# graphcore-research/bess-kge

Measured on AMD Instinct MI355X. Metric: positive+negative triples scored/sec, higher is better.
Workload: dtype f32; 1 GPU; ogbl-biokg-shaped ComplEx d=256 fp32 (W=512), 93,773 entities per shard, n_shard=1, S=4096 positives x 256 per-triple negatives per GPU per step, EmbeddingMoving, mode=score (gather+score+loss); negatives_per_triple=256, mode=score, collectives=none

## Files before the change

bess-kge_amd/besskge/_native.py:

```python

import contextlib
import ctypes
import pathlib
import sys
import threading
from typing import Any, List, Optional, Sequence, Tuple

import torch

LIB_NAME = "libbesskge_hip.so"
ABI_VERSION = 3

TRANSE, ROTATE, DISTMULT, COMPLEX, AFFINE, BOXE = 0, 1, 2, 3, 4, 5
F32, F16 = 0, 1
CORRUPT_HEAD, CORRUPT_TAIL = 0, 1
LOSS_LOGSIGMOID, LOSS_MARGIN, LOSS_SSCE = 0, 1, 2
BAD_NEGATIVE_SCORE = -50000.0

_c_i32p = ctypes.POINTER(ctypes.c_int32)
_c_f32p = ctypes.POINTER(ctypes.c_float)
_c_u8p = ctypes.POINTER(ctypes.c_uint8)
_vp = ctypes.c_void_p
_i64 = ctypes.c_int64
_RETURNS_I64 = ("bess_neg_score_shared_workspace", "bess_neg_score_shared_bwd_workspace",
                "bess_neg_score_shared_fwd_counts_workspace", "bess_neg_score_shared_fwd_pairs_workspace",
                "bess_neg_score_table_fwd_counts_workspace", "bess_neg_score_table_fwd_pairs_workspace")
_i32 = ctypes.c_int32
_f32 = ctypes.c_float


class ModelDesc(ctypes.Structure):

    _fields_ = [
        ("scorer", _i32),
        ("norm_p", _i32),
        ("dtype", _i32),
        ("width", _i32),
        ("rel_width", _i32),
        ("reserved", _i32 * 3),
    ]


class LossDesc(ctypes.Structure):

    _fields_ = [
        ("kind", _i32),
        ("adversarial", _i32),
        ("margin", _f32),
        ("adversarial_scale", _f32),
        ("loss_scale", _f32),
        ("ssce_shift", _f32),
        ("reserved", _i32 * 2),
    ]


class OptDesc(ctypes.Structure):

    _fields_ = [
        ("kind", _i32),
        ("step", _i32),
        ("lr", _f32),
        ("momentum", _f32),
        ("beta1", _f32),
        ("beta2", _f32),
        ("eps", _f32),
        ("weight_decay", _f32),
        ("step_ptr", _i64),
        ("slot_map", _i64),
    ]


OPT_SGD, OPT_ADAGRAD, OPT_ADAM = 0, 1, 2
FLAG_FP32_MATH = 1
FLAG_PREZEROED = 2
FLAG_DNEG_BY_ROW = 4


class KillDesc(ctypes.Structure):

    _fields_ = [
        ("diag_step", _i32),
        ("ht", _i32),
        ("ppp", _i32),
        ("reserved", _i32),
        ("mask", _vp),
        ("mask_rows", _i64),
        ("mask_cols", _i64),
    ]


class Pcg64State(ctypes.Structure):

    _fields_ = [
        ("state_hi", ctypes.c_uint64),
        ("state_lo", ctypes.c_uint64),
        ("inc_hi", ctypes.c_uint64),
        ("inc_lo", ctypes.c_uint64),
        ("has_uint32", ctypes.c_uint32),
        ("uinteger", ctypes.c_uint32),
    ]


_PG = ctypes.POINTER(Pcg64State)

_MD = ctypes.POINTER(ModelDesc)
_LD = ctypes.POINTER(LossDesc)

SIGNATURES = {
    "bess_version": [],
    "bess_last_error": [ctypes.c_char_p, ctypes.c_size_t],
    "bess_gather_rows": [_i32, _i32, _vp, _vp, _i64, _vp, _vp],
    "bess_score_triple_fwd": [_MD, _vp, _vp, _vp, _vp, _vp, _vp, _i64, _vp, _vp],
    "bess_score_triple_bwd": [_MD, _vp, _vp, _vp, _vp, _vp, _vp, _i64, _vp, _vp, _vp, _vp, _vp],
    "bess_query_fwd": [_MD, _i32, _vp, _vp, _vp, _vp, _i64, _vp, _vp],
    "bess_query_bwd": [_MD, _i32, _vp, _vp, _vp, _vp, _i64, _vp, _vp, _vp, _vp],
    "bess_query_triple_fwd": [_MD, _i32, _vp, _vp, _vp, _vp, _vp, _vp, _i64, _vp, _vp, _vp],
    "bess_query_triple_bwd": [_MD, _i32, _vp, _vp, _vp, _vp, _vp, _vp, _i64, _vp, _vp, _vp, _vp, _vp, _vp],
    "bess_sparse_sgd_lists": [_i32, _i32, _vp, _i32, ctypes.POINTER(_vp), ctypes.POINTER(_vp), ctypes.POINTER(_i64), _f32, _vp],
    "bess_sparse_sgd_lists_axpy": [_i32, _i32, _vp, _i32, ctypes.POINTER(_vp), ctypes.POINTER(_vp), ctypes.POINTER(_i64), _f32,
                                   _vp, _vp, _i64, _f32, _vp],
    "bess_neg_score_pertriple_fwd": [_MD, _vp, _i64, _vp, _vp, _i64, _vp, _i64, _vp],
    "bess_neg_score_pertriple_bwd": [_MD, _vp, _i64, _vp, _vp, _i64, _vp, _i64, _vp, _vp, _vp],
    "bess_neg_score_shared_fwd": [_MD, _vp, _i64, _vp, _vp, _i64, _vp, _i64, _vp],
    "bess_neg_score_shared_workspace": [_MD, _i64, _i64],
    "bess_neg_score_shared_fwd_ws": [_MD, _vp, _i64, _vp, _vp, _i64, _vp, _i64, _vp, _i64, _vp],
    "bess_neg_score_shared_fwd_pruned": [_MD, _vp, _i64, _vp, _vp, _i64, _vp, _i64, _vp, _vp, _i64, _vp, _i64, _vp],
    "bess_neg_score_shared_fwd_counts_workspace": [_MD, _i64, _i64],
    "bess_neg_score_shared_fwd_counts": [_MD, _vp, _i64, _vp, _vp, _i64, _vp, _vp, _vp, _i32, _vp, _i64, _vp],
    "bess_neg_score_shared_fwd_pairs_workspace": [_MD, _i64, _i64],
    "bess_neg_score_shared_fwd_pairs": [_MD, _vp, _vp, _vp, _i64, _i64, _i64, _vp, _vp, _i64, _vp],
    "bess_neg_score_table_fwd_counts_workspace": [_MD, _i64, _i64],
    "bess_neg_score_table_fwd_counts": [_MD, _vp, _i64, _vp, _vp, _i64, _vp, _vp, _vp, _i32, _vp, _i64, _vp],
    "bess_neg_score_table_fwd_pairs_workspace": [_MD, _i64, _i64],
    "bess_neg_score_table_fwd_pairs": [_MD, _vp, _vp, _vp, _i64, _i64, _i64, _vp, _vp, _i64, _vp],
    "bess_topk_update_flagged": [_vp, _i64, _i64, _i64, _vp, _i64, _i32, _vp, _vp, _i32, _vp],
    "bess_neg_score_shared_fwd_masked": [_MD, _vp, _i64, _vp, _vp, _i64, _vp, _i64, ctypes.POINTER(KillDesc), _vp, _i64, _vp],
    "bess_neg_score_shared_bwd": [_MD, _vp, _i64, _vp, _vp, _i64, _vp, _i64, _vp, _i64, _vp, _vp, _vp],
    "bess_neg_score_shared_bwd_workspace": [_MD, _i64, _i64],
    "bess_neg_score_shared_bwd_ws": [_MD, _vp, _i64, _vp, _vp, _i64, _vp, _i64, _vp, _i64, _vp, _vp, _vp, _i64, _vp],
    "bess_mask_scores": [_vp, _i64, _i64, _i64, _i32, _i32, _i32, _vp, _i64, _i64, _vp],
    "bess_loss_fwd_bwd": [_LD, _vp, _vp, _i64, _i64, _i64, _vp, _i64, _vp, _vp, _vp, _vp, _i64, _vp],
    "bess_loss_fwd_bwd_norm": [_LD, _vp, _vp, _i64, _i64, _i64, _vp, _i64, _vp, _vp, _vp, _vp, _i64, _vp, _vp],
    "bess_loss_fwd_bwd_one_launch": [_LD, _vp, _vp, _i64, _i64, _i64, _vp, _i64, _vp, _vp, _vp, _vp, _i64, _vp, _vp, _vp],
    "bess_scatter_add_rows": [_vp, _i32, _vp, _vp, _i64, _f32, _vp],
    "bess_sparse_sgd": [_i32, _i32, _vp, _vp, _vp, _i64, _f32, _vp],
    "bess_dense_sgd": [_i32, _vp, _vp, _i64, _f32, _vp],
    "bess_segment_index_workspace": [_i64, ctypes.POINTER(ctypes.c_size_t)],
    "bess_build_segment_index": [_vp, _i64, _i32, _vp, _vp, _vp, _vp, _vp, _i64, _vp, ctypes.c_size_t, _vp],
    "bess_pad_segments": [_vp, _vp, _i64, _vp, _i32, _vp],
    "bess_step_prologue": [_i32, ctypes.POINTER(_vp), ctypes.POINTER(_vp), ctypes.POINTER(ctypes.c_uint32),
                           ctypes.POINTER(_i64), _i32, ctypes.POINTER(_vp), ctypes.POINTER(_i64), _i32, _vp, _vp, _vp, _vp,
                           _vp, _i64, _vp],
    "bess_neg_pertriple_grad_segments": [_MD, _vp, _i64, _vp, _i64, _vp, _i64, _vp, _vp, _vp, _vp, _i64, _vp, _f32,
                                         _vp, _i64, _vp, _vp, _vp],
    "bess_apply_segments_sgd": [_i32, _i32, _vp, _vp, _vp, _i64, _vp, _f32, _vp],
    "bess_segment_sum_rows": [_i32, _vp, _vp, _vp, _vp, _i64, _vp, _vp],
    "bess_topk_update": [_vp, _i64, _i64, _i64, _vp, _i64, _i32, _vp, _i64, _vp, _vp, _i32, _vp],
    "bess_topk_update_excl": [_vp, _i64, _i64, _i64, _vp, _i64, _i32, _vp, _i64, _vp, _vp, _i64, _i32, _vp, _vp, _i32, _vp],
    "bess_topk_update_flagged_excl": [_vp, _i64, _i64, _i64, _vp, _i64, _vp, _i32, _vp, _vp, _i64, _i32, _vp, _vp, _i32, _vp],
    "bess_ranks_from_scores": [_vp, _vp, _i64, _i64, _i64, _i32, _i32, _vp, _vp],
    "bess_ranks_from_indices": [_vp, _vp, _i64, _i64, _i32, _vp, _vp],
    "bess_apply_segments_opt": [ctypes.POINTER(OptDesc), _i32, _i32, _vp, _vp, _vp, _i64, _vp, _vp, _vp, _vp, _vp],
    "bess_neg_pertriple_step_segments": [_MD, _vp, _i64, _vp, _i64, _vp, _i64, _vp, _vp, _vp, _vp, _i64,
                                         _vp, _i64, _vp, _vp, ctypes.POINTER(OptDesc), _vp, _vp, _vp, _vp, _vp],
    "bess_map_extra_rows": [_vp, _vp, _i64, _vp, _vp, _i64, _vp, _vp, _vp],
    "bess_assign_state_rows": [_vp, _vp, _i64, _vp, _vp, _vp, _i64, _vp],
    "bess_coalesced_update": [ctypes.POINTER(OptDesc), _i32, _i32, _vp, _i32, ctypes.POINTER(_vp), ctypes.POINTER(_i64),
                              _vp, _vp, _vp, _vp, _i64, _vp, _vp, _vp, _vp, _vp],
    "bess_coalesced_update_axpy": [ctypes.POINTER(OptDesc), _i32, _i32, _vp, _i32, ctypes.POINTER(_vp), ctypes.POINTER(_i64),
                                   _vp, _vp, _vp, _vp, _i64, _vp, _vp, _vp, _vp, _vp, _vp, _i64, _f32, _vp],
    "bess_neg_pertriple_items": [_MD, _i64, _i64, ctypes.POINTER(ctypes.c_int32)],
    "bess_neg_pertriple_sweep": [_MD, _i64, _i64, ctypes.POINTER(ctypes.c_int32)],
    "bess_neg_score_pertriple_fwd_dq": [_MD, _LD, _vp, _i64, _vp, _vp, _i64, _vp, _vp, _i64, _vp, _i64, _vp, _vp, _vp, _vp],
    "bess_neg_score_pertriple_fwd_dq_masked": [_MD, _LD, _vp, _i64, _vp, _vp, _i64, _vp, _vp, _i64, _vp, _i64, _i64, _vp, _i64, _vp,
                                               _vp, _vp, _vp],
    "bess_neg_score_pertriple_fwd_partials": [_MD, _LD, _vp, _i64, _vp, _vp, _i64, _vp, _i64, _vp, _vp, _vp],
    "bess_combine_dq_partials": [_vp, _vp, _i64, _i32, _i32, _vp, _vp, _vp],
    "bess_normalize_rows": [_i32, _vp, _vp, _i64, _i32, _i32, _i32, _vp, _vp, _vp],
    "bess_normalize_rows_bwd": [_vp, _vp, _vp, _i64, _i32, _i32, _vp, _vp],
    "bess_sample_negatives": [_PG, _vp, _i64, _i32, _i32, _i32, _i64, _i64, _vp, _vp, _vp, _vp, _i32, _i32, _vp, _vp],
    "bess_sample_bucket_indices": [_PG, _vp, _i64, _i64, _i64, _vp, _vp, _vp, _vp],
    "bess_lookup_triples": [_vp, _i64, _vp, _i64, _i64, _i64, _i64, _i32, _vp, _vp, _vp, _vp],
    "bess_gather_candidate_lists": [_vp, _vp, _vp, _vp, _i64, _vp, _i64, _i64, _i64, _i64, _i64, _i64, _i64, _i32, _vp, _vp, _vp],
    "bess_comm_unique_id": [_c_u8p],
    "bess_comm_init_rank": [_i32, _i32, _c_u8p, ctypes.POINTER(_vp)],
    "bess_comm_init_all": [_i32, _c_i32p, ctypes.POINTER(_vp)],
    "bess_comm_destroy": [_vp],
    "bess_comm_info": [_vp, _c_i32p, _c_i32p, _c_i32p],
    "bess_alltoall": [_vp, _vp, _vp, _i64, _vp],
    "bess_allgather": [_vp, _vp, _vp, _i64, _vp],
    "bess_allreduce_sum_f32": [_vp, _vp, _vp, _i64, _vp],
    "bess_pack_exchange": [_vp, _i32, _i32, _vp, _vp, _i64, _vp, _vp, _vp],
    "bess_graph_node_counts": [_vp, _c_i32p, _i32],
    "bess_plan_create": [ctypes.POINTER(_vp)],
    "bess_plan_destroy": [_vp],
    "bess_plan_knows": [ctypes.c_char_p],
    "bess_plan_length": [_vp],
    "bess_plan_add_call": [_vp, ctypes.c_char_p, _i32, _c_u8p, ctypes.POINTER(ctypes.c_uint64), ctypes.POINTER(_vp),
                           ctypes.POINTER(_i64)],
    "bess_plan_run": [_vp, _vp],
    "bess_direct_update": [ctypes.POINTER(OptDesc), _i32, _i32, _vp, _i32, ctypes.POINTER(_vp), ctypes.POINTER(_i64), _vp, _vp,
                           _vp, _vp, _vp, _vp, _vp, _i64, _f32, _vp],
    "bess_neg_score_shared_bwd_parts_plan": [_MD, _i64, _i64, _c_i32p, _c_i32p],
    "bess_neg_score_shared_bwd_parts": [_MD, _vp, _i64, _vp, _vp, _i64, _vp, _i64, _vp, _vp, _vp],
    "bess_query_triple_bwd_parts": [_MD, _i32, _vp, _vp, _vp, _vp, _vp, _vp, _i64, _vp, _vp, _i32, _vp, _i32, _i64, _vp,
                                    _vp, _vp, _vp, _vp, _vp],
    "bess_pertriple_tail_supported": [_MD, _i64],
    "bess_pertriple_tail": [_MD, _LD, _i32, _vp, _vp, _vp, _vp, _vp, _vp, _i64, _vp, _vp, _i32, _vp, _vp, _i64, _i64, _vp,
                            _i64, _vp, _vp, _vp, _vp, _i64, _vp, _vp, _vp, _vp, _vp, _vp],
    "bess_query_triple_fwd_jobs": [_MD, _i32, _vp, _vp, _vp, _vp, _vp, _vp, _i64, _vp, _vp, _i32, ctypes.POINTER(_vp),
                                   ctypes.POINTER(_vp), ctypes.POINTER(ctypes.c_uint32), ctypes.POINTER(_i64), _vp],
    "bess_neg_score_shared_fwd_loss": [_MD, _vp, _i64, _vp, _vp, _i64, _vp, _i64, ctypes.POINTER(KillDesc), _LD, _vp, _vp, _i64,
                                       _vp, _vp, _vp, _vp, _i64, _vp, _vp, _i64, _vp],
}
COMM_ID_BYTES = 128
AFFINE_COUNT_CHUNK_BYTES = 32 << 20
TICKET_INTS = 544
ECOMM_BASE = 10000

_lib: Optional[ctypes.CDLL] = None

_timing: Optional[list] = None
_timed_names: frozenset = frozenset()

TIMING_LABELS = {
    "bess_neg_score_pertriple_fwd_dq_masked": "bess_neg_score_pertriple_fwd_dq",
    "bess_neg_score_shared_fwd_ws": "bess_neg_score_shared_fwd",
    "bess_neg_score_shared_fwd_masked": "bess_neg_score_shared_fwd",
    "bess_neg_score_shared_fwd_pruned": "bess_neg_score_shared_fwd",
    "bess_neg_score_shared_bwd_ws": "bess_neg_score_shared_bwd",
    "bess_neg_score_shared_bwd_parts": "bess_neg_score_shared_bwd",
    "bess_sparse_sgd_lists_axpy": "bess_sparse_sgd_lists",
    "bess_coalesced_update_axpy": "bess_coalesced_update",
    "bess_topk_update_flagged": "bess_topk_update",
    "bess_topk_update_excl": "bess_topk_update",
    "bess_topk_update_flagged_excl": "bess_topk_update",
}


class _Recording(threading.local):
    plan: Optional["Plan"] = None


_recording = _Recording()


def start_kernel_timing(names: Sequence[str]) -> None:
    global _timing, _timed_names
    _timing, _timed_names = [], frozenset(names)


def kernel_timing_log() -> list:
    return list(_timing or [])


def stop_kernel_timing() -> dict:
    global _timing
    rec, _timing = _timing or [], None
    torch.cuda.synchronize()
    out: dict = {}
    for name, _, a, b in rec:
        out.setdefault(TIMING_LABELS.get(name, name), []).append(a.elapsed_time(b))
    return out


def library_path() -> pathlib.Path:
    return pathlib.Path(__file__).parent.absolute() / LIB_NAME


def load() -> ctypes.CDLL:
    global _lib
    if _lib is not None:
        return _lib
    path = library_path()
    if not path.exists():
        raise ImportError(
            f"Cannot find the HIP extension library {LIB_NAME} - tried {[str(path)]}."
            " Build it with `python -c 'import __graft_entry__ as g; g.build()'`"
            " (or `make -C bess-kge_amd/csrc`)."
        )
    lib = ctypes.CDLL(str(path))
    for name, argtypes in SIGNATURES.items():
        try:
            fn = getattr(lib, name)
        except AttributeError as e:
            raise ImportError(f"{path} does not export {name}") from e
        fn.argtypes = argtypes
        fn.restype = ctypes.c_int64 if name in _RETURNS_I64 else ctypes.c_int
    if lib.bess_version() != ABI_VERSION:
        raise ImportError(
            f"{path}: ABI version {lib.bess_version()} != expected {ABI_VERSION}"
        )
    _lib = lib
    return lib


def _check(rc: int, what: str) -> None:
    if rc != 0:
        buf = ctypes.create_string_buffer(512)
        load().bess_last_error(buf, 512)
        kind = "invalid argument" if rc < 0 else (f"ncclResult {rc - ECOMM_BASE}" if rc >= ECOMM_BASE else f"hipError {rc}")
        raise RuntimeError(f"besskge native call {what} failed ({kind}): {buf.value.decode()}")


def _dtype_code(t: torch.Tensor) -> int:
    if t.dtype == torch.float32:
        return F32
    if t.dtype == torch.float16:
        return F16
    raise TypeError(f"embedding tables must be float32 or float16, got {t.dtype}")


def _dev(t: torch.Tensor, name: str) -> torch.device:
    if not t.is_cuda:
        raise RuntimeError(
            f"besskge: `{name}` is on {t.device}; the BESS hot path runs on"
            " HIP devices only (there is no CPU fallback)"
        )
    return t.device


def _same_device(ts: Sequence[Tuple[str, Optional[torch.Tensor]]]) -> torch.device:
    dev = None
    for name, t in ts:
        if t is None:
            continue
        d = _dev(t, name)
        if dev is None:
            dev = d
        elif d != dev:
            raise RuntimeError(f"besskge: `{name}` is on {d}, expected {dev}")
    assert dev is not None
    return dev


def _rows(base: torch.Tensor, name: str, width: int) -> None:
    if base.dim() != 2 or base.shape[1] != width or not base.is_contiguous():
        raise ValueError(
            f"`{name}` must be a contiguous [rows, {width}] tensor, got"
            f" shape {tuple(base.shape)} stride {base.stride()}"
        )


def _idx(idx: Optional[torch.Tensor], name: str, n: Optional[int] = None) -> int:
    if idx is None:
        return 0
    if idx.dtype != torch.int32 or idx.dim() != 1 or not idx.is_contiguous():
        raise ValueError(
            f"`{name}` must be a contiguous 1-D int32 tensor, got {idx.dtype} {tuple(idx.shape)}"
        )
    if n is not None and idx.numel() != n:
        raise ValueError(f"`{name}` has {idx.numel()} entries, expected {n}")
    return idx.data_ptr()


def _f32(t: torch.Tensor, name: str) -> None:
    if t.dtype != torch.float32 or not t.is_contiguous():
        raise ValueError(f"`{name}` must be contiguous float32, got {t.dtype}")


def _row_count(base: torch.Tensor, idx: Optional[torch.Tensor]) -> int:
    return int(idx.numel()) if idx is not None else int(base.shape[0])


def _stream(dev: torch.device) -> int:
    return torch._C._cuda_getCurrentRawStream(dev.index if dev.index is not None else torch.cuda.current_device())


_NO_SWITCH = contextlib.nullcontext()


def _on(dev: torch.device) -> Any:
    if dev.index is None or torch.cuda.current_device() == dev.index:
        return _NO_SWITCH
    return torch.cuda.device(dev)


def _launch(name: str, dev: torch.device, *args: Any) -> None:
# ... 99 lines not shown
    out = torch.empty((n,), dtype=torch.float32, device=dev)
    _launch("bess_score_triple_fwd", dev, ctypes.byref(d), head.base.data_ptr(), _idx(head.idx, "head_idx"),
            tail.base.data_ptr(), _idx(tail.idx, "tail_idx"), rel_table.data_ptr(), rel_idx.data_ptr(), n,
            out.data_ptr())
    return out


def score_triple_bwd(d: ModelDesc, head: RowSource, tail: RowSource, rel_table: torch.Tensor,
                     rel_idx: torch.Tensor, d_out: torch.Tensor, d_rel_table: torch.Tensor
                     ) -> Tuple[torch.Tensor, torch.Tensor]:
    dev, n = _triple_operands(d, head, tail, rel_table, rel_idx)
    _same_device([("d_out", d_out), ("d_rel_table", d_rel_table), ("x", head.base)])
    _f32(d_out, "d_out")
    _f32(d_rel_table, "d_rel_table")
    if d_out.numel() != n or tuple(d_rel_table.shape) != tuple(rel_table.shape):
        raise ValueError("score_triple_bwd: gradient shapes do not match")
    dh = torch.empty((n, d.width), dtype=torch.float32, device=dev)
    dt = torch.empty((n, d.width), dtype=torch.float32, device=dev)
    _launch("bess_score_triple_bwd", dev, ctypes.byref(d), head.base.data_ptr(), _idx(head.idx, "head_idx"),
            tail.base.data_ptr(), _idx(tail.idx, "tail_idx"), rel_table.data_ptr(), rel_idx.data_ptr(), n,
            d_out.data_ptr(), dh.data_ptr(), dt.data_ptr(), d_rel_table.data_ptr())
    return dh, dt


def _job_arrays(jobs: Sequence[Tuple[torch.Tensor, Optional[torch.Tensor], int]], who: str):
    nj = len(jobs)
    if nj > MAX_WORD_JOBS:
        raise ValueError(f"{who}: too many jobs")
    dst, src = (_vp * max(1, nj))(), (_vp * max(1, nj))()
    val, words = (ctypes.c_uint32 * max(1, nj))(), (_i64 * max(1, nj))()
    for i, (d_, s_, v_) in enumerate(jobs):
        if d_.element_size() != 4 or not d_.is_contiguous():
            raise ValueError(f"{who}: job targets must be contiguous tensors of 4-byte elements")
        if s_ is not None and (s_.element_size() != 4 or not s_.is_contiguous() or s_.numel() != d_.numel()):
            raise ValueError(f"{who}: a job's source must match its target")
        dst[i], src[i], val[i], words[i] = d_.data_ptr(), (s_.data_ptr() if s_ is not None else None), int(v_), d_.numel()
    return dst, src, val, words


def query_triple_fwd(d: ModelDesc, side: int, head: RowSource, tail: RowSource, rel_table: torch.Tensor,
                     rel_idx: torch.Tensor, jobs: Optional[Sequence[Tuple[torch.Tensor, Optional[torch.Tensor], int]]] = None
                     ) -> Tuple[torch.Tensor, torch.Tensor]:
    dev, n = _triple_operands(d, head, tail, rel_table, rel_idx)
    q = torch.empty((n, d.width), dtype=torch.float32, device=dev)
    out = torch.empty((n,), dtype=torch.float32, device=dev)
    if jobs:
        _same_device([("query rows", head.base)] + [("job dst", j[0]) for j in jobs] + [("job src", j[1]) for j in jobs])
        dst, src, val, words = _job_arrays(jobs, "query_triple_fwd")
        _launch("bess_query_triple_fwd_jobs", dev, ctypes.byref(d), side, head.base.data_ptr(),
                _idx(head.idx, "head_idx"), tail.base.data_ptr(), _idx(tail.idx, "tail_idx"), rel_table.data_ptr(),
                rel_idx.data_ptr(), n, q.data_ptr(), out.data_ptr(), len(jobs), dst, src, val, words)
        return q, out
    _launch("bess_query_triple_fwd", dev, ctypes.byref(d), side, head.base.data_ptr(), _idx(head.idx, "head_idx"),
            tail.base.data_ptr(), _idx(tail.idx, "tail_idx"), rel_table.data_ptr(), rel_idx.data_ptr(), n, q.data_ptr(),
            out.data_ptr())
    return q, out


def query_triple_bwd(d: ModelDesc, side: int, head: RowSource, tail: RowSource, rel_table: torch.Tensor,
                     rel_idx: torch.Tensor, d_out: torch.Tensor, d_query: torch.Tensor, d_rel_table: torch.Tensor
                     ) -> Tuple[torch.Tensor, torch.Tensor]:
    dev, n = _triple_operands(d, head, tail, rel_table, rel_idx)
    _same_device([("d_out", d_out), ("d_query", d_query), ("d_rel_table", d_rel_table), ("x", head.base)])
    for t, nm in ((d_out, "d_out"), (d_query, "d_query"), (d_rel_table, "d_rel_table")):
        _f32(t, nm)
    if d_out.numel() != n or tuple(d_query.shape) != (n, d.width) or tuple(d_rel_table.shape) != tuple(rel_table.shape):
        raise ValueError("query_triple_bwd: gradient shapes do not match")
    dh = torch.empty((n, d.width), dtype=torch.float32, device=dev)
    dt = torch.empty((n, d.width), dtype=torch.float32, device=dev)
    _launch("bess_query_triple_bwd", dev, ctypes.byref(d), side, head.base.data_ptr(), _idx(head.idx, "head_idx"),
            tail.base.data_ptr(), _idx(tail.idx, "tail_idx"), rel_table.data_ptr(), rel_idx.data_ptr(), n,
            d_out.data_ptr(), d_query.data_ptr(), dh.data_ptr(), dt.data_ptr(), d_rel_table.data_ptr())
    return dh, dt


def _query_operands(d: ModelDesc, ent: RowSource, rel_table: torch.Tensor, rel_idx: torch.Tensor):
    dev = _same_device([("entity rows", ent.base), ("entity idx", ent.idx),
                        ("relation_embedding", rel_table), ("relation", rel_idx)])
    _rows(ent.base, "entity rows", d.width)
    _rows(rel_table, "relation_embedding", d.rel_width)
    if _dtype_code(ent.base) != d.dtype or _dtype_code(rel_table) != d.dtype:
        raise TypeError("query: operand dtype does not match the model descriptor")
    n = len(ent)
    _idx(rel_idx, "relation", n)
    return dev, n


def query_fwd(d: ModelDesc, side: int, ent: RowSource, rel_table: torch.Tensor, rel_idx: torch.Tensor) -> torch.Tensor:
    dev, n = _query_operands(d, ent, rel_table, rel_idx)
    q = torch.empty((n, query_width(d)), dtype=torch.float32, device=dev)
    _launch("bess_query_fwd", dev, ctypes.byref(d), side, ent.base.data_ptr(), _idx(ent.idx, "entity idx"),
            rel_table.data_ptr(), rel_idx.data_ptr(), n, q.data_ptr())
    return q


def query_bwd(d: ModelDesc, side: int, ent: RowSource, rel_table: torch.Tensor, rel_idx: torch.Tensor,
              d_query: torch.Tensor, d_rel_table: torch.Tensor) -> torch.Tensor:
    dev, n = _query_operands(d, ent, rel_table, rel_idx)
    _same_device([("d_query", d_query), ("d_rel_table", d_rel_table), ("x", ent.base)])
    _f32(d_query, "d_query")
    _f32(d_rel_table, "d_rel_table")
    if tuple(d_query.shape) != (n, query_width(d)) or tuple(d_rel_table.shape) != tuple(rel_table.shape):
        raise ValueError("query_bwd: gradient shapes do not match")
    dx = torch.empty((n, d.width), dtype=torch.float32, device=dev)
    _launch("bess_query_bwd", dev, ctypes.byref(d), side, ent.base.data_ptr(), _idx(ent.idx, "entity idx"),
            rel_table.data_ptr(), rel_idx.data_ptr(), n, d_query.data_ptr(), dx.data_ptr(), d_rel_table.data_ptr())
    return dx


def query_width(d: ModelDesc) -> int:
    if d.scorer == AFFINE:
        n_part = int(d.reserved[0])
        return (n_part + 1) * (d.width // n_part)
    if d.scorer == BOXE:
        return 3 * d.width
    return int(d.width)


def _neg_operands(d: ModelDesc, query: torch.Tensor, neg: RowSource, n_idx: int):
    dev = _same_device([("query", query), ("negative rows", neg.base), ("negative idx", neg.idx)])
    _f32(query, "query")
    if query.dim() != 2 or query.shape[1] != query_width(d):
        raise ValueError(f"`query` must be [n_query, {query_width(d)}], got {tuple(query.shape)}")
    _rows(neg.base, "negative rows", d.width)
    if _dtype_code(neg.base) != d.dtype:
        raise TypeError("negative rows dtype does not match the model descriptor")
    if len(neg) != n_idx:
        raise ValueError(f"expected {n_idx} negative rows, got {len(neg)}")
    return dev


def _neg_idx_ptr(neg: RowSource, dev: torch.device) -> Tuple[int, Optional[torch.Tensor]]:
    if neg.idx is not None:
        return _idx(neg.idx, "negative idx"), None
    ar = torch.arange(neg.base.shape[0], dtype=torch.int32, device=dev)
    return ar.data_ptr(), ar


def neg_score_pertriple_fwd(d: ModelDesc, query: torch.Tensor, neg: RowSource, n_neg: int,
                            out: Optional[torch.Tensor] = None) -> torch.Tensor:
    nq = int(query.shape[0])
    dev = _neg_operands(d, query, neg, nq * n_neg)
    if out is None:
        out = torch.empty((nq, n_neg), dtype=torch.float32, device=dev)
    _f32(out, "out")
    if tuple(out.shape) != (nq, n_neg):
        raise ValueError("neg_score_pertriple_fwd: bad `out` shape")
    ip, keep = _neg_idx_ptr(neg, dev)
    d = with_row_count(d, neg.base)
    _launch("bess_neg_score_pertriple_fwd", dev, ctypes.byref(d), query.data_ptr(), nq, neg.base.data_ptr(), ip, n_neg,
            out.data_ptr(), n_neg)
    del keep
    return out


def neg_score_pertriple_fwd_dq(d: ModelDesc, l: LossDesc, query: torch.Tensor, neg: RowSource, n_neg: int,
                               pos: Optional[torch.Tensor], weight: torch.Tensor, mask: Optional[torch.Tensor] = None,
                               defer: bool = False) -> Tuple[torch.Tensor, Any]:
    nq = int(query.shape[0])
    dev = _neg_operands(d, query, neg, nq * n_neg)
    _same_device([("pos", pos), ("weight", weight), ("query", query)])
    _f32(weight, "weight")
    if weight.numel() not in (1, nq):
        raise ValueError("triple weights must have 1 or n_query entries")
    if pos is not None:
        _f32(pos, "pos")
        if pos.numel() != nq:
            raise ValueError("`pos` must have n_query entries")
    items = ctypes.c_int32(0)
    _check(load().bess_neg_pertriple_items(ctypes.byref(d), nq, n_neg, ctypes.byref(items)), "bess_neg_pertriple_items")
    out = torch.empty((nq, n_neg), dtype=torch.float32, device=dev)
    dq = None if defer else torch.empty((nq, d.width), dtype=torch.float32, device=dev)
    st_ml = torch.empty((nq, items.value, 2), dtype=torch.float32, device=dev)
    st_acc = torch.empty((nq, items.value, d.width), dtype=torch.float32, device=dev)
    ip, keep = _neg_idx_ptr(neg, dev)
    mrows = mcols = 0
    if mask is not None:
        _same_device([("mask", mask), ("query", query)])
        if mask.dtype not in (torch.bool, torch.uint8) or mask.dim() != 2 or not mask.is_contiguous():
            raise ValueError("neg_score_pertriple_fwd_dq: `mask` must be a contiguous 2-D bool / uint8 tensor")
        mrows, mcols = int(mask.shape[0]), int(mask.shape[1])
    _launch("bess_neg_score_pertriple_fwd_dq_masked", dev, ctypes.byref(d), ctypes.byref(l), query.data_ptr(), nq,
            neg.base.data_ptr(), ip, n_neg, pos.data_ptr() if pos is not None else 0, weight.data_ptr(), weight.numel(),
            mask.data_ptr() if mask is not None else 0, mrows, mcols, out.data_ptr(), n_neg,
            dq.data_ptr() if dq is not None else 0, st_ml.data_ptr(), st_acc.data_ptr())
    del keep
    return out, ((st_ml, st_acc) if defer else dq)


def pertriple_tail_supported(d: ModelDesc, n_neg: int) -> bool:
    return bool(load().bess_pertriple_tail_supported(ctypes.byref(d), int(n_neg)))


def pertriple_tail(d: ModelDesc, l: LossDesc, side: int, head: RowSource, tail: RowSource, rel_table: torch.Tensor,
                   rel_idx: torch.Tensor, partials: Tuple[torch.Tensor, torch.Tensor], pos: torch.Tensor, neg: torch.Tensor,
                   weight: torch.Tensor, d_rel_table: torch.Tensor, want_d_query: bool = False) -> Tuple[Any, ...]:
    dev, n = _triple_operands(d, head, tail, rel_table, rel_idx)
    st_ml, st_acc = partials
    _same_device([("partials", st_ml), ("partials", st_acc), ("positive_score", pos), ("negative_score", neg),
                  ("triple_weight", weight), ("d_rel_table", d_rel_table), ("x", head.base)])
    for t, nm in ((st_ml, "partials"), (st_acc, "partials"), (pos, "positive_score"), (neg, "negative_score"),
                  (weight, "triple_weight"), (d_rel_table, "d_rel_table")):
        _f32(t, nm)
    N = int(neg.shape[1])
    items = int(st_ml.shape[1])
    if tuple(st_ml.shape) != (n, items, 2) or tuple(st_acc.shape) != (n, items, d.width) or pos.numel() != n \
            or neg.shape[0] != n or weight.numel() not in (1, n) or tuple(d_rel_table.shape) != tuple(rel_table.shape):
        raise ValueError("pertriple_tail: shapes do not match")
    n4 = (n + 3) // 4 * 4
    small = torch.empty((2 * n4 + 4,), dtype=torch.float32, device=dev)
    row_loss, dp, loss = small[:n], small[n4: n4 + n], small[2 * n4: 2 * n4 + 1]
    dn = torch.empty((n, N), dtype=torch.float32, device=dev)
    rows = torch.empty((3 if want_d_query else 2, n, d.width), dtype=torch.float32, device=dev)
    counter = _counters(dev, 1)
    _launch("bess_pertriple_tail", dev, ctypes.byref(d), ctypes.byref(l), side, head.base.data_ptr(),
            _idx(head.idx, "head_idx"), tail.base.data_ptr(), _idx(tail.idx, "tail_idx"), rel_table.data_ptr(),
            rel_idx.data_ptr(), n, st_ml.data_ptr(), st_acc.data_ptr(), items, pos.data_ptr(), neg.data_ptr(), N,
            int(neg.stride(0)), weight.data_ptr(), weight.numel(), row_loss.data_ptr(), loss.data_ptr(), dp.data_ptr(),
            dn.data_ptr(), N, rows[2].data_ptr() if want_d_query else 0, rows[0].data_ptr(), rows[1].data_ptr(),
            d_rel_table.data_ptr(), counter.data_ptr())
    res = (loss.reshape(()), dp, dn, rows[0], rows[1])
    return res + (rows[2],) if want_d_query else res


def row_fits_registers(d: ModelDesc) -> bool:
    W = int(d.width)
    vec = 4 if d.dtype == F32 else 8
    if W % vec:
        vec = 2 if (d.dtype == F16 and W % 2 == 0) else 1
    return W <= 256 * vec


def neg_score_pertriple_fwd_partials(d: ModelDesc, l: LossDesc, query: torch.Tensor, neg: RowSource, n_neg: int
                                     ) -> Tuple[torch.Tensor, Tuple[torch.Tensor, torch.Tensor]]:
    nq = int(query.shape[0])
    dev = _neg_operands(d, query, neg, nq * n_neg)
    items = ctypes.c_int32(0)
    _check(load().bess_neg_pertriple_items(ctypes.byref(d), nq, n_neg, ctypes.byref(items)), "bess_neg_pertriple_items")
    out = torch.empty((nq, n_neg), dtype=torch.float32, device=dev)
    st_ml = torch.empty((nq, items.value, 2), dtype=torch.float32, device=dev)
    st_acc = torch.empty((nq, items.value, d.width), dtype=torch.float32, device=dev)
    ip, keep = _neg_idx_ptr(neg, dev)
    _launch("bess_neg_score_pertriple_fwd_partials", dev, ctypes.byref(d), ctypes.byref(l), query.data_ptr(), nq,
            neg.base.data_ptr(), ip, n_neg, out.data_ptr(), n_neg, st_ml.data_ptr(), st_acc.data_ptr())
    del keep
    return out, (st_ml, st_acc)


def combine_dq_partials(state: Tuple[torch.Tensor, torch.Tensor], norm: torch.Tensor) -> torch.Tensor:
    st_ml, st_acc = state
    nq, items, W = (int(x) for x in st_acc.shape)
    dev = _same_device([("state_ml", st_ml), ("state_acc", st_acc), ("norm", norm)])
    _f32(norm, "norm")
    if tuple(norm.shape) != (nq, 2) or not norm.is_contiguous():
        raise ValueError("combine_dq_partials: `norm` must be a contiguous [n_query, 2] tensor")
    dq = torch.empty((nq, W), dtype=torch.float32, device=dev)
    _launch("bess_combine_dq_partials", dev, st_ml.data_ptr(), st_acc.data_ptr(), nq, items, W, norm.data_ptr(),
            dq.data_ptr())
    return dq


def neg_score_pertriple_bwd(d: ModelDesc, query: torch.Tensor, neg: RowSource, n_neg: int,
                            d_out: torch.Tensor, want_d_neg: bool = True, want_d_query: bool = True,
                            d_neg_rows: Optional[torch.Tensor] = None
                            ) -> Tuple[Optional[torch.Tensor], Optional[torch.Tensor]]:
    nq = int(query.shape[0])
    dev = _neg_operands(d, query, neg, nq * n_neg)
    _same_device([("d_out", d_out), ("query", query)])
    _f32(d_out, "d_out")
    if tuple(d_out.shape) != (nq, n_neg):
        raise ValueError("neg_score_pertriple_bwd: bad `d_out` shape")
    if not want_d_query and (int(d.scorer) > COMPLEX or not want_d_neg):
        raise ValueError("neg_score_pertriple_bwd: want_d_query=False is for the four native scorers, with d_neg")
    dq = torch.empty((nq, query_width(d)), dtype=torch.float32, device=dev) if want_d_query else None
    dn = torch.empty((nq * n_neg, d.width), dtype=torch.float32, device=dev) if want_d_neg else None
    if d_neg_rows is not None:
        if (int(d.scorer) > COMPLEX or not want_d_neg or d_neg_rows.dtype != torch.float32 or not d_neg_rows.is_contiguous()
                or tuple(d_neg_rows.shape) != (int(neg.base.shape[0]), int(d.width)) or d_neg_rows.device != dev):
            raise ValueError("neg_score_pertriple_bwd: `d_neg_rows` must be a contiguous f32 [rows of neg.base, W] "
                             "tensor (native scorers)")
        d = copy_desc(d)
        d.reserved[0] |= FLAG_DNEG_BY_ROW
        dn = d_neg_rows
    ip, keep = _neg_idx_ptr(neg, dev)
    _launch("bess_neg_score_pertriple_bwd", dev, ctypes.byref(d), query.data_ptr(), nq, neg.base.data_ptr(), ip, n_neg,
            d_out.data_ptr(), n_neg, dq.data_ptr() if want_d_query else 0, dn.data_ptr() if want_d_neg else 0)
    del keep
    return dq, (None if d_neg_rows is not None else dn)


def normalize_rows(neg: RowSource, n_part: int, normalize: bool) -> Tuple[torch.Tensor, torch.Tensor]:
    dev = _same_device([("rows", neg.base), ("idx", neg.idx)])
    W = int(neg.base.shape[1])
    _rows(neg.base, "rows", W)
    n = len(neg)
    hat = torch.empty((n, W), dtype=torch.float32, device=dev)
    inv = torch.empty((n, n_part), dtype=torch.float32, device=dev)
    _launch("bess_normalize_rows", dev, _dtype_code(neg.base), neg.base.data_ptr(), _idx(neg.idx, "idx"), n, W, n_part,
            int(normalize), hat.data_ptr(), inv.data_ptr())
    return hat, inv


def normalize_rows_bwd(hat: torch.Tensor, inv: torch.Tensor, d_hat: torch.Tensor) -> torch.Tensor:
    dev = _same_device([("hat", hat), ("inv", inv), ("d_hat", d_hat)])
    for t, name in ((hat, "hat"), (inv, "inv"), (d_hat, "d_hat")):
        _f32(t, name)
# ... 1149 lines not shown
```

bess-kge_amd/besskge/bess.py:

```python

from abc import ABC, abstractmethod
from typing import Any, Dict, List, Optional, Tuple, Union

import torch

from besskge import _native as nat
from besskge._native import RowSource
from besskge.collectives import ReplicaGroup, SingleProcessGroup
from besskge.loss import BaseLossFunction, SampledSoftmaxCrossEntropyLoss
from besskge.negative_sampler import (
    ShardedNegativeSampler,
    TripleBasedShardedNegativeSampler,
)
from besskge.scoring import BaseScoreFunction

BAD_NEGATIVE_SCORE = -50000.0

_Batch = Dict[str, torch.Tensor]



def _i32(x: torch.Tensor) -> torch.Tensor:
    x = x if x.dtype == torch.int32 else x.to(torch.int32)
    return x.contiguous()


class _PlainSGD:

    kind = nat.OPT_SGD
    momentum = 0.0
    weight_decay = 0.0
    is_plain_sgd = True

    def __init__(self, lr: float) -> None:
        self.lr = float(lr)


class _NegGroup:

    def __init__(self, side: int, sel: Optional[torch.Tensor], ent: RowSource, rel_idx: torch.Tensor,
                 neg: RowSource, shared: bool, n_per_query: int) -> None:
        self.side = side
        self.sel = sel
        self.ent = ent
        self.rel_idx = rel_idx
        self.neg = neg
        self.shared = shared
        self.n_per_query = n_per_query
        self.query: Optional[torch.Tensor] = None
        self.query_ctx: Any = None
        self.out: Optional[torch.Tensor] = None
        self.dq: Optional[torch.Tensor] = None
        self.partials: Any = None
        self.kill: Any = None
        self.neg_parts: Optional[List[torch.Tensor]] = None
        self.bwd_buf: Optional[torch.Tensor] = None


class _SmallPlan(list):

    def __init__(self) -> None:
        super().__init__()
        self.concats: Dict[int, Tuple[int, int]] = {}


class _ReplicaStep:

    def __init__(self) -> None:
        self.table: torch.Tensor = None
        self.triple_ctx: Any = None
        self.head_idx: torch.Tensor = None
        self.rel_idx: torch.Tensor = None
        self.tail: RowSource = None
        self.groups: List[_NegGroup] = []
        self.send_idx: Optional[torch.Tensor] = None
        self.recv: Optional[torch.Tensor] = None
        self.recv_rows: int = 0
        self.ext_src: Optional[RowSource] = None
        self.n: int = 1
        self.ppp: int = 0
        self.neg_shape: Tuple[int, ...] = ()
        self.local_neg: torch.Tensor = None
        self.local_tail: torch.Tensor = None
        self.positive_score: torch.Tensor = None
        self.negative_score: torch.Tensor = None
        self.loss_norm: Optional[torch.Tensor] = None
        self.kill_applied = False
        self.fused_qt = False
        self.tail_pre: Optional[Tuple[torch.Tensor, torch.Tensor]] = None
        self.jobs: Optional[List[Tuple[torch.Tensor, Optional[torch.Tensor], int]]] = None
        self.d_recv: Optional[torch.Tensor] = None
        self.loss_pre: Optional[Tuple[torch.Tensor, torch.Tensor, torch.Tensor]] = None
        self.direct: Any = None
        self.direct_lists: List[torch.Tensor] = []
        self.jobs_ride = False


class _PendingUpdate:

    __slots__ = ("steps", "local_updates", "deferred", "d_rel")

    def __init__(self, steps: List[_ReplicaStep], local_updates: List[List[Tuple[torch.Tensor, torch.Tensor]]],
                 deferred: List[Tuple[torch.Tensor, _NegGroup, torch.Tensor]], d_rel: torch.Tensor) -> None:
        self.steps = steps
        self.local_updates = local_updates
        self.deferred = deferred
        self.d_rel = d_rel


class _MergedGroup:

    __slots__ = ("query", "n_per_query")

    def __init__(self, query: torch.Tensor, n_per_query: int) -> None:
        self.query, self.n_per_query = query, n_per_query


class BessKGE(torch.nn.Module, ABC):

    def __init__(
        self,
        negative_sampler: ShardedNegativeSampler,
        score_fn: BaseScoreFunction,
        loss_fn: Optional[BaseLossFunction] = None,
        evaluation: Optional[Any] = None,
        return_scores: bool = False,
        augment_negative: bool = False,
    ) -> None:
        super().__init__()
        self.sharding = score_fn.sharding
        self.negative_sampler = negative_sampler
        self.score_fn = score_fn
        self.loss_fn = loss_fn
        self.evaluation = evaluation
        self.return_scores = return_scores
        self.augment_negative = augment_negative
        if not (loss_fn or evaluation or return_scores):
            raise ValueError(
                "Nothing to return. At least one of loss_fn,"
                " evaluation or return_scores needs to be != None"
            )
        if self.augment_negative:
            assert (
                score_fn.negative_sample_sharing
            ), "Negative augmentation requires negative sample sharing"
            assert not isinstance(
                self, ScoreMovingBessKGE
            ), "ScoreMovingBessKGE does not support negative augmentation"
        if negative_sampler.flat_negative_format:
            assert (
                score_fn.negative_sample_sharing
            ), "Using flat negative format requires negative sample sharing"
        elif score_fn.negative_sample_sharing and isinstance(
            self.negative_sampler, TripleBasedShardedNegativeSampler
        ):
            raise ValueError(
                "Negative sample sharing cannot be used"
                " with non-flat triple-specific negatives"
            )
        self.entity_embedding = self.score_fn.entity_embedding
        self.entity_embedding_size: int = self.score_fn.entity_embedding.shape[-1]
        self.replica_group: Optional[ReplicaGroup] = None
        self._shard_slot: Optional[Dict[int, int]] = None
        self._map_cache: Dict[Any, torch.Tensor] = {}

    @property
    def n_embedding_parameters(self) -> int:
        return self.score_fn.entity_embedding.numel() + self.score_fn.relation_embedding.numel()

    def attach(self, group: ReplicaGroup, shard_slot: Optional[Dict[int, int]] = None) -> None:
        if group.n_shard != self.sharding.n_shard:
            raise ValueError(f"group has {group.n_shard} replicas, sharding {self.sharding.n_shard}")
        self.replica_group = group
        self._shard_slot = shard_slot

    def _group(self) -> ReplicaGroup:
        if self.replica_group is None:
            self.replica_group = SingleProcessGroup(self.sharding.n_shard)
        return self.replica_group

    def _local_table(self, shard: int) -> torch.Tensor:
        emb = self.score_fn.entity_embedding
        slot = shard if self._shard_slot is None else self._shard_slot[shard]
        if emb.dim() != 3 or slot >= emb.shape[0]:
            raise RuntimeError(
                f"entity_embedding {tuple(emb.shape)} does not hold shard {shard};"
                " use besskge.runtime to place the shards"
            )
# ... 566 lines not shown
                contrib = list(upd)
                for table, g, go in deferred:
                    if table is st.table:
                        seg = seg_index[id(g)]
                        gseg = nat.neg_pertriple_grad_segments(desc, g.query, table, g.n_per_query, go, seg)
                        contrib.append(nat.pad_segments(seg, gseg))
                last = st is steps[-1]
                self._apply_optimizer(optimizer, st.table, contrib,
                                      (getattr(self, "_small_ahead", None) or {}).get(id(st)),
                                      axpy=rel_axpy if last else None)
                rel_done = rel_done or (last and rel_axpy is not None)
        if rel_done:
            pass
        elif plain:
            nat.dense_sgd(rel_table, d_rel, lr)
        else:
            self._apply_optimizer_dense(optimizer, rel_table, d_rel)
        dense_grads = self.score_fn.__dict__.pop("dense_grads", {})
        for p in self.score_fn.dense_parameters():
            g = dense_grads.get(p)
            if g is None:
                continue
            (g,) = group.all_reduce_sum([g.contiguous()]) if len(group.local_shards) == 1 else (g,)
            as_table = p.data.view(p.shape[0], -1) if p.dim() > 1 else p.data.view(1, -1)
            g = g.reshape(as_table.shape).contiguous()
            if mean_over_replicas:
                g = g / group.n_shard
            if plain:
                nat.dense_sgd(as_table, g, lr)
            else:
                self._apply_optimizer_dense(optimizer, as_table, g)


    def _run_groups_one(self, g: _NegGroup, desc: nat.ModelDesc, st: Optional[_ReplicaStep] = None,
                        fuse: Optional[Dict[str, Any]] = None, partials_loss: Any = None) -> torch.Tensor:
        ahead = getattr(self, "_seg_ahead", None)
        if ahead is not None and st is not None and self._wants_segments(g, st):
            ahead[id(g)] = self._segment_index_on_side(g, st)
        if g.query is None:
            g.query, g.query_ctx = self.score_fn.query_fwd(g.side, g.ent, g.rel_idx)
        with_loss = getattr(self, "_train_loss_in_scoring", None)
        if g.shared and with_loss is not None and st is not None and len(st.groups) == 1 and g.sel is None \
                and (st.kill_applied or with_loss.get("no_kill")):
            b = with_loss["batch"]
            w = self._triple_weight(b, g.query.device)
            g.out, loss, d_pos, d_neg = nat.neg_score_shared_fwd_loss(
                desc, self.loss_fn.kernel_desc(len(g.neg)), g.query, g.neg, st.positive_score, w, kill=g.kill)
            st.loss_pre = (loss, d_pos, d_neg)
        elif g.shared:
            g.out = nat.neg_score_shared_fwd(desc, g.query, g.neg, kill=g.kill)
        elif fuse is not None and st is not None and (
                g.neg.base is st.table or (g.neg.base is st.recv and self.score_fn.bilinear_candidates)):
            pos, w = st.positive_score, fuse["weight"]
            if g.sel is not None:
                pos = pos[g.sel].contiguous()
                w = w if w.numel() == 1 else w[g.sel].contiguous()
            d_rel = self.__dict__.get("_step_d_rel")
            defer = (self.pertriple_tail and st.fused_qt and g.sel is None and g.neg.base is st.table and d_rel is not None
                     and not self.evaluation and nat.pertriple_tail_supported(desc, g.n_per_query))
            ldesc = fuse["loss"](g.n_per_query)
            g.out, g.dq = nat.neg_score_pertriple_fwd_dq(desc, ldesc, g.query, g.neg, g.n_per_query, pos, w,
                                                         mask=fuse.get("mask"), defer=defer)
            if defer:
                loss, d_pos, d_neg, dh, dt = nat.pertriple_tail(
                    desc, ldesc, g.side, RowSource(st.table, st.head_idx), st.tail, self.score_fn.relation_embedding.data,
                    st.rel_idx, g.dq, pos, g.out, w, d_rel)
                st.loss_pre = (loss, d_pos, d_neg)
                st.tail_pre = (dh, dt)
        elif partials_loss is not None:
            g.out, g.partials = nat.neg_score_pertriple_fwd_partials(desc, partials_loss, g.query, g.neg, g.n_per_query)
        else:
            g.out = nat.neg_score_pertriple_fwd(desc, g.query, g.neg, g.n_per_query)
        return g.out

    def _run_groups(self, st: _ReplicaStep, desc: nat.ModelDesc, fuse: Optional[Dict[str, Any]] = None
                    ) -> List[torch.Tensor]:
        return [self._run_groups_one(g, desc, st, fuse) for g in st.groups]

    def _fusable(self, batch: _Batch) -> Optional[Dict[str, Any]]:
        if self.loss_fn is None or not self.score_fn.supports_fused_forward or self.augment_negative:
            return None
        if not hasattr(self.loss_fn, "kernel_desc") or not nat.row_fits_registers(self.score_fn.kernel_desc()):
            return None
        dev = self.score_fn.relation_embedding.device
        w = self._triple_weight(batch, dev)
        return dict(weight=w, loss=self.loss_fn.kernel_desc, masked=batch.get("negative_mask") is not None)


class EmbeddingMovingBessKGE(BessKGE):

    def score_batch_replicas(self, batches: List[_Batch]) -> List[_ReplicaStep]:
        group = self._group()
        n = group.n_shard
        ns = self.negative_sampler
        fn = self.score_fn
        W = self.entity_embedding_size
        steps: List[_ReplicaStep] = []
        sends: List[torch.Tensor] = []
        exchange_negatives = n > 1 and not ns.local_sampling
        packed_exchange = (hasattr(group, "pack_exchange")
                           and (W * self.score_fn.entity_embedding.element_size()) % 16 == 0)
        prologue = self.__dict__.get("_small_early") is not None
        for shard, b in zip(group.local_shards, batches):
            st = _ReplicaStep()
            if prologue:
                st.jobs = []
            st.table = self._local_table(shard)
            dev = st.table.device
            head, rel, tail, neg = (b[k].to(dev) for k in ("head", "relation", "tail", "negative"))
            if head.shape[0] != n or neg.shape[0] != n:
                raise ValueError(f"batch is laid out for {head.shape[0]} shards, group has {n}")
            st.n, st.ppp = n, int(head.shape[1])
            st.head_idx = head.reshape(-1)
            st.rel_idx = rel.reshape(-1)
            st.neg_shape = tuple(neg.shape)
            if n > 1:
                parts = [tail] + ([neg.flatten(start_dim=1)] if exchange_negatives else [])
                st.send_idx = torch.cat(parts, dim=1).contiguous()
                if packed_exchange:
                    sends.append(group.pack_exchange(st.table, st.send_idx))
                else:
                    sends.append(nat.gather_rows(st.table, st.send_idx.reshape(-1)).reshape(n, -1, W))
            st.local_neg = neg
            st.local_tail = tail
            steps.append(st)
        if n > 1:
            recvs = sends if packed_exchange else group.all_to_all(sends)
            for st, y in zip(steps, recvs):
                st.recv = y.reshape(-1, W)
                st.recv_rows = st.recv.shape[0]

        desc = fn.kernel_desc()
        rel_table = fn.relation_embedding.data
        done: List[_ReplicaStep] = []
        fuse = getattr(self, "_train_fuse", None)
        for st, b in zip(steps, batches):
            self._build_groups(st, exchange_negatives)
            src = b.get("_kill_from")
            if src is not None and len(st.groups) == 1 and st.groups[0].shared:
                st.groups[0].kill = self._kill_spec(src, st.n, st.ppp, st.n * st.ppp, st.table.device)
                st.kill_applied = st.groups[0].kill is not None
            g0 = st.groups[0]
            st.fused_qt = (len(st.groups) == 1 and g0.sel is None and fn.supports_fused_query_triple
                           and st.tail.base.dtype == st.table.dtype)
            early = getattr(self, "_small_early", None)
            if early is not None:
                d_rel = None
                if not done:
                    d_rel = self.__dict__["_step_d_rel"] = torch.empty(rel_table.shape, dtype=torch.float32,
                                                                       device=rel_table.device)
                ahead = self._launch_prologue(st, self._ahead_optimizer, d_rel)
                if ahead is not None:
                    early[id(st)] = ahead
            if st.fused_qt:
                g0.query, st.positive_score = fn.query_triple_fwd(g0.side, RowSource(st.table, st.head_idx), st.tail,
                                                                  st.rel_idx, jobs=st.jobs if st.jobs_ride else None)
                if st.jobs_ride:
                    st.jobs = None
            else:
                st.positive_score, st.triple_ctx = fn.triple_fwd(
                    RowSource(st.table, st.head_idx), st.tail, st.rel_idx)
            if early is not None and id(st) not in early:
                early.update(self._small_index_ahead([st], self._ahead_optimizer))
            fz = fuse[len(done)] if fuse else None
            if fz is not None and fz.get("masked"):
                kill = self._kill_spec(b["_kill_from"], st.n, st.ppp, st.n * st.ppp, st.table.device) \
                    if b.get("_kill_from") is not None else None
                g0 = st.groups[0]
                ok = (kill is not None and kill[0] == 0 and not kill[1] and kill[3] is not None
                      and kill[3].shape[0] in (1, st.n * st.ppp) and len(st.groups) == 1 and g0.sel is None
                      and not g0.shared and g0.neg.base is st.table and kill[3].shape[1] <= g0.n_per_query)
                if ok:
                    fz = dict(fz, mask=kill[3])
                    st.kill_applied = True
                else:
                    fz = None
            in_scoring = self.__dict__.get("_train_loss_in_scoring_on")
            if in_scoring and self.loss_fn is not None and hasattr(self.loss_fn, "kernel_desc") and not self.evaluation:
                src_b = b.get("_kill_from")
                if src_b is not None:
                    no_kill = (not st.kill_applied
                               and self._kill_spec(src_b, st.n, st.ppp, st.n * st.ppp, st.table.device) is None)
                    self.__dict__["_train_loss_in_scoring"] = dict(batch=src_b, no_kill=no_kill)
            try:
                outs = self._run_groups(st, desc, fz)
            finally:
                self.__dict__["_train_loss_in_scoring"] = None
            done.append(st)
            if len(outs) == 1:
                st.negative_score = outs[0]
            else:
                n_, cut = st.n, st.ppp // 2
                st.negative_score = torch.cat(
                    [outs[0].reshape(n_, cut, -1), outs[1].reshape(n_, st.ppp - cut, -1)], dim=1
                ).flatten(end_dim=1).contiguous()
        return steps

    def _build_groups(self, st: _ReplicaStep, exchange_negatives: bool) -> None:
        ns = self.negative_sampler
        fn = self.score_fn
        n, ppp = st.n, st.ppp
        S = n * ppp
        _, B, K = st.neg_shape
        dev = st.table.device
        sharing = bool(fn.negative_sample_sharing)

        if n == 1:
            tail_src = RowSource(st.table, st.local_tail.reshape(-1))
            neg_base = st.table
            neg_idx2d = st.local_neg[0]
        else:
            L = ppp + (B * K if exchange_negatives else 0)
            tail_map = self._static_map(
                ("tail", n, ppp, L),
                lambda: (torch.arange(n)[:, None] * L + torch.arange(ppp)[None, :]).reshape(-1), dev)
            tail_src = RowSource(st.recv, tail_map)
            if exchange_negatives:
                neg_base = st.recv
                neg_idx2d = self._static_map(
                    ("neg", n, ppp, B, K),
                    lambda: (torch.arange(n)[None, :, None] * L + ppp
                             + torch.arange(B)[:, None, None] * K + torch.arange(K)[None, None, :]
                             ).reshape(B, n * K), dev)
            else:
                neg_base = st.table
                neg_idx2d = st.local_neg.transpose(0, 1).reshape(B, n * K).contiguous()
        st.tail = tail_src
        head_src = RowSource(st.table, st.head_idx)
        nK = int(neg_idx2d.shape[1])
        scheme = ns.corruption_scheme

        pos_of = {nat.CORRUPT_HEAD: head_src, nat.CORRUPT_TAIL: tail_src}
        base_of = {nat.CORRUPT_HEAD: neg_base, nat.CORRUPT_TAIL: neg_base}
        rows_of = {nat.CORRUPT_HEAD: neg_idx2d, nat.CORRUPT_TAIL: neg_idx2d}
        if self.augment_negative and n > 1:
            if neg_base is st.recv and scheme in ("h", "ht"):
                st.recv = torch.cat([st.recv, nat.gather_rows(st.table, st.head_idx)], dim=0)
                st.ext_src = head_src
                tail_src = st.tail = RowSource(st.recv, tail_src.idx)
                ext_idx = st.recv_rows + torch.arange(S, dtype=torch.int32, device=dev)
                pos_of[nat.CORRUPT_HEAD] = RowSource(st.recv, ext_idx)
                pos_of[nat.CORRUPT_TAIL] = tail_src
                base_of = {nat.CORRUPT_HEAD: st.recv, nat.CORRUPT_TAIL: st.recv}
            elif neg_base is st.table and scheme in ("t", "ht"):
                local_rows = neg_idx2d.reshape(-1).contiguous()
                st.recv = torch.cat([st.recv, nat.gather_rows(st.table, local_rows)], dim=0)
                st.ext_src = RowSource(st.table, local_rows)
                tail_src = st.tail = RowSource(st.recv, tail_src.idx)
                pos_of[nat.CORRUPT_TAIL] = tail_src
                base_of[nat.CORRUPT_TAIL] = st.recv
                rows_of[nat.CORRUPT_TAIL] = (st.recv_rows + torch.arange(local_rows.numel(), dtype=torch.int32, device=dev)
                                             ).reshape(neg_idx2d.shape)

        def make(side: int, sel: Optional[torch.Tensor], rows2d: torch.Tensor) -> _NegGroup:
            ent_src = tail_src if side == nat.CORRUPT_HEAD else head_src
            pos_src = pos_of[side]
            rel = st.rel_idx
            if sel is not None:
                ent_src = RowSource(ent_src.base, ent_src.idx[sel])
                pos_src = RowSource(pos_src.base, pos_src.idx[sel])
                rel = rel[sel].contiguous()
            Q = len(ent_src)
            Bg = int(rows2d.shape[0])
            base = base_of[side]
            if self.augment_negative:
                assert pos_src.base is base
                if st.jobs is not None and Bg == 1 and len(st.jobs) + 4 <= nat.MAX_WORD_JOBS:
                    parts = [pos_src.idx.reshape(-1).contiguous(), rows2d.reshape(-1).contiguous()]
                    lst = torch.empty((parts[0].numel() + parts[1].numel(),), dtype=torch.int32, device=dev)
                    st.jobs.append((lst[: parts[0].numel()], parts[0], 0))
                    st.jobs.append((lst[parts[0].numel():], parts[1], 0))
                    g = _NegGroup(side, sel, ent_src, rel, RowSource(base, lst), True, int(lst.numel()))
                    g.neg_parts = parts
                    return g
                rows2d = torch.cat([pos_src.idx.reshape(Bg, -1), rows2d], dim=1)
            if sharing or Bg == 1:
                lst = rows2d.reshape(-1).contiguous()
                return _NegGroup(side, sel, ent_src, rel, RowSource(base, lst), True, int(lst.numel()))
            if Bg != Q:
                raise ValueError(f"per-triple negatives: {Bg} candidate lists for {Q} queries")
            return _NegGroup(side, sel, ent_src, rel, RowSource(base, rows2d.reshape(-1).contiguous()),
                             False, int(rows2d.shape[1]))

        rows_hd, rows_tl = rows_of[nat.CORRUPT_HEAD], rows_of[nat.CORRUPT_TAIL]
        if scheme == "h":
            st.groups = [make(nat.CORRUPT_HEAD, None, rows_hd)]
        elif scheme == "t":
            st.groups = [make(nat.CORRUPT_TAIL, None, rows_tl)]
        elif scheme == "ht":
            cut = ppp // 2
            slot = torch.arange(S, device=dev).reshape(n, ppp)
            sel_h = slot[:, :cut].reshape(-1)
            sel_t = slot[:, cut:].reshape(-1)
            if ns.flat_negative_format:
                rows_h, rows_t = rows_hd[0:1], rows_tl[1:2]
            else:
                rows_h = rows_hd.reshape(n, ppp, nK)[:, :cut].reshape(-1, nK)
                rows_t = rows_tl.reshape(n, ppp, nK)[:, cut:].reshape(-1, nK)
            st.groups = [make(nat.CORRUPT_HEAD, sel_h, rows_h), make(nat.CORRUPT_TAIL, sel_t, rows_t)]
        else:
            raise ValueError(f"corruption scheme {scheme!r} not supported")

    def train_step_replicas(self, batches: List[_Batch], optimizer: Any,
                            pending: Optional[List[_PendingUpdate]] = None) -> List[Dict[str, Any]]:
        if self.loss_fn is None:
            raise RuntimeError("train_step needs a loss function")
# ... 396 lines not shown
```

bess-kge_amd/besskge/scoring.py:

```python

import struct
from abc import ABC, abstractmethod
from typing import Any, Callable, Dict, List, Optional, Tuple, Union

import torch

from besskge import _native as nat
from besskge import ops
from besskge.embedding import (
    init_KGE_normal,
    init_KGE_uniform,
    init_uniform_norm,
    init_uniform_rotation,
    init_xavier_norm,
    initialize_entity_embedding,
    initialize_relation_embedding,
    refactor_embedding_sharding,
)
from besskge.sharding import Sharding

_Init = Union[torch.Tensor, List[Callable[..., torch.Tensor]]]


def _placement(kw: Optional[Dict[str, Any]]) -> Dict[str, Any]:
    kw = dict(kw or {})
    out = dict(device=kw.pop("device", None), shards=kw.pop("shards", None), dtype=kw.pop("dtype", None))
    if kw:
        raise TypeError(f"unexpected keyword arguments {sorted(kw)}")
    return out


class BaseScoreFunction(torch.nn.Module, ABC):

    negative_sample_sharing: bool
    sharding: Sharding
    entity_embedding: torch.nn.Parameter
    relation_embedding: torch.nn.Parameter

    _scorer_id: int = -1

    def kernel_desc(self) -> nat.ModelDesc:
        rel, ent = self.relation_embedding, self.entity_embedding
        key = (rel.dtype, int(ent.shape[-1]), int(rel.shape[-1]), int(getattr(self, "scoring_norm", 0)),
               bool(getattr(self, "fp32_math", False)))
        cached = self.__dict__.get("_kernel_desc_cache")
        if cached is not None and cached[0] == key:
            return cached[1]
        d = nat.ModelDesc()
        d.scorer = self._scorer_id
        d.norm_p = key[3]
        d.dtype = nat._dtype_code(rel)
        d.width = key[1]
        d.rel_width = key[2]
        if 0 <= self._scorer_id <= nat.COMPLEX and key[4]:
            d.reserved[0] = nat.FLAG_FP32_MATH
        self.__dict__["_kernel_desc_cache"] = (key, d)
        return d

    fp32_math: bool = False

    def _table_dtype(self, x: torch.Tensor) -> torch.Tensor:
        dt = self.relation_embedding.dtype
        return x if x.dtype == dt else x.to(dt)

    supports_fused_segments = True
    supports_fused_forward = True
    bilinear_candidates = False
    supports_fused_query_triple = True

    def query_triple_fwd(self, side: int, head: nat.RowSource, tail: nat.RowSource, rel_idx: torch.Tensor,
                         jobs: Any = None) -> Tuple[torch.Tensor, torch.Tensor]:
        return nat.query_triple_fwd(self.kernel_desc(), side, head, tail, self.relation_embedding.data, rel_idx,
                                    jobs=jobs)

    def query_triple_bwd(self, side: int, head: nat.RowSource, tail: nat.RowSource, rel_idx: torch.Tensor,
                         d_pos: torch.Tensor, dq: torch.Tensor, d_rel: torch.Tensor
                         ) -> Tuple[torch.Tensor, torch.Tensor]:
        return nat.query_triple_bwd(self.kernel_desc(), side, head, tail, self.relation_embedding.data, rel_idx,
                                    d_pos, dq, d_rel)

    def query_triple_bwd_parts(self, side: int, head: nat.RowSource, tail: nat.RowSource, rel_idx: torch.Tensor,
                               d_pos: torch.Tensor, dq_parts: torch.Tensor, dneg_parts: torch.Tensor, neg_idx: torch.Tensor,
                               rows_acc: Tuple[torch.Tensor, torch.Tensor, torch.Tensor], d_rel: torch.Tensor) -> None:
        nat.query_triple_bwd_parts(self.kernel_desc(), side, head, tail, self.relation_embedding.data, rel_idx, d_pos,
                                   dq_parts, dneg_parts, neg_idx, rows_acc, d_rel)

    def dense_parameters(self) -> List[torch.nn.Parameter]:
        return []

    def _collect_dense(self, grads: Any) -> None:
        store = self.__dict__.setdefault("dense_grads", {})
        for p, g in zip(self.dense_parameters(), grads):
            if g is not None:
                store[p] = g.float() if p not in store else store[p] + g.float()

    def query_fwd(self, side: int, ent: nat.RowSource, rel_idx: torch.Tensor) -> Tuple[torch.Tensor, Any]:
        return nat.query_fwd(self.kernel_desc(), side, ent, self.relation_embedding.data, rel_idx), None

    def query_bwd(self, side: int, ent: nat.RowSource, rel_idx: torch.Tensor, ctx: Any, dq: torch.Tensor,
                  d_rel: torch.Tensor) -> torch.Tensor:
        return nat.query_bwd(self.kernel_desc(), side, ent, self.relation_embedding.data, rel_idx, dq, d_rel)

    def triple_fwd(self, head: nat.RowSource, tail: nat.RowSource, rel_idx: torch.Tensor) -> Tuple[torch.Tensor, Any]:
        return nat.score_triple_fwd(self.kernel_desc(), head, tail, self.relation_embedding.data, rel_idx), None

    def triple_bwd(self, head: nat.RowSource, tail: nat.RowSource, rel_idx: torch.Tensor, ctx: Any,
                   d_pos: torch.Tensor, d_rel: torch.Tensor) -> Tuple[torch.Tensor, torch.Tensor]:
        return nat.score_triple_bwd(self.kernel_desc(), head, tail, self.relation_embedding.data, rel_idx, d_pos,
                                    d_rel)

    def score_triple(
        self, head_emb: torch.Tensor, relation_id: torch.Tensor, tail_emb: torch.Tensor
    ) -> torch.Tensor:
        return ops.ScoreTriple.apply(
            self.kernel_desc(),
            self._table_dtype(head_emb),
            self.relation_embedding,
            relation_id,
            self._table_dtype(tail_emb),
        )

    def score_heads(
        self, head_emb: torch.Tensor, relation_id: torch.Tensor, tail_emb: torch.Tensor
    ) -> torch.Tensor:
        return ops.ScoreNegatives.apply(
            self.kernel_desc(),
            nat.CORRUPT_HEAD,
            bool(self.negative_sample_sharing),
            self._table_dtype(tail_emb),
            self.relation_embedding,
            relation_id,
            self._table_dtype(head_emb),
        )

    def score_tails(
        self, head_emb: torch.Tensor, relation_id: torch.Tensor, tail_emb: torch.Tensor
    ) -> torch.Tensor:
        return ops.ScoreNegatives.apply(
            self.kernel_desc(),
            nat.CORRUPT_TAIL,
            bool(self.negative_sample_sharing),
            self._table_dtype(head_emb),
            self.relation_embedding,
            relation_id,
            self._table_dtype(tail_emb),
        )

    def forward(
        self, head_emb: torch.Tensor, relation_id: torch.Tensor, tail_emb: torch.Tensor
    ) -> torch.Tensor:
        return self.score_triple(head_emb, relation_id, tail_emb)

    def update_sharding(self, new_sharding: Sharding) -> None:
        self.entity_embedding = refactor_embedding_sharding(
            entity_embedding=self.entity_embedding,
            old_sharding=self.sharding,
            new_sharding=new_sharding,
        )
        self.sharding = new_sharding

    def _allocate(
        self,
        sharding: Sharding,
        n_relation_type: int,
        inverse_relations: bool,
        entity_initializer: _Init,
        relation_initializer: _Init,
        entity_width: int,
        relation_width: int,
        what: str,
        placement: Optional[Dict[str, Any]] = None,
    ) -> None:
        self.sharding = sharding
        pl = _placement(placement)
        self.entity_embedding = initialize_entity_embedding(
            sharding, entity_initializer, [entity_width], **pl
        )
        self.relation_embedding = initialize_relation_embedding(
            n_relation_type, inverse_relations, relation_initializer, [relation_width],
            device=pl["device"], dtype=pl["dtype"]
        )
        assert (
            self.entity_embedding.shape[-1] == entity_width
            and self.relation_embedding.shape[-1] == relation_width
        ), what


class DistanceBasedScoreFunction(BaseScoreFunction, ABC):

    supported_norms: Optional[Tuple[int, ...]] = None

    def __init__(self, negative_sample_sharing: bool, scoring_norm: int) -> None:
        super().__init__()
        if int(scoring_norm) != scoring_norm or scoring_norm < 1:
            raise ValueError(f"scoring_norm must be an integer p >= 1, got {scoring_norm!r}")
        if self.supported_norms is not None and scoring_norm not in self.supported_norms:
            raise ValueError(f"the HIP kernels of {type(self).__name__} implement scoring_norm in {self.supported_norms}")
        self.negative_sample_sharing = negative_sample_sharing
        self.scoring_norm = int(scoring_norm)

    def reduce_embedding(self, v: torch.Tensor) -> torch.Tensor:
        return torch.norm(v, p=self.scoring_norm, dim=-1)

    def broadcasted_distance(self, v1: torch.Tensor, v2: torch.Tensor) -> torch.Tensor:
        return -ops.ReduceNegatives.apply(_plain_desc(nat.TRANSE, self.scoring_norm, v2), bool(self.negative_sample_sharing),
                                          v1.float().contiguous(), v2)


def _plain_desc(scorer: int, norm_p: int, rows: torch.Tensor) -> nat.ModelDesc:
    d = nat.ModelDesc()
    d.scorer, d.norm_p = scorer, int(norm_p)
    d.dtype = nat._dtype_code(rows)
    d.width = d.rel_width = int(rows.shape[-1])
    return d


class MatrixDecompositionScoreFunction(BaseScoreFunction, ABC):

    def __init__(self, negative_sample_sharing: bool) -> None:
        super().__init__()
        self.negative_sample_sharing = negative_sample_sharing

    def reduce_embedding(self, v: torch.Tensor) -> torch.Tensor:
        return torch.sum(v, dim=-1)

    def broadcasted_dot_product(self, v1: torch.Tensor, v2: torch.Tensor) -> torch.Tensor:
# ... 658 lines not shown
```

bess-kge_amd/csrc/loss.hip:

```cpp
#include "common.h"
#include "loss_rows.h"

namespace bess {

__global__ __launch_bounds__(256) void k_mask_scores(float* __restrict__ neg, int64_t n_triple,
                                                     int64_t n_neg, int64_t ld, int diag_step, int ht,
                                                     int ppp, const uint8_t* __restrict__ mask,
                                                     int64_t mask_rows, int64_t mask_cols) {
    const int64_t total = n_triple * n_neg;
    const int cut = ppp / 2;
    for (int64_t t = blockIdx.x * 256ll + threadIdx.x; t < total; t += 256ll * gridDim.x) {
        const int64_t s = t / n_neg;
        const int64_t j = t - s * n_neg;
        const int64_t blk = ppp > 0 ? s / ppp : 0;
        const int p = ppp > 0 ? static_cast<int>(s - blk * ppp) : 0;
        bool kill = false;
        if (diag_step > 0) {
            const int64_t qpos = ht ? (blk * cut + (p % cut)) : s;
            kill = (j == static_cast<int64_t>(diag_step) * qpos);
        }
        const int64_t mj = j - (n_neg - mask_cols);
        if (mask && mj >= 0) {
            int64_t mrow = s;
            if (mask_rows == 1) mrow = 0;
            else if (mask_rows == 2) mrow = (p >= cut) ? 1 : 0;
            kill = mask[mrow * mask_cols + mj] == 0;
        }
        if (kill) neg[s * ld + j] += BESS_BAD_NEGATIVE_SCORE;
    }
}

template <int KIND, bool ADV, bool GRAD, int CH>
__global__ __launch_bounds__(256) void k_loss_rows(bess_loss_desc l, const float* __restrict__ pos,
                                                   const float* __restrict__ neg, int64_t n_triple,
                                                   int64_t n_neg, int64_t ld_neg,
                                                   const float* __restrict__ weight,
                                                   int64_t weight_len, float* __restrict__ row_loss,
                                                   float* __restrict__ d_pos,
                                                   float* __restrict__ d_neg, int64_t ld_dneg,
                                                   float* __restrict__ row_norm, int32_t* __restrict__ counter,
                                                   float* __restrict__ loss) {
    const int64_t s = blockIdx.x * 4ll + (threadIdx.x >> 6);
    if (s < n_triple)
        loss_row<KIND, ADV, GRAD, CH>(l, pos, neg, s, n_neg, ld_neg, weight, weight_len, row_loss, d_pos, d_neg, ld_dneg,
                                      row_norm);
    if (!counter) return;
    __shared__ float part[256];
    __shared__ int last;
    release_to_agent();
    __syncthreads();
    if (threadIdx.x == 0) last = last_workgroup_ticket(counter);
    __syncthreads();
    if (!last) return;
    float acc = 0.f;
    for (int64_t i = threadIdx.x; i < n_triple; i += 256) acc += load_agent(row_loss + i);
    part[threadIdx.x] = acc;
    __syncthreads();
    for (int h = 128; h > 0; h >>= 1) {
        if (threadIdx.x < h) part[threadIdx.x] += part[threadIdx.x + h];
        __syncthreads();
    }
    if (threadIdx.x == 0) loss[0] = part[0];
}

__global__ __launch_bounds__(256) void k_ranks_from_scores(const float* __restrict__ pos,
                                                           const float* __restrict__ cand, int64_t n_row,
                                                           int64_t n_cand, int64_t ld, int mode, int worst_inf,
                                                           float* __restrict__ rank) {
    const int lane = threadIdx.x & 63;
    const int64_t s = blockIdx.x * 4ll + (threadIdx.x >> 6);
    if (s >= n_row) return;
    float p = pos[s];
    if (p != p) p = -INFINITY;
    const float* row = cand + s * ld;
    float gt = 0.f, ge = 0.f;
    for (int64_t j = lane; j < n_cand; j += 64) {
        const float c = row[j];
        gt += (c > p) ? 1.f : 0.f;
        ge += (c >= p) ? 1.f : 0.f;
    }
    gt = wave_allreduce_sum(gt);
    ge = wave_allreduce_sum(ge);
    if (lane == 0) {
        const float n = static_cast<float>(n_cand);
        float better;
        bool worst;
        if (mode == 0) { better = gt; worst = gt == n; }
        else if (mode == 1) { better = ge; worst = ge == n; }
        else { better = 0.5f * (gt + ge); worst = (gt == n) || (ge == n); }
        rank[s] = (worst_inf && worst) ? INFINITY : 1.f + better;
    }
}

__global__ __launch_bounds__(256) void k_ranks_from_indices(const int64_t* __restrict__ truth,
                                                            const int64_t* __restrict__ cand, int64_t n_row,
                                                            int64_t n_cand, int worst_inf,
                                                            float* __restrict__ rank) {
    const int64_t s = blockIdx.x * 256ll + threadIdx.x;
    if (s >= n_row) return;
    const int64_t t = truth[s];
    float r = worst_inf ? INFINITY : static_cast<float>(n_cand + 1);
    for (int64_t j = n_cand - 1; j >= 0; --j)
        if (cand[s * n_cand + j] == t) r = static_cast<float>(j + 1);
    rank[s] = r;
}

__global__ __launch_bounds__(1024) void k_sum_rows(const float* __restrict__ row_loss, int64_t n,
                                                   float* __restrict__ loss) {
    __shared__ float part[1024];
    float acc = 0.f;
    for (int64_t i = threadIdx.x; i < n; i += 1024) acc += row_loss[i];
    part[threadIdx.x] = acc;
    __syncthreads();
    for (int s = 512; s > 0; s >>= 1) {
        if (threadIdx.x < s) part[threadIdx.x] += part[threadIdx.x + s];
        __syncthreads();
    }
    if (threadIdx.x == 0) loss[0] = part[0];
}

template <int KIND, bool ADV, int CH>
static void launch_loss_ch(bool grad, const bess_loss_desc& l, const float* pos, const float* neg,
                           int64_t S, int64_t N, int64_t ld, const float* w, int64_t wl, float* rl,
                           float* dp, float* dn, int64_t ldd, float* rn, int32_t* cnt, float* loss, hipStream_t st) {
    const unsigned grid = static_cast<unsigned>(ceil_div(S, 4));
    if (grad) k_loss_rows<KIND, ADV, true, CH><<<grid, 256, 0, st>>>(l, pos, neg, S, N, ld, w, wl, rl, dp, dn, ldd, rn, cnt, loss);
    else k_loss_rows<KIND, ADV, false, CH><<<grid, 256, 0, st>>>(l, pos, neg, S, N, ld, w, wl, rl, dp, dn, ldd, rn, cnt, loss);
}

template <int KIND, bool ADV>
static void launch_loss(bool grad, const bess_loss_desc& l, const float* pos, const float* neg,
                        int64_t S, int64_t N, int64_t ld, const float* w, int64_t wl, float* rl,
                        float* dp, float* dn, int64_t ldd, float* rn, int32_t* cnt, float* loss, hipStream_t st) {
    const bool vec = N % 4 == 0 && ld % 4 == 0 && reinterpret_cast<uintptr_t>(neg) % 16 == 0 &&
                     (!grad || (ldd % 4 == 0 && reinterpret_cast<uintptr_t>(dn) % 16 == 0));
#define BESS_LOSS_CH(CH) launch_loss_ch<KIND, ADV, CH>(grad, l, pos, neg, S, N, ld, w, wl, rl, dp, dn, ldd, rn, cnt, loss, st)
    if (!vec) BESS_LOSS_CH(0);
    else if (N > 256 * 24) BESS_LOSS_CH(-1);
    else if (N <= 256 * 4) BESS_LOSS_CH(4);
    else if (N <= 256 * 12) BESS_LOSS_CH(12);
    else BESS_LOSS_CH(24);
#undef BESS_LOSS_CH
}

}

using namespace bess;

extern "C" int bess_mask_scores(float* neg, int64_t n_triple, int64_t n_neg, int64_t ld,
                                int32_t diag_step, int32_t ht, int32_t ppp, const uint8_t* mask,
                                int64_t mask_rows, int64_t mask_cols, void* stream) {
    BESS_REQUIRE(n_triple >= 0 && n_neg >= 0 && ld >= n_neg, "mask_scores: bad sizes");
    if (n_triple == 0 || n_neg == 0) return BESS_OK;
    BESS_REQUIRE(neg, "mask_scores: NULL scores");
    BESS_REQUIRE(diag_step >= 0, "mask_scores: negative diag_step");
    if (mask) {
        BESS_REQUIRE(mask_cols > 0 && mask_cols <= n_neg, "mask_scores: mask_cols %lld not in (0, n_neg]", (long long)mask_cols);
        BESS_REQUIRE(mask_rows == 1 || mask_rows == 2 || mask_rows == n_triple,
                     "mask_scores: mask_rows %lld not 1, 2 or n_triple", (long long)mask_rows);
    } else {
        mask_cols = 0;
    }
    if (ht || mask_rows == 2)
        BESS_REQUIRE(ppp >= 2 && (ppp % 2) == 0 && (n_triple % ppp) == 0, "mask_scores: 'ht' needs an even block size dividing n_triple");
    const int64_t total = n_triple * n_neg;
    int64_t blocks = ceil_div(total, 256);
    if (blocks > 4096) blocks = 4096;
    k_mask_scores<<<static_cast<unsigned>(blocks), 256, 0, as_stream(stream)>>>(
        neg, n_triple, n_neg, ld, diag_step, ht, ppp, mask, mask_rows, mask_cols);
    return check_launch("mask_scores");
}

extern "C" int bess_loss_fwd_bwd(const bess_loss_desc* l, const float* pos, const float* neg,
                                 int64_t n_triple, int64_t n_neg, int64_t ld_neg,
                                 const float* weight, int64_t weight_len, float* row_loss,
                                 float* loss, float* d_pos, float* d_neg, int64_t ld_dneg,
                                 void* stream) {
    return bess_loss_fwd_bwd_norm(l, pos, neg, n_triple, n_neg, ld_neg, weight, weight_len, row_loss, loss, d_pos, d_neg,
                                  ld_dneg, nullptr, stream);
}

static int loss_impl(const bess_loss_desc* l, const float* pos, const float* neg, int64_t n_triple, int64_t n_neg,
                     int64_t ld_neg, const float* weight, int64_t weight_len, float* row_loss, float* loss,
                     float* d_pos, float* d_neg, int64_t ld_dneg, float* row_norm, int32_t* counter, void* stream) {
    BESS_REQUIRE(l, "loss: NULL descriptor");
    BESS_REQUIRE(l->kind >= BESS_LOSS_LOGSIGMOID && l->kind <= BESS_LOSS_SSCE, "loss: unknown kind %d", l->kind);
    BESS_REQUIRE(n_triple > 0 && n_neg > 0 && n_neg < (1ll << 31), "loss: bad sizes");
    BESS_REQUIRE(pos && neg && weight && row_loss && loss, "loss: NULL pointer");
    BESS_REQUIRE(weight_len == 1 || weight_len == n_triple, "loss: weight_len must be 1 or n_triple");
    BESS_REQUIRE(ld_neg >= n_neg, "loss: leading dimension < n_neg");
    const bool grad = d_pos || d_neg;
    if (grad) BESS_REQUIRE(d_pos && d_neg && ld_dneg >= n_neg, "loss: gradients need d_pos, d_neg and ld_dneg >= n_neg");
    hipStream_t st = as_stream(stream);
    const bool adv = l->adversarial != 0;
    if (n_triple > 4 * 4096) counter = nullptr;
#define BESS_LOSS(KIND, ADV) \
    launch_loss<KIND, ADV>(grad, *l, pos, neg, n_triple, n_neg, ld_neg, weight, weight_len, row_loss, d_pos, d_neg, ld_dneg, \
                           row_norm, counter, loss, st)
    switch (l->kind) {
        case BESS_LOSS_LOGSIGMOID: adv ? BESS_LOSS(BESS_LOSS_LOGSIGMOID, true) : BESS_LOSS(BESS_LOSS_LOGSIGMOID, false); break;
        case BESS_LOSS_MARGIN: adv ? BESS_LOSS(BESS_LOSS_MARGIN, true) : BESS_LOSS(BESS_LOSS_MARGIN, false); break;
        default: BESS_LOSS(BESS_LOSS_SSCE, false);
    }
#undef BESS_LOSS
    if (int e = check_launch("loss rows")) return e;
    if (counter) return BESS_OK;
    k_sum_rows<<<1, 1024, 0, st>>>(row_loss, n_triple, loss);
    return check_launch("loss sum");
// ... 43 lines not shown
```

bess-kge_amd/csrc/neg_pertriple.hip:

```cpp
#include "common.h"
#include "loss_rows.h"

namespace bess {

struct NegPtArgs {
    const float* query;
    const void* base;
    const int32_t* idx;
    int64_t n_query;
    int n_neg;
    int W;
    int nch;
    int nb;
    int items_per_query;
    float sign;
    int accum = 0;
    float p = 2.f;
    int dn_by_row = 0;
    int sweep_shift = -1;
};

struct FuseArgs {
    const float* pos;
    int kind;
    float beta;
    float margin;
    float shift;
    float* st_ml;
    float* st_acc;
    const uint8_t* mask = nullptr;
    int64_t mask_rows = 0;
    int mask_cols = 0, mask_from = 0;
};

__device__ __forceinline__ float sigmoid_f(float x) { return 1.f / (1.f + expf(-x)); }

template <typename T, int VEC, int IT, int RED, int UNROLL, bool FUSE>
__global__ __launch_bounds__(256) void k_neg_pertriple_fwd(NegPtArgs a, float* __restrict__ out,
                                                           int64_t ld_out, FuseArgs f) {
    const int lane = threadIdx.x & 63;
    const int g = lane & 15;
    const int sub = lane >> 4;
    const int64_t item = blockIdx.x * 4ll + (threadIdx.x >> 6);
    if (item >= a.n_query * a.items_per_query) return;
    const int64_t q = item / a.items_per_query;
    const int k0 = static_cast<int>(item - q * a.items_per_query) * a.nb;
    const int k1 = min(k0 + a.nb, a.n_neg);

    float qv[IT][VEC];
    const float* qp = a.query + q * a.W;
#pragma unroll
    for (int it = 0; it < IT; ++it) {
        load_chunk<float, VEC>(qp, g + 16 * it, a.nch, qv[it]);
    }

    const T* base = static_cast<const T*>(a.base);
    const int32_t* idx = a.idx + q * a.n_neg;
    float* orow = out + q * ld_out;
    float fm = -INFINITY, fl = 0.f, facc[IT][VEC];
    float fpos = 0.f;
    if (FUSE) {
#pragma unroll
        for (int it = 0; it < IT; ++it)
#pragma unroll
            for (int v = 0; v < VEC; ++v) facc[it][v] = 0.f;
        if (f.kind == BESS_LOSS_MARGIN) fpos = f.pos[q];
    }

    int32_t nrow[UNROLL];
#pragma unroll
    for (int u = 0; u < UNROLL; ++u) nrow[u] = idx[min(k0 + sub + 4 * u, k1 - 1)];
    for (int kb = k0; kb < k1; kb += 4 * UNROLL) {
        float ev[UNROLL][IT][VEC];
        bool valid[UNROLL];
#pragma unroll
        for (int u = 0; u < UNROLL; ++u) {
            const int k = kb + sub + 4 * u;
            valid[u] = k < k1;
            const T* rp = base + static_cast<int64_t>(nrow[u]) * a.W;
            nrow[u] = idx[min(k + 4 * UNROLL, k1 - 1)];
#pragma unroll
            for (int it = 0; it < IT; ++it) {
                load_chunk<T, VEC>(rp, g + 16 * it, a.nch, ev[u][it]);
            }
        }
#pragma unroll
        for (int u = 0; u < UNROLL; ++u) {
            float acc = 0.f;
#pragma unroll
            for (int it = 0; it < IT; ++it) {
#pragma unroll
                for (int v = 0; v < VEC; ++v) {
                    if (RED == RED_DOT) {
                        acc = fmaf(qv[it][v], ev[u][it][v], acc);
                    } else if (RED == RED_L1) {
                        acc += fabsf(qv[it][v] - ev[u][it][v]);
                    } else {
                        acc += lp_term(qv[it][v] - ev[u][it][v], a.p);
                    }
                }
            }
            acc = row16_allreduce_sum(acc);
            if (RED == RED_L2) acc = lp_root(acc, a.p);
            float sc = a.sign * acc;
            if (FUSE && f.mask && valid[u]) {
                const int kcol = kb + sub + 4 * u - f.mask_from;
                const int64_t mrow = f.mask_rows == 1 ? 0 : q;
                if (kcol >= 0 && f.mask[mrow * f.mask_cols + kcol] == 0) sc += BESS_BAD_NEGATIVE_SCORE;
            }
            if (g == 0 && valid[u]) orow[kb + sub + 4 * u] = a.accum ? orow[kb + sub + 4 * u] + sc : sc;
            if (FUSE && valid[u]) {
                const float z = f.beta * (sc + f.shift);
                const float m_new = fmaxf(fm, z);
                const float corr = expf(fm - m_new);
                const float e = expf(z - m_new);
                float gs = 1.f;
                if (f.kind == BESS_LOSS_LOGSIGMOID) gs = sigmoid_f(sc + f.margin);
                else if (f.kind == BESS_LOSS_MARGIN) gs = (sc - fpos + f.margin > 0.f) ? 1.f : 0.f;
                const float p = e * gs;
                fl = fmaf(fl, corr, e);
                fm = m_new;
                const float inv_norm = RED == RED_L2 ? lp_inv(acc, a.p) : 0.f;
#pragma unroll
                for (int it = 0; it < IT; ++it)
#pragma unroll
                    for (int v = 0; v < VEC; ++v) {
                        float dsdq;
                        if (RED == RED_DOT) dsdq = ev[u][it][v];
                        else if (RED == RED_L1) dsdq = -sgnf(qv[it][v] - ev[u][it][v]);
                        else dsdq = -lp_dterm(qv[it][v] - ev[u][it][v], a.p) * inv_norm;
                        facc[it][v] = fmaf(facc[it][v], corr, p * dsdq);
                    }
            }
        }
    }
    if (FUSE) {
        float m_all = fmaxf(fm, __shfl_xor(fm, 16, 64));
        m_all = fmaxf(m_all, __shfl_xor(m_all, 32, 64));
        const float sc = (fm == -INFINITY) ? 0.f : expf(fm - m_all);
        float l = fl * sc;
        l += __shfl_xor(l, 16, 64);
        l += __shfl_xor(l, 32, 64);
        const int64_t slot = q * a.items_per_query + (item - q * a.items_per_query);
        if (lane == 0) {
            f.st_ml[slot * 2 + 0] = m_all;
            f.st_ml[slot * 2 + 1] = l;
        }
        float* ap = f.st_acc + slot * a.W;
#pragma unroll
        for (int it = 0; it < IT; ++it) {
            const int c = g + 16 * it;
#pragma unroll
            for (int v = 0; v < VEC; ++v) {
                float x = facc[it][v] * sc;
                x += __shfl_xor(x, 16, 64);
                x += __shfl_xor(x, 32, 64);
                if (sub == 0 && c < a.nch) ap[c * VEC + v] = x;
            }
        }
    }
}

constexpr int SW_NB = 1024;
constexpr int SW_PMAX = 8192;
constexpr int SW_PPT = SW_PMAX / 256;
constexpr int SW_SHARE = SW_PMAX / 8;
constexpr int SW_QFLOATS = 16384;
constexpr int64_t SW_REUSE_MIN = 4;

struct SweepArgs {
    int qb;
    int kc;
    int n_kchunks;
    int shift;
    int qstride;
};

template <typename T, int VEC, int IT, int RED, int UNROLL>
__global__ __launch_bounds__(256) void k_neg_pertriple_fwd_sweep(NegPtArgs a, SweepArgs s, float* __restrict__ out,
                                                                 int64_t ld_out) {
    extern __shared__ __attribute__((aligned(16))) float qs[];
    __shared__ int hist[SW_NB + 4];
    __shared__ int2 ent[SW_SHARE];
    __shared__ int rk[2][SW_PPT * 4];
    __shared__ int wsum[4];
    __shared__ int cut[4];

    const int tid = threadIdx.x;
    const int lane = tid & 63;
    const int wave = tid >> 6;
    const int label = blockIdx.x & 7;
    const int bc = blockIdx.x >> 3;
    const int qblk = bc / s.n_kchunks;
    const int kch = bc - qblk * s.n_kchunks;
    const int64_t q0 = static_cast<int64_t>(qblk) * s.qb;
    const int nqb = static_cast<int>(min(static_cast<int64_t>(s.qb), a.n_query - q0));
    const int kc0 = kch * s.kc;
    const int kcn = min(s.kc, a.n_neg - kc0);
    const int P = nqb * kcn;
    const int lo = static_cast<int>((static_cast<int64_t>(label) * P) >> 3);
    const int hi = static_cast<int>((static_cast<int64_t>(label + 1) * P) >> 3);

    for (int i = tid; i < nqb * IT * 16; i += 256) {
        const int qi = i / (IT * 16);
        const int c = i - qi * (IT * 16);
        float v[VEC];
        load_chunk<float, VEC>(a.query + (q0 + qi) * a.W, c, a.nch, v);
#pragma unroll
        for (int j = 0; j < VEC; ++j) qs[qi * s.qstride + c * VEC + j] = v[j];
    }
    for (int b = tid; b < SW_NB; b += 256) hist[b] = 0;
    if (tid < 2) cut[tid] = -1;
    int rr[SW_PPT];
#pragma unroll
    for (int j = 0; j < SW_PPT; ++j) {
        const int p = tid + 256 * j;
        rr[j] = 0;
        if (p < P) {
            const int qi = p / kcn;
            rr[j] = a.idx[(q0 + qi) * a.n_neg + kc0 + (p - qi * kcn)];
        }
    }
    __syncthreads();
#pragma unroll
    for (int j = 0; j < SW_PPT; ++j)
        if (tid + 256 * j < P) atomicAdd(&hist[min(static_cast<unsigned>(rr[j]) >> s.shift, SW_NB - 1u)], 1);
    __syncthreads();

    {
        int c[4], sum = 0;
#pragma unroll
        for (int i = 0; i < 4; ++i) {
            c[i] = hist[4 * tid + i];
            sum += c[i];
        }
        int incl = sum;
#pragma unroll
        for (int off = 1; off < 64; off <<= 1) {
            const int y = __shfl_up(incl, off, 64);
            if (lane >= off) incl += y;
        }
        if (lane == 63) wsum[wave] = incl;
        __syncthreads();
        int run = incl - sum;
        for (int w = 0; w < wave; ++w) run += wsum[w];
#pragma unroll
        for (int i = 0; i < 4; ++i) {
            const int b = 4 * tid + i;
            hist[b] = run;
            if (run < lo && lo < run + c[i]) cut[0] = b;
            if (run < hi && hi < run + c[i]) cut[1] = b;
            run += c[i];
        }
        if (tid == 255) hist[SW_NB] = run;
    }
    __syncthreads();

    const int cut0 = cut[0], cut1 = cut[1];
    const uint64_t lt = (1ull << lane) - 1ull;
#pragma unroll
    for (int j = 0; j < SW_PPT; ++j) {
        const bool live = tid + 256 * j < P;
        const unsigned b = min(static_cast<unsigned>(rr[j]) >> s.shift, SW_NB - 1u);
        const uint64_t m0 = __ballot(live && static_cast<int>(b) == cut0);
        const uint64_t m1 = __ballot(live && static_cast<int>(b) == cut1);
        if (lane == 0) {
            rk[0][j * 4 + wave] = __popcll(m0);
            rk[1][j * 4 + wave] = __popcll(m1);
        }
    }
    __syncthreads();
    if (wave == 0) {
#pragma unroll
        for (int h = 0; h < 2; ++h) {
            const int x0 = rk[h][2 * lane], x1 = rk[h][2 * lane + 1];
            int incl = x0 + x1;
#pragma unroll
            for (int off = 1; off < 64; off <<= 1) {
                const int y = __shfl_up(incl, off, 64);
                if (lane >= off) incl += y;
            }
            rk[h][2 * lane] = incl - x0 - x1;
            rk[h][2 * lane + 1] = incl - x1;
        }
    }
    __syncthreads();

    int slot[SW_PPT];
#pragma unroll
    for (int j = 0; j < SW_PPT; ++j) {
        const bool live = tid + 256 * j < P;
        const unsigned b = min(static_cast<unsigned>(rr[j]) >> s.shift, SW_NB - 1u);
        const bool in0 = live && static_cast<int>(b) == cut0;
        const bool in1 = live && static_cast<int>(b) == cut1 && !in0;
        const uint64_t m0 = __ballot(in0);
        const uint64_t m1 = __ballot(in1);
        const int b0 = live ? hist[b] : 0, b1 = live ? hist[b + 1] : 0;
        slot[j] = -1;
        if (live) {
            if (in0 || in1) {
                const int r = in0 ? rk[0][j * 4 + wave] + __popcll(m0 & lt) : rk[1][j * 4 + wave] + __popcll(m1 & lt);
                const int pos = b0 + r;
                if (pos >= lo && pos < hi) slot[j] = pos - lo;
            } else if (b0 >= lo && b1 <= hi) {
                slot[j] = -2;
            }
        }
    }
    __syncthreads();
#pragma unroll
    for (int j = 0; j < SW_PPT; ++j) {
        const int p = tid + 256 * j;
        if (slot[j] == -1) continue;
        const unsigned b = min(static_cast<unsigned>(rr[j]) >> s.shift, SW_NB - 1u);
        const int e = slot[j] >= 0 ? slot[j] : atomicAdd(&hist[b], 1) - lo;
        const int qi = p / kcn;
        ent[e] = make_int2(rr[j], (qi << 16) | (p - qi * kcn));
    }
    __syncthreads();

    const int n = hi - lo;
    const int g = lane & 15;
    const int sub = lane >> 4;
    const T* base = static_cast<const T*>(a.base);
    int2 nx[UNROLL];
#pragma unroll
    for (int u = 0; u < UNROLL; ++u) nx[u] = ent[max(0, min(wave * 4 * UNROLL + sub + 4 * u, n - 1))];
    for (int e0 = wave * 4 * UNROLL; e0 < n; e0 += 16 * UNROLL) {
        float ev[UNROLL][IT][VEC];
        int2 cur[UNROLL];
        bool valid[UNROLL];
#pragma unroll
        for (int u = 0; u < UNROLL; ++u) {
            const int e = e0 + sub + 4 * u;
            valid[u] = e < n;
            cur[u] = nx[u];
            const T* rp = base + static_cast<int64_t>(cur[u].x) * a.W;
            nx[u] = ent[min(e + 16 * UNROLL, n - 1)];
#pragma unroll
            for (int it = 0; it < IT; ++it) load_chunk<T, VEC>(rp, g + 16 * it, a.nch, ev[u][it]);
        }
#pragma unroll
        for (int u = 0; u < UNROLL; ++u) {
            const int qi = cur[u].y >> 16;
            const int kk = cur[u].y & 0xffff;
            const float* qp = qs + qi * s.qstride;
            float acc = 0.f;
#pragma unroll
            for (int it = 0; it < IT; ++it) {
                float qv[VEC];
                VecLoad<float, VEC>::load(qp + (g + 16 * it) * VEC, qv);
#pragma unroll
                for (int v = 0; v < VEC; ++v) {
                    if (RED == RED_DOT) {
                        acc = fmaf(qv[v], ev[u][it][v], acc);
                    } else if (RED == RED_L1) {
                        acc += fabsf(qv[v] - ev[u][it][v]);
                    } else {
                        acc += lp_term(qv[v] - ev[u][it][v], a.p);
                    }
                }
            }
            acc = row16_allreduce_sum(acc);
            if (RED == RED_L2) acc = lp_root(acc, a.p);
            if (g == 0 && valid[u]) out[(q0 + qi) * ld_out + kc0 + kk] = a.sign * acc;
        }
    }
}

__global__ __launch_bounds__(256) void k_combine_dq(const float* __restrict__ st_ml, const float* __restrict__ st_acc,
                                                    int64_t n_query, int items, int W, int kind, float loss_scale,
                                                    const float* __restrict__ pos, const float* __restrict__ weight,
                                                    int64_t weight_len, const float* __restrict__ norm,
                                                    float* __restrict__ d_query) {
    const int64_t q = blockIdx.x * 4ll + (threadIdx.x >> 6);
    if (q >= n_query) return;
    combine_dq_row(st_ml, st_acc, q, items, W, kind, loss_scale, pos, weight, weight_len, norm, d_query + q * W, nullptr);
}

template <typename T, int VEC, int IT, int RED, int UNROLL>
__global__ __launch_bounds__(256) void k_neg_pertriple_bwd(NegPtArgs a,
                                                           const float* __restrict__ d_out,
                                                           int64_t ld_dout,
                                                           float* __restrict__ d_query,
                                                           float* __restrict__ d_neg) {
    const int lane = threadIdx.x & 63;
    const int g = lane & 15;
    const int sub = lane >> 4;
    const int64_t item = blockIdx.x * 4ll + (threadIdx.x >> 6);
    if (item >= a.n_query * a.items_per_query) return;
    const int64_t q = item / a.items_per_query;
    const int k0 = static_cast<int>(item - q * a.items_per_query) * a.nb;
    const int k1 = min(k0 + a.nb, a.n_neg);

    float qv[IT][VEC], dq[IT][VEC];
    const float* qp = a.query + q * a.W;
#pragma unroll
    for (int it = 0; it < IT; ++it) {
#pragma unroll
        for (int v = 0; v < VEC; ++v) dq[it][v] = 0.f;
        load_chunk<float, VEC>(qp, g + 16 * it, a.nch, qv[it]);
    }
    const T* base = static_cast<const T*>(a.base);
    const int32_t* idx = a.idx + q * a.n_neg;
    const float* grow = d_out + q * ld_dout;

    int32_t nrow[UNROLL];
    float ngo[UNROLL];
#pragma unroll
    for (int u = 0; u < UNROLL; ++u) {
        const int kk = min(k0 + sub + 4 * u, k1 - 1);
        nrow[u] = idx[kk];
        ngo[u] = grow[kk];
    }
    const bool need_rows = !(RED == RED_DOT && d_query == nullptr);
    for (int kb = k0; kb < k1; kb += 4 * UNROLL) {
        float ev[UNROLL][IT][VEC], go[UNROLL];
        int ks[UNROLL];
        int32_t row_now[UNROLL];
        bool valid[UNROLL];
#pragma unroll
        for (int u = 0; u < UNROLL; ++u) {
            const int k = kb + sub + 4 * u;
            valid[u] = k < k1;
            ks[u] = min(k, k1 - 1);
            const T* rp = base + static_cast<int64_t>(nrow[u]) * a.W;
            row_now[u] = nrow[u];
            go[u] = valid[u] ? a.sign * ngo[u] : 0.f;
            const int kn = min(k + 4 * UNROLL, k1 - 1);
            nrow[u] = idx[kn];
            ngo[u] = grow[kn];
            if (need_rows) {
#pragma unroll
                for (int it = 0; it < IT; ++it) load_chunk<T, VEC>(rp, g + 16 * it, a.nch, ev[u][it]);
            } else {
#pragma unroll
                for (int it = 0; it < IT; ++it)
#pragma unroll
                    for (int v = 0; v < VEC; ++v) ev[u][it][v] = 0.f;
            }
        }
#pragma unroll
        for (int u = 0; u < UNROLL; ++u) {
            float gg = go[u];
            if (RED == RED_L2) {
                float ss = 0.f;
#pragma unroll
                for (int it = 0; it < IT; ++it)
#pragma unroll
                    for (int v = 0; v < VEC; ++v) {
                        ss += lp_term(qv[it][v] - ev[u][it][v], a.p);
                    }
                ss = row16_allreduce_sum(ss);
                gg *= lp_inv(lp_root(ss, a.p), a.p);
            }
            float* dn = d_neg + (a.dn_by_row ? static_cast<int64_t>(row_now[u]) : q * a.n_neg + ks[u]) * a.W;
#pragma unroll
            for (int it = 0; it < IT; ++it) {
                const int c = g + 16 * it;
                float de[VEC];
#pragma unroll
                for (int v = 0; v < VEC; ++v) {
                    float dqe;
                    if (RED == RED_DOT) {
                        dqe = gg * ev[u][it][v];
                        de[v] = gg * qv[it][v];
                    } else if (RED == RED_L1) {
                        dqe = gg * sgnf(qv[it][v] - ev[u][it][v]);
                        de[v] = -dqe;
                    } else {
                        dqe = gg * lp_dterm(qv[it][v] - ev[u][it][v], a.p);
                        de[v] = -dqe;
                    }
                    dq[it][v] += dqe;
                }
                if (d_neg && valid[u] && c < a.nch) {
                    if constexpr (VEC == 4) {
                        typedef float f4 __attribute__((ext_vector_type(4)));
#pragma unroll
                        for (int v = 0; v < VEC; v += 4) {
                            f4 o = {de[v], de[v + 1], de[v + 2], de[v + 3]};
                            __builtin_nontemporal_store(o, reinterpret_cast<f4*>(dn + c * VEC + v));
                        }
                    } else {
#pragma unroll
                        for (int v = 0; v < VEC; ++v) dn[c * VEC + v] = de[v];
                    }
                }
            }
        }
    }
    if (!d_query) return;
    float* dqp = d_query + q * a.W;
#pragma unroll
    for (int it = 0; it < IT; ++it) {
        const int c = g + 16 * it;
#pragma unroll
        for (int v = 0; v < VEC; ++v) {
            float x = dq[it][v];
            x += __shfl_xor(x, 16, 64);
            x += __shfl_xor(x, 32, 64);
            if (sub == 0 && c < a.nch) {
                if (a.items_per_query == 1) dqp[c * VEC + v] = x;
                else unsafeAtomicAdd(dqp + c * VEC + v, x);
            }
        }
    }
}

template <typename T, int VEC, int IT, int RED>
static void launch_fwd(const NegPtArgs& a, float* out, int64_t ld, const FuseArgs* fuse, hipStream_t st) {
    const int64_t items = a.n_query * a.items_per_query;
    constexpr int EPL = IT * VEC;
    constexpr int UNROLL = EPL <= 16 ? 4 : (EPL <= 32 ? 2 : 1);
    if (!fuse && a.sweep_shift >= 0) {
        SweepArgs s;
        s.qstride = IT * 16 * VEC;
        s.qb = SW_QFLOATS / s.qstride < 32 ? SW_QFLOATS / s.qstride : 32;
        s.kc = a.n_neg < SW_PMAX / s.qb ? a.n_neg : SW_PMAX / s.qb;
        s.n_kchunks = static_cast<int>(ceil_div(a.n_neg, s.kc));
        s.shift = a.sweep_shift;
        const int64_t blocks = ceil_div(a.n_query, s.qb) * s.n_kchunks * 8;
        const int lds = s.qb * s.qstride * static_cast<int>(sizeof(float));
        k_neg_pertriple_fwd_sweep<T, VEC, IT, RED, UNROLL>
            <<<static_cast<unsigned>(blocks), 256, lds, st>>>(a, s, out, ld);
    } else if (fuse) {
        constexpr int FU = EPL <= 16 ? 2 : 1;
        k_neg_pertriple_fwd<T, VEC, IT, RED, FU, true><<<ceil_div(items, 4), 256, 0, st>>>(a, out, ld, *fuse);
    } else {
        k_neg_pertriple_fwd<T, VEC, IT, RED, UNROLL, false><<<ceil_div(items, 4), 256, 0, st>>>(a, out, ld, FuseArgs{});
    }
}
template <typename T, int VEC, int IT, int RED>
static void launch_bwd(const NegPtArgs& a, const float* d_out, int64_t ld, float* dq, float* dn,
                       hipStream_t st) {
    const int64_t items = a.n_query * a.items_per_query;
    constexpr int EPL = IT * VEC;
    constexpr int BU = EPL <= 16 ? 2 : 1;
    k_neg_pertriple_bwd<T, VEC, IT, RED, BU><<<ceil_div(items, 4), 256, 0, st>>>(a, d_out, ld, dq, dn);
}

template <typename T, int VEC, int IT>
static void by_red(int red, bool fwd, const NegPtArgs& a, float* out, const float* d_out, int64_t ld,
                   float* dq, float* dn, const FuseArgs* fuse, hipStream_t st) {
    switch (red) {
        case RED_DOT:
            fwd ? launch_fwd<T, VEC, IT, RED_DOT>(a, out, ld, fuse, st)
                : launch_bwd<T, VEC, IT, RED_DOT>(a, d_out, ld, dq, dn, st);
            break;
        case RED_L1:
            fwd ? launch_fwd<T, VEC, IT, RED_L1>(a, out, ld, fuse, st)
                : launch_bwd<T, VEC, IT, RED_L1>(a, d_out, ld, dq, dn, st);
            break;
        default:
            fwd ? launch_fwd<T, VEC, IT, RED_L2>(a, out, ld, fuse, st)
                : launch_bwd<T, VEC, IT, RED_L2>(a, d_out, ld, dq, dn, st);
    }
}

template <typename T, int VEC>
static int by_it(int it, int red, bool fwd, const NegPtArgs& a, float* out, const float* d_out,
                 int64_t ld, float* dq, float* dn, const FuseArgs* fuse, hipStream_t st) {
    if (it <= 1) by_red<T, VEC, 1>(red, fwd, a, out, d_out, ld, dq, dn, fuse, st);
    else if (it <= 2) by_red<T, VEC, 2>(red, fwd, a, out, d_out, ld, dq, dn, fuse, st);
    else if (it <= 4) by_red<T, VEC, 4>(red, fwd, a, out, d_out, ld, dq, dn, fuse, st);
    else if (it <= 8) by_red<T, VEC, 8>(red, fwd, a, out, d_out, ld, dq, dn, fuse, st);
    else if (it <= 16) by_red<T, VEC, 16>(red, fwd, a, out, d_out, ld, dq, dn, fuse, st);
    else return fail(BESS_EUNSUPPORTED, "neg_score_pertriple: row of %d scalars too wide", a.W);
    return BESS_OK;
}

static int negatives_per_item(int64_t n_query, int64_t n_neg, int64_t row_bytes) {
    int nb = 64;
    while (nb < 256 && nb * row_bytes < 131072) nb <<= 1;
    while (nb > 8 && n_query * ceil_div(n_neg, nb) < 256 * 16 * 2) nb >>= 1;
    return nb;
}

static int vec_of(const bess_model_desc* d) {
    const int maxvec = d->dtype == BESS_F32 ? 4 : 8;
    if (d->width % maxvec == 0) return maxvec;
    return (d->dtype == BESS_F16 && d->width % 2 == 0) ? 2 : 1;
}

static int sweep_shift_for(const bess_model_desc* d, int64_t n_query, int64_t n_neg) {
    if (d->scorer > BESS_COMPLEX || d->width > 16 * 16 * vec_of(d)) return -1;
    const int64_t rows = d->reserved[1];
    if (rows <= 0 || n_query <= 0 || n_neg <= 0 || n_query * n_neg < SW_REUSE_MIN * rows) return -1;
    if (ceil_div(n_query, 8) * ceil_div(n_neg, 256) * 8 >= (1ll << 31)) return -1;
    int shift = 0;
    while (((rows - 1) >> shift) >= SW_NB) ++shift;
    return shift;
}

static int run(const bess_model_desc* d, bool fwd, const float* query, int64_t n_query,
               const void* neg_base, const int32_t* neg_idx, int64_t n_neg, float* out,
               const float* d_out, int64_t ld, float* dq, float* dn, void* stream,
               const FuseArgs* fuse = nullptr) {
    if (int e = check_desc(d)) return e;
    BESS_REQUIRE(n_query >= 0 && n_neg >= 0 && n_neg < (1ll << 31), "neg_score_pertriple: bad sizes");
    if (n_query == 0 || n_neg == 0) return BESS_OK;
    BESS_REQUIRE(query && neg_base && neg_idx, "neg_score_pertriple: NULL pointer");
    BESS_REQUIRE(ld >= n_neg, "neg_score_pertriple: leading dimension %lld < n_neg %lld", (long long)ld,
                 (long long)n_neg);
    if (d->scorer == BESS_BOXE)
        return boxe_negatives(d, fwd, false, query, n_query, neg_base, neg_idx, n_neg, out, d_out, ld, dq, dn,
                              as_stream(stream));
    if (d->scorer == BESS_AFFINE)
        return affine_pertriple(d, fwd, query, n_query, neg_base, neg_idx, n_neg, out, d_out, ld, dq, dn,
                                as_stream(stream));
    const int W = d->width;
    const int vec = vec_of(d);
    NegPtArgs a;
    a.query = query;
    a.base = neg_base;
    a.idx = neg_idx;
    a.n_query = n_query;
    a.n_neg = static_cast<int>(n_neg);
    a.W = W;
    a.nch = W / vec;
    a.nb = negatives_per_item(n_query, n_neg, static_cast<int64_t>(W) * (d->dtype == BESS_F32 ? 4 : 2));
    a.items_per_query = static_cast<int>(ceil_div(n_neg, a.nb));
    a.sign = is_distance(d->scorer) ? -1.f : 1.f;
    a.p = static_cast<float>(d->norm_p);
    a.dn_by_row = (!fwd && (d->reserved[0] & BESS_FLAG_DNEG_BY_ROW)) ? 1 : 0;
    if (fwd && !fuse) a.sweep_shift = sweep_shift_for(d, n_query, n_neg);
    const int red = reduce_of(d);
    hipStream_t st = as_stream(stream);
    if (!fwd && a.items_per_query > 1 && dq) {
        hipError_t e = fill_words_async(dq, 0u, n_query * W, st);
        if (e != hipSuccess) return fail(static_cast<int>(e), "memset d_query: %s", hipGetErrorString(e));
    }
    const int max_cols = 16 * 16 * vec;
    if (W > max_cols) {
        if (red == RED_L2)
            return fail(BESS_EUNSUPPORTED, "neg_score_pertriple: p = 2 on rows of %d scalars (more than %d)", W, max_cols);
        if (fuse)
            return fail(BESS_EUNSUPPORTED, "neg_score_pertriple: fused training forward on rows of %d scalars (more than %d)",
                        W, max_cols);
    }
    const int64_t sz = d->dtype == BESS_F32 ? 4 : 2;
    for (int col0 = 0; col0 < W; col0 += max_cols) {
        const int cols = W - col0 < max_cols ? W - col0 : max_cols;
        NegPtArgs w = a;
        w.query = query + col0;
        w.base = static_cast<const char*>(neg_base) + col0 * sz;
        w.nch = cols / vec;
        w.accum = col0 > 0;
        const int it = static_cast<int>(ceil_div(w.nch, 16));
        float* dqw = dq ? dq + col0 : nullptr;
        float* dnw = dn ? dn + col0 : nullptr;
        int rc = BESS_OK;
        if (d->dtype == BESS_F32) {
            if (vec == 4) rc = by_it<float, 4>(it, red, fwd, w, out, d_out, ld, dqw, dnw, fuse, st);
            else rc = by_it<float, 1>(it, red, fwd, w, out, d_out, ld, dqw, dnw, fuse, st);
        } else {
            if (vec == 8) rc = by_it<half_t, 8>(it, red, fwd, w, out, d_out, ld, dqw, dnw, fuse, st);
            else if (vec == 2) rc = by_it<half_t, 2>(it, red, fwd, w, out, d_out, ld, dqw, dnw, fuse, st);
            else rc = by_it<half_t, 1>(it, red, fwd, w, out, d_out, ld, dqw, dnw, fuse, st);
        }
        if (rc) return rc;
    }
    return check_launch(fwd ? "neg_score_pertriple_fwd" : "neg_score_pertriple_bwd");
}

}

extern "C" int bess_neg_score_pertriple_fwd(const bess_model_desc* d, const float* query,
                                            int64_t n_query, const void* neg_base,
                                            const int32_t* neg_idx, int64_t n_neg, float* out,
                                            int64_t ld_out, void* stream) {
    if (n_query > 0 && n_neg > 0 && !out) return bess::fail(BESS_EINVAL, "neg_score_pertriple_fwd: NULL out");
    return bess::run(d, true, query, n_query, neg_base, neg_idx, n_neg, out, nullptr, ld_out, nullptr,
                     nullptr, stream);
}

extern "C" int bess_neg_score_pertriple_bwd(const bess_model_desc* d, const float* query,
                                            int64_t n_query, const void* neg_base,
                                            const int32_t* neg_idx, int64_t n_neg,
                                            const float* d_out, int64_t ld_dout, float* d_query,
                                            float* d_neg, void* stream) {
    if (n_query > 0 && n_neg > 0 && !(d_out && (d_query || d_neg)))
        return bess::fail(BESS_EINVAL, "neg_score_pertriple_bwd: NULL pointer");
    return bess::run(d, false, query, n_query, neg_base, neg_idx, n_neg, nullptr, d_out, ld_dout,
                     d_query, d_neg, stream);
}

extern "C" int bess_neg_pertriple_sweep(const bess_model_desc* d, int64_t n_query, int64_t n_neg, int32_t* sweep) {
    if (int e = bess::check_desc(d)) return e;
    if (!sweep || n_query < 0 || n_neg < 0) return bess::fail(BESS_EINVAL, "neg_pertriple_sweep: bad argument");
    *sweep = bess::sweep_shift_for(d, n_query, n_neg) >= 0 ? 1 : 0;
    return BESS_OK;
}

static int64_t row_bytes_of(const bess_model_desc* d) {
    return static_cast<int64_t>(d->width) * (d->dtype == BESS_F32 ? 4 : 2);
}

extern "C" int bess_neg_pertriple_items(const bess_model_desc* d, int64_t n_query, int64_t n_neg, int32_t* items) {
    if (!d || !items || n_query < 0 || n_neg < 0) return bess::fail(BESS_EINVAL, "neg_pertriple_items: bad argument");
    *items = n_neg > 0 ? static_cast<int32_t>(bess::ceil_div(n_neg, bess::negatives_per_item(n_query, n_neg, row_bytes_of(d))))
                       : 0;
    return BESS_OK;
}

extern "C" int bess_neg_score_pertriple_fwd_dq(const bess_model_desc* d, const bess_loss_desc* l, const float* query,
                                               int64_t n_query, const void* neg_base, const int32_t* neg_idx,
                                               int64_t n_neg, const float* pos, const float* weight,
                                               int64_t weight_len, float* out, int64_t ld_out, float* d_query,
                                               float* state_ml, float* state_acc, void* stream) {
    return bess_neg_score_pertriple_fwd_dq_masked(d, l, query, n_query, neg_base, neg_idx, n_neg, pos, weight, weight_len,
                                                  nullptr, 0, 0, out, ld_out, d_query, state_ml, state_acc, stream);
}

extern "C" int bess_neg_score_pertriple_fwd_dq_masked(const bess_model_desc* d, const bess_loss_desc* l,
                                                      const float* query, int64_t n_query, const void* neg_base,
                                                      const int32_t* neg_idx, int64_t n_neg, const float* pos,
                                                      const float* weight, int64_t weight_len, const uint8_t* mask,
                                                      int64_t mask_rows, int64_t mask_cols, float* out,
                                                      int64_t ld_out, float* d_query, float* state_ml,
                                                      float* state_acc, void* stream) {
    using namespace bess;
    if (int e = check_desc(d)) return e;
    BESS_REQUIRE(l, "neg_score_pertriple_fwd_dq: NULL loss descriptor");
    BESS_REQUIRE(d->scorer <= BESS_COMPLEX, "neg_score_pertriple_fwd_dq: scorer %d has no fused form", d->scorer);
    BESS_REQUIRE(l->kind == BESS_LOSS_LOGSIGMOID || l->kind == BESS_LOSS_MARGIN || l->kind == BESS_LOSS_SSCE,
                 "neg_score_pertriple_fwd_dq: unknown loss %d", l->kind);
    if (n_query <= 0 || n_neg <= 0) return BESS_OK;
    BESS_REQUIRE(out && state_ml && state_acc && weight && (weight_len == 1 || weight_len == n_query),
                 "neg_score_pertriple_fwd_dq: NULL pointer or bad weight length");
    BESS_REQUIRE(pos || l->kind == BESS_LOSS_LOGSIGMOID, "neg_score_pertriple_fwd_dq: this loss needs the positive scores");
    FuseArgs f;
    f.pos = pos;
    f.kind = l->kind;
    f.beta = l->kind == BESS_LOSS_SSCE ? 1.f : (l->adversarial ? l->adversarial_scale : 0.f);
    f.margin = l->margin;
    f.shift = l->kind == BESS_LOSS_SSCE ? l->ssce_shift : 0.f;
    f.st_ml = state_ml;
    f.st_acc = state_acc;
    if (mask) {
        BESS_REQUIRE(mask_cols > 0 && mask_cols <= n_neg && (mask_rows == 1 || mask_rows == n_query),
                     "neg_score_pertriple_fwd_dq_masked: mask [%lld, %lld] for %lld queries x %lld negatives",
                     (long long)mask_rows, (long long)mask_cols, (long long)n_query, (long long)n_neg);
        f.mask = mask;
        f.mask_rows = mask_rows;
        f.mask_cols = static_cast<int>(mask_cols);
        f.mask_from = static_cast<int>(n_neg - mask_cols);
    }
    const int rc = run(d, true, query, n_query, neg_base, neg_idx, n_neg, out, nullptr, ld_out, nullptr, nullptr, stream,
                       &f);
    if (rc) return rc;
    const int items = static_cast<int>(ceil_div(n_neg, negatives_per_item(n_query, n_neg, row_bytes_of(d))));
    if (!d_query) return BESS_OK;
    k_combine_dq<<<static_cast<unsigned>(ceil_div(n_query, 4)), 256, 0, as_stream(stream)>>>(
        state_ml, state_acc, n_query, items, d->width, l->kind, l->loss_scale, pos, weight, weight_len, nullptr, d_query);
    return check_launch("neg_score_pertriple_fwd_dq");
}

extern "C" int bess_neg_score_pertriple_fwd_partials(const bess_model_desc* d, const bess_loss_desc* l,
                                                     const float* query, int64_t n_query, const void* neg_base,
                                                     const int32_t* neg_idx, int64_t n_neg, float* out,
                                                     int64_t ld_out, float* state_ml, float* state_acc, void* stream) {
    using namespace bess;
    if (int e = check_desc(d)) return e;
    BESS_REQUIRE(l, "neg_score_pertriple_fwd_partials: NULL loss descriptor");
    BESS_REQUIRE(d->scorer <= BESS_COMPLEX, "neg_score_pertriple_fwd_partials: scorer %d has no fused form", d->scorer);
    if (l->kind != BESS_LOSS_LOGSIGMOID && l->kind != BESS_LOSS_SSCE)
        return fail(BESS_EUNSUPPORTED, "neg_score_pertriple_fwd_partials: loss %d weighs a negative by the positive score, "
                                       "which the scoring shard does not have", l->kind);
    if (n_query <= 0 || n_neg <= 0) return BESS_OK;
    BESS_REQUIRE(out && state_ml && state_acc, "neg_score_pertriple_fwd_partials: NULL pointer");
    FuseArgs f;
    f.pos = nullptr;
    f.kind = l->kind;
    f.beta = l->kind == BESS_LOSS_SSCE ? 1.f : (l->adversarial ? l->adversarial_scale : 0.f);
    f.margin = l->margin;
    f.shift = l->kind == BESS_LOSS_SSCE ? l->ssce_shift : 0.f;
    f.st_ml = state_ml;
    f.st_acc = state_acc;
    return run(d, true, query, n_query, neg_base, neg_idx, n_neg, out, nullptr, ld_out, nullptr, nullptr, stream, &f);
}

extern "C" int bess_combine_dq_partials(const float* state_ml, const float* state_acc, int64_t n_query, int32_t items,
                                        int32_t width, const float* norm, float* d_query, void* stream) {
    using namespace bess;
    BESS_REQUIRE(n_query >= 0 && items > 0 && width > 0, "combine_dq_partials: bad sizes");
    if (n_query == 0) return BESS_OK;
    BESS_REQUIRE(state_ml && state_acc && norm && d_query, "combine_dq_partials: NULL pointer");
    k_combine_dq<<<static_cast<unsigned>(ceil_div(n_query, 4)), 256, 0, as_stream(stream)>>>(
        state_ml, state_acc, n_query, items, width, 0, 1.f, nullptr, nullptr, 1, norm, d_query);
    return check_launch("combine_dq_partials");
}
```

bess-kge_amd/csrc/plan.hip:

```cpp
#include <string.h>

#include <string>
#include <type_traits>
#include <utility>
#include <vector>

#include "common.h"

namespace bess {

union Slot {
    int64_t i;
    double d;
    void* p;
};

constexpr int PLAN_MAX_ARGS = 32;

template <typename T>
static T slot_get(const Slot& s) {
    if constexpr (std::is_pointer_v<T>) return reinterpret_cast<T>(s.p);
    else if constexpr (std::is_floating_point_v<T>) return static_cast<T>(s.d);
    else return static_cast<T>(s.i);
}
template <typename... A, size_t... I>
static int invoke(int (*f)(A...), const Slot* s, std::index_sequence<I...>) {
    return f(slot_get<A>(s[I])...);
}
template <typename... A>
static int invoke(int (*f)(A...), const Slot* s) {
    return invoke(f, s, std::index_sequence_for<A...>{});
}
template <typename... A>
static constexpr int arity(int (*)(A...)) {
    return static_cast<int>(sizeof...(A));
}

struct PlanFn {
    const char* name;
    int n_args;
    int (*thunk)(const Slot*);
};

#define BESS_PLAN_FN(fn) \
    PlanFn { #fn, arity(&fn), [](const Slot* s) -> int { return invoke(&fn, s); } }
static const PlanFn PLAN_FNS[] = {
    BESS_PLAN_FN(bess_gather_rows),
    BESS_PLAN_FN(bess_score_triple_fwd),
    BESS_PLAN_FN(bess_score_triple_bwd),
    BESS_PLAN_FN(bess_query_fwd),
    BESS_PLAN_FN(bess_query_bwd),
    BESS_PLAN_FN(bess_query_triple_fwd),
    BESS_PLAN_FN(bess_query_triple_fwd_jobs),
    BESS_PLAN_FN(bess_query_triple_bwd),
    BESS_PLAN_FN(bess_query_triple_bwd_parts),
    BESS_PLAN_FN(bess_neg_score_pertriple_fwd),
    BESS_PLAN_FN(bess_neg_score_pertriple_bwd),
    BESS_PLAN_FN(bess_neg_score_pertriple_fwd_dq),
    BESS_PLAN_FN(bess_neg_score_pertriple_fwd_dq_masked),
    BESS_PLAN_FN(bess_neg_score_pertriple_fwd_partials),
    BESS_PLAN_FN(bess_combine_dq_partials),
    BESS_PLAN_FN(bess_pertriple_tail),
    BESS_PLAN_FN(bess_neg_score_shared_fwd),
    BESS_PLAN_FN(bess_neg_score_shared_fwd_ws),
    BESS_PLAN_FN(bess_neg_score_shared_fwd_masked),
    BESS_PLAN_FN(bess_neg_score_shared_fwd_loss),
    BESS_PLAN_FN(bess_neg_score_shared_fwd_pruned),
    BESS_PLAN_FN(bess_neg_score_shared_fwd_counts),
    BESS_PLAN_FN(bess_neg_score_shared_fwd_pairs),
    BESS_PLAN_FN(bess_neg_score_table_fwd_counts),
    BESS_PLAN_FN(bess_neg_score_table_fwd_pairs),
    BESS_PLAN_FN(bess_neg_score_shared_bwd),
    BESS_PLAN_FN(bess_neg_score_shared_bwd_ws),
    BESS_PLAN_FN(bess_neg_score_shared_bwd_parts),
    BESS_PLAN_FN(bess_mask_scores),
    BESS_PLAN_FN(bess_loss_fwd_bwd),
    BESS_PLAN_FN(bess_loss_fwd_bwd_norm),
    BESS_PLAN_FN(bess_loss_fwd_bwd_one_launch),
    BESS_PLAN_FN(bess_topk_update),
    BESS_PLAN_FN(bess_topk_update_flagged),
    BESS_PLAN_FN(bess_topk_update_excl),
    BESS_PLAN_FN(bess_topk_update_flagged_excl),
    BESS_PLAN_FN(bess_ranks_from_scores),
    BESS_PLAN_FN(bess_ranks_from_indices),
    BESS_PLAN_FN(bess_scatter_add_rows),
    BESS_PLAN_FN(bess_sparse_sgd),
    BESS_PLAN_FN(bess_sparse_sgd_lists),
    BESS_PLAN_FN(bess_sparse_sgd_lists_axpy),
    BESS_PLAN_FN(bess_dense_sgd),
    BESS_PLAN_FN(bess_build_segment_index),
    BESS_PLAN_FN(bess_pad_segments),
    BESS_PLAN_FN(bess_step_prologue),
    BESS_PLAN_FN(bess_neg_pertriple_grad_segments),
    BESS_PLAN_FN(bess_neg_pertriple_step_segments),
    BESS_PLAN_FN(bess_apply_segments_sgd),
    BESS_PLAN_FN(bess_apply_segments_opt),
    BESS_PLAN_FN(bess_segment_sum_rows),
    BESS_PLAN_FN(bess_coalesced_update),
    BESS_PLAN_FN(bess_coalesced_update_axpy),
    BESS_PLAN_FN(bess_direct_update),
    BESS_PLAN_FN(bess_assign_state_rows),
    BESS_PLAN_FN(bess_map_extra_rows),
    BESS_PLAN_FN(bess_normalize_rows),
    BESS_PLAN_FN(bess_normalize_rows_bwd),
    BESS_PLAN_FN(bess_sample_negatives),
    BESS_PLAN_FN(bess_sample_bucket_indices),
    BESS_PLAN_FN(bess_lookup_triples),
    BESS_PLAN_FN(bess_gather_candidate_lists),
    BESS_PLAN_FN(bess_alltoall),
    BESS_PLAN_FN(bess_allgather),
    BESS_PLAN_FN(bess_allreduce_sum_f32),
    BESS_PLAN_FN(bess_pack_exchange),
};
#undef BESS_PLAN_FN

static const PlanFn* find_fn(const char* name) {
    for (const PlanFn& f : PLAN_FNS)
        if (strcmp(f.name, name) == 0) return &f;
    return nullptr;
}

struct PlanCall {
    const PlanFn* fn;
    uint8_t kind[PLAN_MAX_ARGS];
    Slot value[PLAN_MAX_ARGS];
};

}

struct bess_plan {
    std::vector<bess::PlanCall> calls;
    std::vector<char> arena;
};

using namespace bess;

extern "C" int bess_plan_create(bess_plan** plan) {
    BESS_REQUIRE(plan, "plan_create: NULL result pointer");
    *plan = new bess_plan();
    return BESS_OK;
}

extern "C" int bess_plan_destroy(bess_plan* plan) {
    delete plan;
    return BESS_OK;
}

extern "C" int bess_plan_knows(const char* name) { return name && find_fn(name) ? 1 : 0; }

extern "C" int bess_plan_length(const bess_plan* plan) { return plan ? static_cast<int>(plan->calls.size()) : 0; }

extern "C" int bess_plan_add_call(bess_plan* plan, const char* name, int32_t n_args, const uint8_t* kinds,
                                  const uint64_t* values, const void* const* blobs, const int64_t* blob_bytes) {
    BESS_REQUIRE(plan && name && (n_args == 0 || (kinds && values)), "plan_add_call: NULL pointer");
    const PlanFn* fn = find_fn(name);
    BESS_REQUIRE(fn, "plan_add_call: `%s` is not an entry point that enqueues work", name);
    BESS_REQUIRE(n_args == fn->n_args && n_args <= PLAN_MAX_ARGS, "plan_add_call: %s takes %d arguments, got %d", name,
                 fn->n_args, n_args);
    PlanCall c{};
    c.fn = fn;
    for (int k = 0; k < n_args; ++k) {
        c.kind[k] = kinds[k];
        switch (kinds[k]) {
            case BESS_PLAN_ARG_INT: c.value[k].i = static_cast<int64_t>(values[k]); break;
            case BESS_PLAN_ARG_FLOAT: memcpy(&c.value[k].d, &values[k], sizeof(double)); break;
            case BESS_PLAN_ARG_PTR: c.value[k].p = reinterpret_cast<void*>(static_cast<uintptr_t>(values[k])); break;
            case BESS_PLAN_ARG_STREAM: c.value[k].p = nullptr; break;
            case BESS_PLAN_ARG_BLOB: {
                BESS_REQUIRE(blobs && blob_bytes && blobs[k] && blob_bytes[k] > 0, "plan_add_call: %s argument %d: empty blob",
                             name, k);
                const size_t at = (plan->arena.size() + 15) & ~size_t(15);
                plan->arena.resize(at + static_cast<size_t>(blob_bytes[k]));
                memcpy(plan->arena.data() + at, blobs[k], static_cast<size_t>(blob_bytes[k]));
                c.value[k].i = static_cast<int64_t>(at);
                break;
            }
            default: return fail(BESS_EINVAL, "plan_add_call: %s argument %d: unknown kind %d", name, k, kinds[k]);
        }
    }
    BESS_REQUIRE(n_args > 0 && kinds[n_args - 1] == BESS_PLAN_ARG_STREAM, "plan_add_call: the last argument of %s is its stream",
                 name);
    plan->calls.push_back(c);
    return BESS_OK;
}

extern "C" int bess_plan_run(const bess_plan* plan, void* stream) {
    BESS_REQUIRE(plan, "plan_run: NULL plan");
    const char* base = plan->arena.data();
    for (const PlanCall& c : plan->calls) {
        Slot s[PLAN_MAX_ARGS];
        for (int k = 0; k < c.fn->n_args; ++k) {
            s[k] = c.value[k];
            if (c.kind[k] == BESS_PLAN_ARG_BLOB) s[k].p = const_cast<char*>(base) + c.value[k].i;
            else if (c.kind[k] == BESS_PLAN_ARG_STREAM) s[k].p = stream;
        }
        if (int rc = c.fn->thunk(s)) return rc;
    }
    return BESS_OK;
}
```

bess-kge_amd/csrc/prepare.hip:

```cpp
#include "common.h"
#include "loss_rows.h"

namespace bess {

struct TripleArgs {
    const void* head_base;
    const int32_t* head_idx;
    const void* tail_base;
    const int32_t* tail_idx;
    const void* rel_table;
    const int32_t* rel_idx;
    int64_t n;
    int W;
    int Wr;
    int norm_p;
};

template <typename T, int SCORER>
__device__ __forceinline__ void triple_fwd_body(const TripleArgs& a, int64_t s, int lane, float* __restrict__ out) {
    const T* h = row_ptr(static_cast<const T*>(a.head_base), a.head_idx, s, a.W);
    const T* t = row_ptr(static_cast<const T*>(a.tail_base), a.tail_idx, s, a.W);
    const T* r = static_cast<const T*>(a.rel_table) + static_cast<int64_t>(a.rel_idx[s]) * a.Wr;
    float acc = 0.f;
    if (SCORER == BESS_TRANSE) {
        for (int e = lane; e < a.W; e += 64) {
            const float x = to_f32(h[e]) + to_f32(r[e]) - to_f32(t[e]);
            acc += (a.norm_p == 1) ? fabsf(x) : lp_term(x, static_cast<float>(a.norm_p));
        }
    } else if (SCORER == BESS_DISTMULT) {
        for (int e = lane; e < a.W; e += 64) acc += to_f32(h[e]) * to_f32(r[e]) * to_f32(t[e]);
    } else {
        const int d = a.W / 2;
        for (int e = lane; e < d; e += 64) {
            const float hr = to_f32(h[e]), hi = to_f32(h[d + e]);
            const float tr = to_f32(t[e]), ti = to_f32(t[d + e]);
            float rr, ri;
            if (SCORER == BESS_ROTATE) {
                const float ph = to_f32(r[e]);
                rr = cosf(ph);
                ri = sinf(ph);
            } else {
                rr = to_f32(r[e]);
                ri = to_f32(r[d + e]);
            }
            const float qr = hr * rr - hi * ri;
            const float qi = hr * ri + hi * rr;
            if (SCORER == BESS_ROTATE) {
                const float xr = qr - tr, xi = qi - ti;
                acc += (a.norm_p == 1) ? (fabsf(xr) + fabsf(xi))
                                       : (lp_term(xr, static_cast<float>(a.norm_p)) + lp_term(xi, static_cast<float>(a.norm_p)));
            } else {
                acc += qr * tr + qi * ti;
            }
        }
    }
    acc = wave_allreduce_sum(acc);
    if (SCORER == BESS_TRANSE || SCORER == BESS_ROTATE)
        acc = -((a.norm_p == 1) ? acc : lp_root(acc, static_cast<float>(a.norm_p)));
    if (lane == 0) out[s] = acc;
}

template <typename T, int SCORER>
__global__ __launch_bounds__(256) void k_score_triple_fwd(TripleArgs a, float* __restrict__ out) {
    const int lane = threadIdx.x & 63;
    const int64_t s = blockIdx.x * 4ll + (threadIdx.x >> 6);
    if (s >= a.n) return;
    triple_fwd_body<T, SCORER>(a, s, lane, out);
}

struct QueryArgs {
    const void* ent_base;
    const int32_t* ent_idx;
    const void* rel_table;
    const int32_t* rel_idx;
    int64_t n;
    int W;
    int Wr;
    int side;
};

template <typename T, int SCORER>
__device__ __forceinline__ void query_fwd_body(const QueryArgs& a, int64_t q, int lane, float* __restrict__ query) {
    const T* x = row_ptr(static_cast<const T*>(a.ent_base), a.ent_idx, q, a.W);
    const T* r = static_cast<const T*>(a.rel_table) + static_cast<int64_t>(a.rel_idx[q]) * a.Wr;
    float* o = query + q * a.W;
    const bool tail = a.side == BESS_CORRUPT_TAIL;
    if (SCORER == BESS_TRANSE) {
        for (int e = lane; e < a.W; e += 64)
            o[e] = tail ? (to_f32(x[e]) + to_f32(r[e])) : (to_f32(x[e]) - to_f32(r[e]));
    } else if (SCORER == BESS_DISTMULT) {
        for (int e = lane; e < a.W; e += 64) o[e] = to_f32(x[e]) * to_f32(r[e]);
    } else {
        const int d = a.W / 2;
        for (int e = lane; e < d; e += 64) {
            const float xr = to_f32(x[e]), xi = to_f32(x[d + e]);
            float rr, ri;
            if (SCORER == BESS_ROTATE) {
                const float ph = tail ? to_f32(r[e]) : -to_f32(r[e]);
                rr = cosf(ph);
                ri = sinf(ph);
            } else {
                rr = to_f32(r[e]);
                ri = tail ? to_f32(r[d + e]) : -to_f32(r[d + e]);
            }
            o[e] = xr * rr - xi * ri;
            o[d + e] = xr * ri + xi * rr;
        }
    }
}

template <typename T, int SCORER>
__global__ __launch_bounds__(256) void k_query_fwd(QueryArgs a, float* __restrict__ query) {
    const int lane = threadIdx.x & 63;
    const int64_t q = blockIdx.x * 4ll + (threadIdx.x >> 6);
    if (q >= a.n) return;
    query_fwd_body<T, SCORER>(a, q, lane, query);
}

template <typename T, int SCORER>
__global__ __launch_bounds__(256) void k_query_triple_fwd(TripleArgs a, QueryArgs qa, float* __restrict__ query,
                                                          float* __restrict__ out) {
    const int lane = threadIdx.x & 63;
    const int64_t s = blockIdx.x * 4ll + (threadIdx.x >> 6);
    if (s >= a.n) return;
    query_fwd_body<T, SCORER>(qa, s, lane, query);
    triple_fwd_body<T, SCORER>(a, s, lane, out);
}

template <typename T, int SCORER>
__global__ __launch_bounds__(256) void k_query_triple_fwd_jobs(TripleArgs a, QueryArgs qa, float* __restrict__ query,
                                                               float* __restrict__ out, WordJobs J, int triple_blocks) {
    if (static_cast<int>(blockIdx.x) >= triple_blocks) {
        run_word_jobs(J, static_cast<int>(blockIdx.x) - triple_blocks, static_cast<int>(gridDim.x) - triple_blocks, 256);
        return;
    }
    const int lane = threadIdx.x & 63;
    const int64_t s = blockIdx.x * 4ll + (threadIdx.x >> 6);
    if (s >= a.n) return;
    query_fwd_body<T, SCORER>(qa, s, lane, query);
    triple_fwd_body<T, SCORER>(a, s, lane, out);
}

template <bool ACCUM>
__device__ __forceinline__ void put(float* p, float v) {
    if (ACCUM) *p += v;
    else *p = v;
}
template <bool BYROW>
__device__ __forceinline__ void emit(float* p, float v) {
    if (BYROW) {
        if (v != 0.f) unsafeAtomicAdd(p, v);
    } else {
        *p = v;
    }
}
template <bool BYROW, bool ACCUM>
__device__ __forceinline__ void emit2(float* p, float v) {
    if (BYROW) {
        if (v != 0.f) unsafeAtomicAdd(p, v);
    } else {
        put<ACCUM>(p, v);
    }
}

template <typename T, int SCORER, bool BYROW = false>
__device__ __forceinline__ void triple_bwd_body(const TripleArgs& a, int64_t s, int lane,
                                                const float g, float* __restrict__ d_head,
                                                float* __restrict__ d_tail, float* __restrict__ d_rel) {
    const T* h = row_ptr(static_cast<const T*>(a.head_base), a.head_idx, s, a.W);
    const T* t = row_ptr(static_cast<const T*>(a.tail_base), a.tail_idx, s, a.W);
    const int64_t rid = a.rel_idx[s];
    const T* r = static_cast<const T*>(a.rel_table) + rid * a.Wr;
    float* dh = d_head + (BYROW ? (a.head_idx ? static_cast<int64_t>(a.head_idx[s]) : s) : s) * a.W;
    float* dt = d_tail + (BYROW ? (a.tail_idx ? static_cast<int64_t>(a.tail_idx[s]) : s) : s) * a.W;
    float* dr = d_rel + rid * a.Wr;

    if (SCORER == BESS_TRANSE) {
        float inv = 0.f;
        const float pf = static_cast<float>(a.norm_p);
        if (a.norm_p != 1) {
            float ss = 0.f;
            for (int e = lane; e < a.W; e += 64) {
                const float x = to_f32(h[e]) + to_f32(r[e]) - to_f32(t[e]);
                ss += lp_term(x, pf);
            }
            ss = wave_allreduce_sum(ss);
            inv = lp_inv(lp_root(ss, pf), pf);
        }
        for (int e = lane; e < a.W; e += 64) {
            const float x = to_f32(h[e]) + to_f32(r[e]) - to_f32(t[e]);
            const float dx = -g * ((a.norm_p == 1) ? sgnf(x) : lp_dterm(x, pf) * inv);
            emit<BYROW>(dh + e, dx);
            emit<BYROW>(dt + e, -dx);
            if (dx != 0.f) unsafeAtomicAdd(dr + e, dx);
        }
    } else if (SCORER == BESS_DISTMULT) {
        for (int e = lane; e < a.W; e += 64) {
            const float hv = to_f32(h[e]), rv = to_f32(r[e]), tv = to_f32(t[e]);
            emit<BYROW>(dh + e, g * rv * tv);
            emit<BYROW>(dt + e, g * hv * rv);
            unsafeAtomicAdd(dr + e, g * hv * tv);
        }
    } else {
        const int d = a.W / 2;
        float inv = 0.f;
        const float pf = static_cast<float>(a.norm_p);
        if (SCORER == BESS_ROTATE && a.norm_p != 1) {
            float ss = 0.f;
            for (int e = lane; e < d; e += 64) {
                const float hr = to_f32(h[e]), hi = to_f32(h[d + e]);
                const float ph = to_f32(r[e]);
                const float c = cosf(ph), sn = sinf(ph);
                const float xr = hr * c - hi * sn - to_f32(t[e]);
                const float xi = hr * sn + hi * c - to_f32(t[d + e]);
                ss += lp_term(xr, pf) + lp_term(xi, pf);
            }
            ss = wave_allreduce_sum(ss);
            inv = lp_inv(lp_root(ss, pf), pf);
        }
        for (int e = lane; e < d; e += 64) {
            const float hr = to_f32(h[e]), hi = to_f32(h[d + e]);
            const float tr = to_f32(t[e]), ti = to_f32(t[d + e]);
            if (SCORER == BESS_ROTATE) {
                const float ph = to_f32(r[e]);
                const float c = cosf(ph), sn = sinf(ph);
                const float xr = hr * c - hi * sn - tr;
                const float xi = hr * sn + hi * c - ti;
                const float dxr = -g * ((a.norm_p == 1) ? sgnf(xr) : lp_dterm(xr, pf) * inv);
                const float dxi = -g * ((a.norm_p == 1) ? sgnf(xi) : lp_dterm(xi, pf) * inv);
                emit<BYROW>(dh + e, dxr * c + dxi * sn);
                emit<BYROW>(dh + d + e, -dxr * sn + dxi * c);
                emit<BYROW>(dt + e, -dxr);
                emit<BYROW>(dt + d + e, -dxi);
                const float dph = dxr * (-hr * sn - hi * c) + dxi * (hr * c - hi * sn);
                if (dph != 0.f) unsafeAtomicAdd(dr + e, dph);
            } else {
                const float rr = to_f32(r[e]), ri = to_f32(r[d + e]);
                emit<BYROW>(dh + e, g * (rr * tr + ri * ti));
                emit<BYROW>(dh + d + e, g * (-ri * tr + rr * ti));
                emit<BYROW>(dt + e, g * (hr * rr - hi * ri));
                emit<BYROW>(dt + d + e, g * (hr * ri + hi * rr));
                unsafeAtomicAdd(dr + e, g * (hr * tr + hi * ti));
                unsafeAtomicAdd(dr + d + e, g * (-hi * tr + hr * ti));
            }
        }
    }
}

template <typename T, int SCORER>
__global__ __launch_bounds__(256) void k_score_triple_bwd(TripleArgs a,
                                                          const float* __restrict__ d_out,
                                                          float* __restrict__ d_head,
                                                          float* __restrict__ d_tail,
                                                          float* __restrict__ d_rel) {
    const int lane = threadIdx.x & 63;
    const int64_t s = blockIdx.x * 4ll + (threadIdx.x >> 6);
    if (s >= a.n) return;
    triple_bwd_body<T, SCORER>(a, s, lane, d_out[s], d_head, d_tail, d_rel);
}

template <typename T, int SCORER, bool ACCUM, bool BYROW = false>
// ... 590 lines not shown
```

include/besskge_hip.h:

```cpp
#ifndef BESSKGE_HIP_H
#define BESSKGE_HIP_H

#include <stddef.h>
#include <stdint.h>

#ifdef __cplusplus
extern "C" {
#endif

#define BESS_ABI_VERSION 3

#define BESS_OK 0
#define BESS_EINVAL -1
#define BESS_EUNSUPPORTED -2
#define BESS_ECOMM_BASE 10000

#define BESS_TRANSE 0
#define BESS_ROTATE 1
#define BESS_DISTMULT 2
#define BESS_COMPLEX 3
#define BESS_AFFINE 4
#define BESS_BOXE 5

#define BESS_F32 0
#define BESS_F16 1

#define BESS_CORRUPT_HEAD 0
#define BESS_CORRUPT_TAIL 1

#define BESS_LOSS_LOGSIGMOID 0
#define BESS_LOSS_MARGIN 1
#define BESS_LOSS_SSCE 2

#define BESS_MAX_ROW_LISTS 8

#define BESS_BAD_NEGATIVE_SCORE (-50000.0f)

#define BESS_FLAG_PREZEROED 2
#define BESS_FLAG_DNEG_BY_ROW 4
#define BESS_FLAG_FP32_MATH 1

typedef struct bess_model_desc {
    int32_t scorer;
    int32_t norm_p;
    int32_t dtype;
    int32_t width;
    int32_t rel_width;
    int32_t reserved[3];
} bess_model_desc;

#define BESS_OPT_SGD 0
#define BESS_OPT_ADAGRAD 1
#define BESS_OPT_ADAM 2

typedef struct bess_opt_desc {
    int32_t kind;
    int32_t step;
    float lr;
    float momentum;
    float beta1;
    float beta2;
    float eps;
    float weight_decay;
    int64_t step_ptr;
    int64_t slot_map;
} bess_opt_desc;

typedef struct bess_loss_desc {
    int32_t kind;
    int32_t adversarial;
    float margin;
    float adversarial_scale;
    float loss_scale;
    float ssce_shift;
    int32_t reserved[2];
} bess_loss_desc;

typedef struct bess_pcg64_state {
    uint64_t state_hi, state_lo;
    uint64_t inc_hi, inc_lo;
    uint32_t has_uint32;
    uint32_t uinteger;
} bess_pcg64_state;

int bess_version(void);
int bess_last_error(char* buf, size_t len);

int bess_gather_rows(int32_t dtype, int32_t width, const void* table,
                     const int32_t* idx, int64_t n, void* out, void* stream);

int bess_score_triple_fwd(const bess_model_desc* d, const void* head_base,
                          const int32_t* head_idx, const void* tail_base,
                          const int32_t* tail_idx, const void* rel_table,
                          const int32_t* rel_idx, int64_t n_triple, float* out,
                          void* stream);

int bess_score_triple_bwd(const bess_model_desc* d, const void* head_base,
                          const int32_t* head_idx, const void* tail_base,
                          const int32_t* tail_idx, const void* rel_table,
                          const int32_t* rel_idx, int64_t n_triple,
                          const float* d_out, float* d_head, float* d_tail,
                          float* d_rel_table, void* stream);

int bess_query_fwd(const bess_model_desc* d, int32_t side, const void* ent_base,
                   const int32_t* ent_idx, const void* rel_table,
                   const int32_t* rel_idx, int64_t n_query, float* query,
                   void* stream);

int bess_query_bwd(const bess_model_desc* d, int32_t side, const void* ent_base,
                   const int32_t* ent_idx, const void* rel_table,
                   const int32_t* rel_idx, int64_t n_query, const float* d_query,
                   float* d_ent, float* d_rel_table, void* stream);

int bess_query_triple_fwd(const bess_model_desc* d, int32_t side, const void* head_base,
                          const int32_t* head_idx, const void* tail_base, const int32_t* tail_idx,
                          const void* rel_table, const int32_t* rel_idx, int64_t n_triple,
                          float* query, float* out, void* stream);
int bess_query_triple_bwd(const bess_model_desc* d, int32_t side, const void* head_base,
                          const int32_t* head_idx, const void* tail_base, const int32_t* tail_idx,
                          const void* rel_table, const int32_t* rel_idx, int64_t n_triple,
                          const float* d_out, const float* d_query, float* d_head, float* d_tail,
                          float* d_rel_table, void* stream);

int bess_neg_score_pertriple_fwd(const bess_model_desc* d, const float* query,
                                 int64_t n_query, const void* neg_base,
                                 const int32_t* neg_idx, int64_t n_neg, float* out,
                                 int64_t ld_out, void* stream);
int bess_neg_pertriple_sweep(const bess_model_desc* d, int64_t n_query, int64_t n_neg, int32_t* sweep);

int bess_neg_score_pertriple_bwd(const bess_model_desc* d, const float* query,
                                 int64_t n_query, const void* neg_base,
                                 const int32_t* neg_idx, int64_t n_neg,
                                 const float* d_out, int64_t ld_dout,
                                 float* d_query, float* d_neg, void* stream);

int bess_neg_score_shared_fwd(const bess_model_desc* d, const float* query,
                              int64_t n_query, const void* neg_base,
                              const int32_t* neg_idx, int64_t n_neg, float* out,
                              int64_t ld_out, void* stream);


typedef struct bess_kill_desc {
    int32_t diag_step;
    int32_t ht;
    int32_t ppp;
    int32_t reserved;
    const uint8_t* mask;
    int64_t mask_rows;
    int64_t mask_cols;
} bess_kill_desc;
int bess_neg_score_shared_fwd_masked(const bess_model_desc* d, const float* query,
                                     int64_t n_query, const void* neg_base,
                                     const int32_t* neg_idx, int64_t n_neg, float* out,
                                     int64_t ld_out, const bess_kill_desc* kill, void* workspace,
                                     int64_t workspace_bytes, void* stream);

int64_t bess_neg_score_shared_workspace(const bess_model_desc* d, int64_t n_query, int64_t n_neg);
int bess_neg_score_shared_fwd_ws(const bess_model_desc* d, const float* query,
                                 int64_t n_query, const void* neg_base,
                                 const int32_t* neg_idx, int64_t n_neg, float* out,
                                 int64_t ld_out, void* workspace, int64_t workspace_bytes,
                                 void* stream);

int bess_neg_score_shared_bwd(const bess_model_desc* d, const float* query,
                              int64_t n_query, const void* neg_base,
                              const int32_t* neg_idx, int64_t n_neg,
                              const float* out, int64_t ld_out, const float* d_out,
                              int64_t ld_dout, float* d_query, float* d_neg,
                              void* stream);

int bess_neg_score_shared_fwd_pruned(const bess_model_desc* d, const float* query, int64_t n_query,
                                     const void* neg_base, const int32_t* neg_idx, int64_t n_neg, float* out,
                                     int64_t ld_out, const float* thr, uint8_t* flags, int64_t ld_flags,
                                     void* workspace, int64_t workspace_bytes, void* stream);

int64_t bess_neg_score_shared_fwd_counts_workspace(const bess_model_desc* d, int64_t n_query, int64_t n_neg);
int bess_neg_score_shared_fwd_counts(const bess_model_desc* d, const float* query, int64_t n_query,
                                     const void* neg_base, const int32_t* neg_idx, int64_t n_neg, const float* thr,
                                     const int32_t* excl, int32_t* counts, int32_t round_f16, void* workspace,
                                     int64_t workspace_bytes, void* stream);

int64_t bess_neg_score_shared_fwd_pairs_workspace(const bess_model_desc* d, int64_t like_n_query, int64_t like_n_neg);
int bess_neg_score_shared_fwd_pairs(const bess_model_desc* d, const float* query, const void* neg_base,
                                    const int32_t* neg_idx, int64_t n_pair, int64_t like_n_query, int64_t like_n_neg,
                                    float* out, void* workspace, int64_t workspace_bytes, void* stream);

#define BESS_AFFINE_COUNT_CHUNK_BYTES (32ll << 20)
int64_t bess_neg_score_table_fwd_counts_workspace(const bess_model_desc* d, int64_t n_query, int64_t n_neg);
int bess_neg_score_table_fwd_counts(const bess_model_desc* d, const float* query, int64_t n_query,
                                    const void* neg_base, const int32_t* neg_idx, int64_t n_neg, const float* thr,
                                    const int32_t* excl, int32_t* counts, int32_t round_f16, void* workspace,
                                    int64_t workspace_bytes, void* stream);
int64_t bess_neg_score_table_fwd_pairs_workspace(const bess_model_desc* d, int64_t like_n_query, int64_t like_n_neg);
int bess_neg_score_table_fwd_pairs(const bess_model_desc* d, const float* query, const void* neg_base,
                                   const int32_t* neg_idx, int64_t n_pair, int64_t like_n_query, int64_t like_n_neg,
                                   float* out, void* workspace, int64_t workspace_bytes, void* stream);

int64_t bess_neg_score_shared_bwd_workspace(const bess_model_desc* d, int64_t n_query, int64_t n_neg);
int bess_neg_score_shared_bwd_ws(const bess_model_desc* d, const float* query,
                                 int64_t n_query, const void* neg_base,
                                 const int32_t* neg_idx, int64_t n_neg, const float* out,
                                 int64_t ld_out, const float* d_out, int64_t ld_dout,
                                 float* d_query, float* d_neg, void* workspace,
                                 int64_t workspace_bytes, void* stream);

int bess_mask_scores(float* neg, int64_t n_triple, int64_t n_neg, int64_t ld,
                     int32_t diag_step, int32_t ht, int32_t ppp,
                     const uint8_t* mask, int64_t mask_rows, int64_t mask_cols,
                     void* stream);

int bess_loss_fwd_bwd(const bess_loss_desc* l, const float* pos, const float* neg,
                      int64_t n_triple, int64_t n_neg, int64_t ld_neg,
                      const float* weight, int64_t weight_len, float* row_loss,
                      float* loss, float* d_pos, float* d_neg, int64_t ld_dneg,
                      void* stream);

int bess_loss_fwd_bwd_norm(const bess_loss_desc* l, const float* pos, const float* neg,
                           int64_t n_triple, int64_t n_neg, int64_t ld_neg,
                           const float* weight, int64_t weight_len, float* row_loss,
                           float* loss, float* d_pos, float* d_neg, int64_t ld_dneg,
                           float* row_norm, void* stream);

#define BESS_TICKET_INTS 544
int bess_loss_fwd_bwd_one_launch(const bess_loss_desc* l, const float* pos, const float* neg,
                                 int64_t n_triple, int64_t n_neg, int64_t ld_neg,
                                 const float* weight, int64_t weight_len, float* row_loss,
                                 float* loss, float* d_pos, float* d_neg, int64_t ld_dneg,
                                 float* row_norm, int32_t* counter, void* stream);

int bess_topk_update(const float* scores, int64_t n_row, int64_t n_col, int64_t ld,
                     const int32_t* ids, int64_t ids_rows, int32_t id_base,
                     const uint8_t* mask, int64_t mask_rows, float* best_score,
                     int32_t* best_id, int32_t kk, void* stream);

int bess_topk_update_flagged(const float* scores, int64_t n_row, int64_t n_col, int64_t ld,
                             const uint8_t* flags, int64_t ld_flags, int32_t id_base, float* best_score,
                             int32_t* best_id, int32_t kk, void* stream);

int bess_topk_update_excl(const float* scores, int64_t n_row, int64_t n_col, int64_t ld,
                          const int32_t* ids, int64_t ids_rows, int32_t id_base,
                          const uint8_t* mask, int64_t mask_rows, const int32_t* excl_ptr,
                          const int32_t* excl_ids, int64_t n_excl, int32_t round_f16, float* best_score,
                          int32_t* best_id, int32_t kk, void* stream);
int bess_topk_update_flagged_excl(const float* scores, int64_t n_row, int64_t n_col, int64_t ld,
                                  const uint8_t* flags, int64_t ld_flags, const int32_t* ids, int32_t id_base,
                                  const int32_t* excl_ptr, const int32_t* excl_ids, int64_t n_excl,
                                  int32_t round_f16, float* best_score, int32_t* best_id, int32_t kk,
                                  void* stream);

int bess_ranks_from_scores(const float* pos, const float* cand, int64_t n_row,
                           int64_t n_cand, int64_t ld, int32_t mode,
                           int32_t worst_rank_infty, float* rank, void* stream);
int bess_ranks_from_indices(const int64_t* ground_truth, const int64_t* candidates,
                            int64_t n_row, int64_t n_cand, int32_t worst_rank_infty,
                            float* rank, void* stream);

int bess_scatter_add_rows(float* dst, int32_t width, const int32_t* idx,
                          const float* src, int64_t n, float scale, void* stream);

int bess_sparse_sgd(int32_t dtype, int32_t width, void* table, const int32_t* idx,
                    const float* grad, int64_t n, float lr, void* stream);

int bess_sparse_sgd_lists(int32_t dtype, int32_t width, void* table, int32_t n_lists,
                          const int32_t* const* list_idx, const float* const* list_grad,
                          const int64_t* list_rows, float lr, void* stream);
int bess_sparse_sgd_lists_axpy(int32_t dtype, int32_t width, void* table, int32_t n_lists,
                               const int32_t* const* list_idx, const float* const* list_grad,
                               const int64_t* list_rows, float lr, void* axpy_table, const float* axpy_grad,
                               int64_t axpy_n, float axpy_alpha, void* stream);

#define BESS_SEGMENT_CAP 256
#define BESS_MAX_WORD_JOBS 8
#define BESS_SMALL_INDEX_MAX 15360
int bess_segment_index_workspace(int64_t n_refs, size_t* bytes);
int bess_build_segment_index(const int32_t* idx, int64_t n_refs, int32_t row_bits,
                             int32_t* refs_sorted, int32_t* seg_rows,
                             int32_t* seg_offsets, int32_t* n_seg, int32_t* long_segs,
                             int64_t long_cap, void* workspace,
                             size_t workspace_bytes, void* stream);

int bess_pad_segments(int32_t* seg_rows, const int32_t* n_seg, int64_t max_seg, float* grad_seg, int32_t width,
// ... 197 lines not shown
```

Measured before the change: 5.152 billion triples/s.

## Fuse query construction and positive scoring into per-triple negative sweep kernel

Adds a fused forward path for score-only steps. The per-triple negative sweep kernel builds each query (head times relation) straight into shared memory and scores the positive triples in its tail, so the separate query_triple_fwd launch and the round-trip of the query tensor through global memory go away. Every k-chunk block now recomputes its queries from entity and relation rows, which duplicates gather work when there are several k-chunks. The loss reduction's final accumulation loop is also unrolled with batched loads.

Result: slower. 5.054 billion triples/s (-1.9%).

```diff
diff --git a/bess-kge_amd/besskge/_native.py b/bess-kge_amd/besskge/_native.py
--- a/bess-kge_amd/besskge/_native.py
+++ b/bess-kge_amd/besskge/_native.py
@@ -120,6 +120,8 @@
     "bess_sparse_sgd_lists_axpy": [_i32, _i32, _vp, _i32, ctypes.POINTER(_vp), ctypes.POINTER(_vp), ctypes.POINTER(_i64), _f32,
                                    _vp, _vp, _i64, _f32, _vp],
     "bess_neg_score_pertriple_fwd": [_MD, _vp, _i64, _vp, _vp, _i64, _vp, _i64, _vp],
+    "bess_neg_score_pertriple_fwd_triples": [_MD, _i32, _vp, _vp, _vp, _vp, _vp, _vp, _i64, _vp, _vp, _i64, _vp, _vp, _i64,
+                                             _vp],
     "bess_neg_score_pertriple_bwd": [_MD, _vp, _i64, _vp, _vp, _i64, _vp, _i64, _vp, _vp, _vp],
     "bess_neg_score_shared_fwd": [_MD, _vp, _i64, _vp, _vp, _i64, _vp, _i64, _vp],
     "bess_neg_score_shared_workspace": [_MD, _i64, _i64],
@@ -224,6 +226,7 @@
 _timed_names: frozenset = frozenset()
 
 TIMING_LABELS = {
+    "bess_neg_score_pertriple_fwd_triples": "bess_neg_score_pertriple_fwd",
     "bess_neg_score_pertriple_fwd_dq_masked": "bess_neg_score_pertriple_fwd_dq",
     "bess_neg_score_shared_fwd_ws": "bess_neg_score_shared_fwd",
     "bess_neg_score_shared_fwd_masked": "bess_neg_score_shared_fwd",
@@ -629,6 +632,33 @@
             out.data_ptr(), n_neg)
     del keep
     return out
+
+
+def neg_score_pertriple_fwd_triples(d: ModelDesc, side: int, head: RowSource, tail: RowSource, rel_table: torch.Tensor,
+                                    rel_idx: torch.Tensor, neg: RowSource, n_neg: int,
+                                    out: Optional[torch.Tensor] = None
+                                    ) -> Optional[Tuple[torch.Tensor, torch.Tensor]]:
+    dev, n = _triple_operands(d, head, tail, rel_table, rel_idx)
+    _same_device([("negative rows", neg.base), ("negative idx", neg.idx), ("head", head.base), ("out", out)])
+    _rows(neg.base, "negative rows", d.width)
+    if _dtype_code(neg.base) != d.dtype:
+        raise TypeError("negative rows dtype does not match the model descriptor")
+    if neg.idx is None or len(neg) != n * n_neg:
+        raise ValueError(f"expected {n * n_neg} indexed negative rows")
+    d = with_row_count(d, neg.base)
+    if d.scorer > COMPLEX or not pertriple_sweep(d, n, n_neg):
+        return None
+    if out is None:
+        out = torch.empty((n, n_neg), dtype=torch.float32, device=dev)
+    _f32(out, "out")
+    if out.dim() != 2 or out.shape[0] != n or out.shape[1] < n_neg:
+        raise ValueError("neg_score_pertriple_fwd_triples: bad `out` shape")
+    pos = torch.empty((n,), dtype=torch.float32, device=dev)
+    _launch("bess_neg_score_pertriple_fwd_triples", dev, ctypes.byref(d), side, head.base.data_ptr(),
+            _idx(head.idx, "head_idx"), tail.base.data_ptr(), _idx(tail.idx, "tail_idx"), rel_table.data_ptr(),
+            rel_idx.data_ptr(), n, neg.base.data_ptr(), _idx(neg.idx, "negative idx"), n_neg, pos.data_ptr(),
+            out.data_ptr(), int(out.shape[1]))
+    return out, pos
 
 
 def neg_score_pertriple_fwd_dq(d: ModelDesc, l: LossDesc, query: torch.Tensor, neg: RowSource, n_neg: int,
diff --git a/bess-kge_amd/besskge/bess.py b/bess-kge_amd/besskge/bess.py
--- a/bess-kge_amd/besskge/bess.py
+++ b/bess-kge_amd/besskge/bess.py
@@ -34,6 +34,9 @@
 
     def __init__(self, lr: float) -> None:
         self.lr = float(lr)
+
+
+fused_score_step = True
 
 
 class _NegGroup:
@@ -906,6 +909,17 @@
                 ahead = self._launch_prologue(st, self._ahead_optimizer, d_rel)
                 if ahead is not None:
                     early[id(st)] = ahead
+            scored = None
+            if (fused_score_step and st.fused_qt and fuse is None and early is None and not g0.shared
+                    and g0.neg.base is st.table and not self.__dict__.get("_train_loss_in_scoring_on")
+                    and not torch.is_grad_enabled()):
+                scored = fn.score_step_fwd(g0.side, RowSource(st.table, st.head_idx), st.tail, st.rel_idx, g0.neg,
+                                           g0.n_per_query)
+            if scored is not None:
+                g0.out, st.positive_score = scored
+                st.negative_score = g0.out
+                done.append(st)
+                continue
             if st.fused_qt:
                 g0.query, st.positive_score = fn.query_triple_fwd(g0.side, RowSource(st.table, st.head_idx), st.tail,
                                                                   st.rel_idx, jobs=st.jobs if st.jobs_ride else None)
diff --git a/bess-kge_amd/besskge/scoring.py b/bess-kge_amd/besskge/scoring.py
--- a/bess-kge_amd/besskge/scoring.py
+++ b/bess-kge_amd/besskge/scoring.py
@@ -72,6 +72,11 @@
                          jobs: Any = None) -> Tuple[torch.Tensor, torch.Tensor]:
         return nat.query_triple_fwd(self.kernel_desc(), side, head, tail, self.relation_embedding.data, rel_idx,
                                     jobs=jobs)
+
+    def score_step_fwd(self, side: int, head: nat.RowSource, tail: nat.RowSource, rel_idx: torch.Tensor,
+                       neg: nat.RowSource, n_neg: int) -> Optional[Tuple[torch.Tensor, torch.Tensor]]:
+        return nat.neg_score_pertriple_fwd_triples(self.kernel_desc(), side, head, tail, self.relation_embedding.data,
+                                                   rel_idx, neg, n_neg)
 
     def query_triple_bwd(self, side: int, head: nat.RowSource, tail: nat.RowSource, rel_idx: torch.Tensor,
                          d_pos: torch.Tensor, dq: torch.Tensor, d_rel: torch.Tensor
diff --git a/bess-kge_amd/csrc/loss.hip b/bess-kge_amd/csrc/loss.hip
--- a/bess-kge_amd/csrc/loss.hip
+++ b/bess-kge_amd/csrc/loss.hip
@@ -52,8 +52,15 @@
     if (threadIdx.x == 0) last = last_workgroup_ticket(counter);
     __syncthreads();
     if (!last) return;
+    constexpr int TB = 16;
     float acc = 0.f;
-    for (int64_t i = threadIdx.x; i < n_triple; i += 256) acc += load_agent(row_loss + i);
+    for (int64_t i0 = threadIdx.x; i0 < n_triple; i0 += 256 * TB) {
+        float v[TB];
+#pragma unroll
+        for (int j = 0; j < TB; ++j) v[j] = load_agent(row_loss + min(i0 + 256 * j, n_triple - 1));
+#pragma unroll
+        for (int j = 0; j < TB; ++j) acc = i0 + 256 * j < n_triple ? acc + v[j] : acc;
+    }
     part[threadIdx.x] = acc;
     __syncthreads();
     for (int h = 128; h > 0; h >>= 1) {
diff --git a/bess-kge_amd/csrc/neg_pertriple.hip b/bess-kge_amd/csrc/neg_pertriple.hip
--- a/bess-kge_amd/csrc/neg_pertriple.hip
+++ b/bess-kge_amd/csrc/neg_pertriple.hip
@@ -1,5 +1,6 @@
 #include "common.h"
 #include "loss_rows.h"
+#include "triple_rows.h"
 
 namespace bess {
 
@@ -176,9 +177,135 @@
     int qstride;
 };
 
-template <typename T, int VEC, int IT, int RED, int UNROLL>
+struct TripleStage {
+    TripleArgs t;
+    QueryArgs q;
+    float* pos;
+    int scorer;
+    int vec;
+};
+struct NoStage {};
+template <bool TRIPLES>
+struct StageOf {
+    typedef NoStage type;
+};
+template <>
+struct StageOf<true> {
+    typedef TripleStage type;
+};
+
+template <typename T, int VEC, int SCORER>
+__device__ __forceinline__ void stage_real(const QueryArgs& qa, bool vec, int64_t q0, int nqb, int qstride, float* qs, int tid) {
+    const T* eb = static_cast<const T*>(qa.ent_base);
+    const T* rt = static_cast<const T*>(qa.rel_table);
+    const bool tail = qa.side == BESS_CORRUPT_TAIL;
+    if (VEC > 1 && vec) {
+        const int nch = qa.W / VEC;
+#pragma unroll 2
+        for (int i = tid; i < nqb * nch; i += 256) {
+            const int qi = i / nch;
+            const int c = i - qi * nch;
+            const T* x = row_ptr(eb, qa.ent_idx, q0 + qi, qa.W) + c * VEC;
+            const T* r = rt + static_cast<int64_t>(qa.rel_idx[q0 + qi]) * qa.Wr + c * VEC;
+            float xv[VEC], rv[VEC];
+            VecLoad<T, VEC>::load(x, xv);
+            VecLoad<T, VEC>::load(r, rv);
+            float* o = qs + qi * qstride + c * VEC;
+#pragma unroll
+            for (int j = 0; j < VEC; ++j) o[j] = query_scalar<SCORER>(xv[j], rv[j], tail);
+        }
+    } else {
+#pragma unroll 2
+        for (int i = tid; i < nqb * qa.W; i += 256) {
+            const int qi = i / qa.W;
+            const int e = i - qi * qa.W;
+            const T* x = row_ptr(eb, qa.ent_idx, q0 + qi, qa.W);
+            const T* r = rt + static_cast<int64_t>(qa.rel_idx[q0 + qi]) * qa.Wr;
+            qs[qi * qstride + e] = query_scalar<SCORER>(to_f32(x[e]), to_f32(r[e]), tail);
+        }
+    }
+}
+
+template <typename T, int VEC, int SCORER>
+__device__ __forceinline__ void stage_cplx(const QueryArgs& qa, bool vec, int64_t q0, int nqb, int qstride, float* qs, int tid) {
+    const T* eb = static_cast<const T*>(qa.ent_base);
+    const T* rt = static_cast<const T*>(qa.rel_table);
+    const bool tail = qa.side == BESS_CORRUPT_TAIL;
+    const int d = qa.W / 2;
+    if (VEC > 1 && vec) {
+        const int hc = d / VEC;
+#pragma unroll 2
+        for (int i = tid; i < nqb * hc; i += 256) {
+            const int qi = i / hc;
+            const int c = i - qi * hc;
+            const T* x = row_ptr(eb, qa.ent_idx, q0 + qi, qa.W) + c * VEC;
+            const T* r = rt + static_cast<int64_t>(qa.rel_idx[q0 + qi]) * qa.Wr + c * VEC;
+            float xr[VEC], xi[VEC], r0[VEC], r1[VEC];
+            VecLoad<T, VEC>::load(x, xr);
+            VecLoad<T, VEC>::load(x + d, xi);
+            VecLoad<T, VEC>::load(r, r0);
+            if (SCORER == BESS_COMPLEX) {
+                VecLoad<T, VEC>::load(r + d, r1);
+            } else {
+#pragma unroll
+                for (int j = 0; j < VEC; ++j) r1[j] = 0.f;
+            }
+            float* o = qs + qi * qstride + c * VEC;
+#pragma unroll
+            for (int j = 0; j < VEC; ++j) {
+                float qr, qim;
+                query_pair<SCORER>(xr[j], xi[j], r0[j], r1[j], tail, qr, qim);
+                o[j] = qr;
+                o[d + j] = qim;
+            }
+        }
+    } else {
+#pragma unroll 2
+        for (int i = tid; i < nqb * d; i += 256) {
+            const int qi = i / d;
+            const int e = i - qi * d;
+            const T* x = row_ptr(eb, qa.ent_idx, q0 + qi, qa.W);
+            const T* r = rt + static_cast<int64_t>(qa.rel_idx[q0 + qi]) * qa.Wr;
+            const float r1 = SCORER == BESS_COMPLEX ? to_f32(r[d + e]) : 0.f;
+            float qr, qim;
+            query_pair<SCORER>(to_f32(x[e]), to_f32(x[d + e]), to_f32(r[e]), r1, tail, qr, qim);
+            qs[qi * qstride + e] = qr;
+            qs[qi * qstride + d + e] = qim;
+        }
+    }
+}
+
+template <typename T, int VEC, int RED>
+__device__ __forceinline__ void stage_queries(const TripleStage& ts, int64_t q0, int nqb, int qstride, float* qs, int tid) {
+    const int W = ts.q.W;
+    const int pad = qstride - W;
+    for (int i = tid; i < nqb * pad; i += 256) {
+        const int qi = i / pad;
+        qs[qi * qstride + W + (i - qi * pad)] = 0.f;
+    }
+    const bool vec = ts.vec != 0;
+    if (RED == RED_DOT) {
+        if (ts.scorer == BESS_DISTMULT) stage_real<T, VEC, BESS_DISTMULT>(ts.q, vec, q0, nqb, qstride, qs, tid);
+        else stage_cplx<T, VEC, BESS_COMPLEX>(ts.q, vec, q0, nqb, qstride, qs, tid);
+    } else {
+        if (ts.scorer == BESS_TRANSE) stage_real<T, VEC, BESS_TRANSE>(ts.q, vec, q0, nqb, qstride, qs, tid);
+        else stage_cplx<T, VEC, BESS_ROTATE>(ts.q, vec, q0, nqb, qstride, qs, tid);
+    }
+}
+template <typename T, int RED>
+__device__ __forceinline__ void stage_positive(const TripleStage& ts, int64_t s, int lane) {
+    if (RED == RED_DOT) {
+        if (ts.scorer == BESS_DISTMULT) triple_fwd_body<T, BESS_DISTMULT>(ts.t, s, lane, ts.pos);
+        else triple_fwd_body<T, BESS_COMPLEX>(ts.t, s, lane, ts.pos);
+    } else {
+        if (ts.scorer == BESS_TRANSE) triple_fwd_body<T, BESS_TRANSE>(ts.t, s, lane, ts.pos);
+        else triple_fwd_body<T, BESS_ROTATE>(ts.t, s, lane, ts.pos);
+    }
+}
+
+template <typename T, int VEC, int IT, int RED, int UNROLL, bool TRIPLES = false>
 __global__ __launch_bounds__(256) void k_neg_pertriple_fwd_sweep(NegPtArgs a, SweepArgs s, float* __restrict__ out,
-                                                                 int64_t ld_out) {
+                                                                 int64_t ld_out, typename StageOf<TRIPLES>::type ts) {
     extern __shared__ __attribute__((aligned(16))) float qs[];
     __shared__ int hist[SW_NB + 4];
     __shared__ int2 ent[SW_SHARE];
@@ -201,13 +328,17 @@
     const int lo = static_cast<int>((static_cast<int64_t>(label) * P) >> 3);
     const int hi = static_cast<int>((static_cast<int64_t>(label + 1) * P) >> 3);
 
-    for (int i = tid; i < nqb * IT * 16; i += 256) {
-        const int qi = i / (IT * 16);
-        const int c = i - qi * (IT * 16);
-        float v[VEC];
-        load_chunk<float, VEC>(a.query + (q0 + qi) * a.W, c, a.nch, v);
-#pragma unroll
-        for (int j = 0; j < VEC; ++j) qs[qi * s.qstride + c * VEC + j] = v[j];
+    if constexpr (TRIPLES) {
+        stage_queries<T, VEC, RED>(ts, q0, nqb, s.qstride, qs, tid);
+    } else {
+        for (int i = tid; i < nqb * IT * 16; i += 256) {
+            const int qi = i / (IT * 16);
+            const int c = i - qi * (IT * 16);
+            float v[VEC];
+            load_chunk<float, VEC>(a.query + (q0 + qi) * a.W, c, a.nch, v);
+#pragma unroll
+            for (int j = 0; j < VEC; ++j) qs[qi * s.qstride + c * VEC + j] = v[j];
+        }
     }
     for (int b = tid; b < SW_NB; b += 256) hist[b] = 0;
     if (tid < 2) cut[tid] = -1;
@@ -365,6 +496,10 @@
             if (RED == RED_L2) acc = lp_root(acc, a.p);
             if (g == 0 && valid[u]) out[(q0 + qi) * ld_out + kc0 + kk] = a.sign * acc;
         }
+    }
+    if constexpr (TRIPLES) {
+        if (kch == 0)
+            for (int j = 4 * label + wave; j < nqb; j += 32) stage_positive<T, RED>(ts, q0 + j, lane);
     }
 }
 
@@ -508,22 +643,29 @@
     }
 }
 
+static int sweep_queries_per_block(int qstride) { return SW_QFLOATS / qstride < 32 ? SW_QFLOATS / qstride : 32; }
+
 template <typename T, int VEC, int IT, int RED>
-static void launch_fwd(const NegPtArgs& a, float* out, int64_t ld, const FuseArgs* fuse, hipStream_t st) {
+static void launch_fwd(const NegPtArgs& a, float* out, int64_t ld, const FuseArgs* fuse, hipStream_t st,
+                       const TripleStage* ts = nullptr) {
     const int64_t items = a.n_query * a.items_per_query;
     constexpr int EPL = IT * VEC;
     constexpr int UNROLL = EPL <= 16 ? 4 : (EPL <= 32 ? 2 : 1);
     if (!fuse && a.sweep_shift >= 0) {
         SweepArgs s;
         s.qstride = IT * 16 * VEC;
-        s.qb = SW_QFLOATS / s.qstride < 32 ? SW_QFLOATS / s.qstride : 32;
+        s.qb = sweep_queries_per_block(s.qstride);
         s.kc = a.n_neg < SW_PMAX / s.qb ? a.n_neg : SW_PMAX / s.qb;
         s.n_kchunks = static_cast<int>(ceil_div(a.n_neg, s.kc));
         s.shift = a.sweep_shift;
         const int64_t blocks = ceil_div(a.n_query, s.qb) * s.n_kchunks * 8;
         const int lds = s.qb * s.qstride * static_cast<int>(sizeof(float));
-        k_neg_pertriple_fwd_sweep<T, VEC, IT, RED, UNROLL>
-            <<<static_cast<unsigned>(blocks), 256, lds, st>>>(a, s, out, ld);
+        if (ts)
+            k_neg_pertriple_fwd_sweep<T, VEC, IT, RED, UNROLL, true>
+                <<<static_cast<unsigned>(blocks), 256, lds, st>>>(a, s, out, ld, *ts);
+        else
+            k_neg_pertriple_fwd_sweep<T, VEC, IT, RED, UNROLL>
+                <<<static_cast<unsigned>(blocks), 256, lds, st>>>(a, s, out, ld, NoStage{});
     } else if (fuse) {
         constexpr int FU = EPL <= 16 ? 2 : 1;
         k_neg_pertriple_fwd<T, VEC, IT, RED, FU, true><<<ceil_div(items, 4), 256, 0, st>>>(a, out, ld, *fuse);
@@ -542,30 +684,30 @@
 
 template <typename T, int VEC, int IT>
 static void by_red(int red, bool fwd, const NegPtArgs& a, float* out, const float* d_out, int64_t ld,
-                   float* dq, float* dn, const FuseArgs* fuse, hipStream_t st) {
+                   float* dq, float* dn, const FuseArgs* fuse, hipStream_t st, const TripleStage* ts) {
     switch (red) {
         case RED_DOT:
-            fwd ? launch_fwd<T, VEC, IT, RED_DOT>(a, out, ld, fuse, st)
+            fwd ? launch_fwd<T, VEC, IT, RED_DOT>(a, out, ld, fuse, st, ts)
                 : launch_bwd<T, VEC, IT, RED_DOT>(a, d_out, ld, dq, dn, st);
             break;
         case RED_L1:
-            fwd ? launch_fwd<T, VEC, IT, RED_L1>(a, out, ld, fuse, st)
+            fwd ? launch_fwd<T, VEC, IT, RED_L1>(a, out, ld, fuse, st, ts)
                 : launch_bwd<T, VEC, IT, RED_L1>(a, d_out, ld, dq, dn, st);
             break;
         default:
-            fwd ? launch_fwd<T, VEC, IT, RED_L2>(a, out, ld, fuse, st)
+            fwd ? launch_fwd<T, VEC, IT, RED_L2>(a, out, ld, fuse, st, ts)
                 : launch_bwd<T, VEC, IT, RED_L2>(a, d_out, ld, dq, dn, st);
     }
 }
 
 template <typename T, int VEC>
 static int by_it(int it, int red, bool fwd, const NegPtArgs& a, float* out, const float* d_out,
-                 int64_t ld, float* dq, float* dn, const FuseArgs* fuse, hipStream_t st) {
-    if (it <= 1) by_red<T, VEC, 1>(red, fwd, a, out, d_out, ld, dq, dn, fuse, st);
-    else if (it <= 2) by_red<T, VEC, 2>(red, fwd, a, out, d_out, ld, dq, dn, fuse, st);
-    else if (it <= 4) by_red<T, VEC, 4>(red, fwd, a, out, d_out, ld, dq, dn, fuse, st);
-    else if (it <= 8) by_red<T, VEC, 8>(red, fwd, a, out, d_out, ld, dq, dn, fuse, st);
-    else if (it <= 16) by_red<T, VEC, 16>(red, fwd, a, out, d_out, ld, dq, dn, fuse, st);
+                 int64_t ld, float* dq, float* dn, const FuseArgs* fuse, hipStream_t st, const TripleStage* ts) {
+    if (it <= 1) by_red<T, VEC, 1>(red, fwd, a, out, d_out, ld, dq, dn, fuse, st, ts);
+    else if (it <= 2) by_red<T, VEC, 2>(red, fwd, a, out, d_out, ld, dq, dn, fuse, st, ts);
+    else if (it <= 4) by_red<T, VEC, 4>(red, fwd, a, out, d_out, ld, dq, dn, fuse, st, ts);
+    else if (it <= 8) by_red<T, VEC, 8>(red, fwd, a, out, d_out, ld, dq, dn, fuse, st, ts);
+    else if (it <= 16) by_red<T, VEC, 16>(red, fwd, a, out, d_out, ld, dq, dn, fuse, st, ts);
     else return fail(BESS_EUNSUPPORTED, "neg_score_pertriple: row of %d scalars too wide", a.W);
     return BESS_OK;
 }
@@ -596,11 +738,11 @@
 static int run(const bess_model_desc* d, bool fwd, const float* query, int64_t n_query,
                const void* neg_base, const int32_t* neg_idx, int64_t n_neg, float* out,
                const float* d_out, int64_t ld, float* dq, float* dn, void* stream,
-               const FuseArgs* fuse = nullptr) {
+               const FuseArgs* fuse = nullptr, TripleStage* ts = nullptr) {
     if (int e = check_desc(d)) return e;
     BESS_REQUIRE(n_query >= 0 && n_neg >= 0 && n_neg < (1ll << 31), "neg_score_pertriple: bad sizes");
     if (n_query == 0 || n_neg == 0) return BESS_OK;
-    BESS_REQUIRE(query && neg_base && neg_idx, "neg_score_pertriple: NULL pointer");
+    BESS_REQUIRE((query || ts) && neg_base && neg_idx, "neg_score_pertriple: NULL pointer");
     BESS_REQUIRE(ld >= n_neg, "neg_score_pertriple: leading dimension %lld < n_neg %lld", (long long)ld,
                  (long long)n_neg);
     if (d->scorer == BESS_BOXE)
@@ -625,6 +767,17 @@
     a.p = static_cast<float>(d->norm_p);
     a.dn_by_row = (!fwd && (d->reserved[0] & BESS_FLAG_DNEG_BY_ROW)) ? 1 : 0;
     if (fwd && !fuse) a.sweep_shift = sweep_shift_for(d, n_query, n_neg);
+    if (ts) {
+        if (a.sweep_shift < 0)
+            return fail(BESS_EUNSUPPORTED, "neg_score_pertriple_fwd_triples: not a row-ordered launch");
+        const int it = static_cast<int>(ceil_div(a.nch, 16));
+        const int qb = sweep_queries_per_block((it <= 2 ? it : it <= 4 ? 4 : it <= 8 ? 8 : 16) * 16 * vec);
+        BESS_REQUIRE(qb >= 1 && qb <= 32, "neg_score_pertriple_fwd_triples: %d queries per block (8 workgroups x 4 waves score "
+                     "one positive each)", qb);
+        const bool cplx = is_complex_entity(d->scorer);
+        const uintptr_t al = reinterpret_cast<uintptr_t>(ts->q.ent_base) | reinterpret_cast<uintptr_t>(ts->q.rel_table);
+        ts->vec = al % 16 == 0 && d->rel_width % vec == 0 && (!cplx || (W / 2) % vec == 0);
+    }
     const int red = reduce_of(d);
     hipStream_t st = as_stream(stream);
     if (!fwd && a.items_per_query > 1 && dq) {
@@ -652,12 +805,12 @@
         float* dnw = dn ? dn + col0 : nullptr;
         int rc = BESS_OK;
         if (d->dtype == BESS_F32) {
-            if (vec == 4) rc = by_it<float, 4>(it, red, fwd, w, out, d_out, ld, dqw, dnw, fuse, st);
-            else rc = by_it<float, 1>(it, red, fwd, w, out, d_out, ld, dqw, dnw, fuse, st);
+            if (vec == 4) rc = by_it<float, 4>(it, red, fwd, w, out, d_out, ld, dqw, dnw, fuse, st, ts);
+            else rc = by_it<float, 1>(it, red, fwd, w, out, d_out, ld, dqw, dnw, fuse, st, ts);
         } else {
-            if (vec == 8) rc = by_it<half_t, 8>(it, red, fwd, w, out, d_out, ld, dqw, dnw, fuse, st);
-            else if (vec == 2) rc = by_it<half_t, 2>(it, red, fwd, w, out, d_out, ld, dqw, dnw, fuse, st);
-            else rc = by_it<half_t, 1>(it, red, fwd, w, out, d_out, ld, dqw, dnw, fuse, st);
+            if (vec == 8) rc = by_it<half_t, 8>(it, red, fwd, w, out, d_out, ld, dqw, dnw, fuse, st, ts);
+            else if (vec == 2) rc = by_it<half_t, 2>(it, red, fwd, w, out, d_out, ld, dqw, dnw, fuse, st, ts);
+            else rc = by_it<half_t, 1>(it, red, fwd, w, out, d_out, ld, dqw, dnw, fuse, st, ts);
         }
         if (rc) return rc;
     }
@@ -691,6 +844,33 @@
     if (!sweep || n_query < 0 || n_neg < 0) return bess::fail(BESS_EINVAL, "neg_pertriple_sweep: bad argument");
     *sweep = bess::sweep_shift_for(d, n_query, n_neg) >= 0 ? 1 : 0;
     return BESS_OK;
+}
+
+extern "C" int bess_neg_score_pertriple_fwd_triples(const bess_model_desc* d, int32_t side, const void* head_base,
+                                                    const int32_t* head_idx, const void* tail_base,
+                                                    const int32_t* tail_idx, const void* rel_table,
+                                                    const int32_t* rel_idx, int64_t n_triple, const void* neg_base,
+                                                    const int32_t* neg_idx, int64_t n_neg, float* pos, float* out,
+                                                    int64_t ld_out, void* stream) {
+    using namespace bess;
+    if (int e = check_desc(d)) return e;
+    BESS_REQUIRE(side == BESS_CORRUPT_HEAD || side == BESS_CORRUPT_TAIL, "neg_score_pertriple_fwd_triples: bad side %d", side);
+    BESS_REQUIRE(n_triple >= 0 && n_neg >= 0 && n_neg < (1ll << 31), "neg_score_pertriple_fwd_triples: bad sizes");
+    if (sweep_shift_for(d, n_triple, n_neg) < 0)
+        return fail(BESS_EUNSUPPORTED, "neg_score_pertriple_fwd_triples: %lld x %lld pairs are not scored in row order "
+                                       "(bess_neg_pertriple_sweep)", (long long)n_triple, (long long)n_neg);
+    BESS_REQUIRE(head_base && tail_base && rel_table && rel_idx && neg_base && neg_idx && pos && out,
+                 "neg_score_pertriple_fwd_triples: NULL pointer");
+    const bool tail = side == BESS_CORRUPT_TAIL;
+    TripleStage ts;
+    ts.t = TripleArgs{head_base, head_idx, tail_base, tail_idx, rel_table, rel_idx, n_triple, d->width, d->rel_width, d->norm_p};
+    ts.q = QueryArgs{tail ? head_base : tail_base, tail ? head_idx : tail_idx, rel_table, rel_idx, n_triple, d->width,
+                     d->rel_width, side};
+    ts.pos = pos;
+    ts.scorer = d->scorer;
+    ts.vec = 0;
+    return run(d, true, nullptr, n_triple, neg_base, neg_idx, n_neg, out, nullptr, ld_out, nullptr, nullptr, stream, nullptr,
+               &ts);
 }
 
 static int64_t row_bytes_of(const bess_model_desc* d) {
diff --git a/bess-kge_amd/csrc/plan.hip b/bess-kge_amd/csrc/plan.hip
--- a/bess-kge_amd/csrc/plan.hip
+++ b/bess-kge_amd/csrc/plan.hip
@@ -55,6 +55,7 @@
     BESS_PLAN_FN(bess_query_triple_bwd),
     BESS_PLAN_FN(bess_query_triple_bwd_parts),
     BESS_PLAN_FN(bess_neg_score_pertriple_fwd),
+    BESS_PLAN_FN(bess_neg_score_pertriple_fwd_triples),
     BESS_PLAN_FN(bess_neg_score_pertriple_bwd),
     BESS_PLAN_FN(bess_neg_score_pertriple_fwd_dq),
     BESS_PLAN_FN(bess_neg_score_pertriple_fwd_dq_masked),
diff --git a/bess-kge_amd/csrc/prepare.hip b/bess-kge_amd/csrc/prepare.hip
--- a/bess-kge_amd/csrc/prepare.hip
+++ b/bess-kge_amd/csrc/prepare.hip
@@ -1,64 +1,9 @@
 #include "common.h"
 #include "loss_rows.h"
+#include "triple_rows.h"
 
 namespace bess {
 
-struct TripleArgs {
-    const void* head_base;
-    const int32_t* head_idx;
-    const void* tail_base;
-    const int32_t* tail_idx;
-    const void* rel_table;
-    const int32_t* rel_idx;
-    int64_t n;
-    int W;
-    int Wr;
-    int norm_p;
-};
-
-template <typename T, int SCORER>
-__device__ __forceinline__ void triple_fwd_body(const TripleArgs& a, int64_t s, int lane, float* __restrict__ out) {
-    const T* h = row_ptr(static_cast<const T*>(a.head_base), a.head_idx, s, a.W);
-    const T* t = row_ptr(static_cast<const T*>(a.tail_base), a.tail_idx, s, a.W);
-    const T* r = static_cast<const T*>(a.rel_table) + static_cast<int64_t>(a.rel_idx[s]) * a.Wr;
-    float acc = 0.f;
-    if (SCORER == BESS_TRANSE) {
-        for (int e = lane; e < a.W; e += 64) {
-            const float x = to_f32(h[e]) + to_f32(r[e]) - to_f32(t[e]);
-            acc += (a.norm_p == 1) ? fabsf(x) : lp_term(x, static_cast<float>(a.norm_p));
-        }
-    } else if (SCORER == BESS_DISTMULT) {
-        for (int e = lane; e < a.W; e += 64) acc += to_f32(h[e]) * to_f32(r[e]) * to_f32(t[e]);
-    } else {
-        const int d = a.W / 2;
-        for (int e = lane; e < d; e += 64) {
-            const float hr = to_f32(h[e]), hi = to_f32(h[d + e]);
-            const float tr = to_f32(t[e]), ti = to_f32(t[d + e]);
-            float rr, ri;
-            if (SCORER == BESS_ROTATE) {
-                const float ph = to_f32(r[e]);
-                rr = cosf(ph);
-                ri = sinf(ph);
-            } else {
-                rr = to_f32(r[e]);
-                ri = to_f32(r[d + e]);
-            }
-            const float qr = hr * rr - hi * ri;
-            const float qi = hr * ri + hi * rr;
-            if (SCORER == BESS_ROTATE) {
-                const float xr = qr - tr, xi = qi - ti;
-                acc += (a.norm_p == 1) ? (fabsf(xr) + fabsf(xi))
-                                       : (lp_term(xr, static_cast<float>(a.norm_p)) + lp_term(xi, static_cast<float>(a.norm_p)));
-            } else {
-                acc += qr * tr + qi * ti;
-            }
-        }
-    }
-    acc = wave_allreduce_sum(acc);
-    if (SCORER == BESS_TRANSE || SCORER == BESS_ROTATE)
-        acc = -((a.norm_p == 1) ? acc : lp_root(acc, static_cast<float>(a.norm_p)));
-    if (lane == 0) out[s] = acc;
-}
 
 template <typename T, int SCORER>
 __global__ __launch_bounds__(256) void k_score_triple_fwd(TripleArgs a, float* __restrict__ out) {
@@ -66,47 +11,6 @@
     const int64_t s = blockIdx.x * 4ll + (threadIdx.x >> 6);
     if (s >= a.n) return;
     triple_fwd_body<T, SCORER>(a, s, lane, out);
-}
-
-struct QueryArgs {
-    const void* ent_base;
-    const int32_t* ent_idx;
-    const void* rel_table;
-    const int32_t* rel_idx;
-    int64_t n;
-    int W;
-    int Wr;
-    int side;
-};
-
-template <typename T, int SCORER>
-__device__ __forceinline__ void query_fwd_body(const QueryArgs& a, int64_t q, int lane, float* __restrict__ query) {
-    const T* x = row_ptr(static_cast<const T*>(a.ent_base), a.ent_idx, q, a.W);
-    const T* r = static_cast<const T*>(a.rel_table) + static_cast<int64_t>(a.rel_idx[q]) * a.Wr;
-    float* o = query + q * a.W;
-    const bool tail = a.side == BESS_CORRUPT_TAIL;
-    if (SCORER == BESS_TRANSE) {
-        for (int e = lane; e < a.W; e += 64)
-            o[e] = tail ? (to_f32(x[e]) + to_f32(r[e])) : (to_f32(x[e]) - to_f32(r[e]));
-    } else if (SCORER == BESS_DISTMULT) {
-        for (int e = lane; e < a.W; e += 64) o[e] = to_f32(x[e]) * to_f32(r[e]);
-    } else {
-        const int d = a.W / 2;
-        for (int e = lane; e < d; e += 64) {
-            const float xr = to_f32(x[e]), xi = to_f32(x[d + e]);
-            float rr, ri;
-            if (SCORER == BESS_ROTATE) {
-                const float ph = tail ? to_f32(r[e]) : -to_f32(r[e]);
-                rr = cosf(ph);
-                ri = sinf(ph);
-            } else {
-                rr = to_f32(r[e]);
-                ri = tail ? to_f32(r[d + e]) : -to_f32(r[d + e]);
-            }
-            o[e] = xr * rr - xi * ri;
-            o[d + e] = xr * ri + xi * rr;
-        }
-    }
 }
 
 template <typename T, int SCORER>
diff --git a/bess-kge_amd/csrc/triple_rows.h b/bess-kge_amd/csrc/triple_rows.h
--- /dev/null
+++ b/bess-kge_amd/csrc/triple_rows.h
@@ -0,0 +1,115 @@
+#pragma once
+#include "common.h"
+
+namespace bess {
+
+struct TripleArgs {
+    const void* head_base;
+    const int32_t* head_idx;
+    const void* tail_base;
+    const int32_t* tail_idx;
+    const void* rel_table;
+    const int32_t* rel_idx;
+    int64_t n;
+    int W;
+    int Wr;
+    int norm_p;
+};
+
+template <typename T, int SCORER>
+__device__ __forceinline__ void triple_fwd_body(const TripleArgs& a, int64_t s, int lane, float* __restrict__ out) {
+    const T* h = row_ptr(static_cast<const T*>(a.head_base), a.head_idx, s, a.W);
+    const T* t = row_ptr(static_cast<const T*>(a.tail_base), a.tail_idx, s, a.W);
+    const T* r = static_cast<const T*>(a.rel_table) + static_cast<int64_t>(a.rel_idx[s]) * a.Wr;
+    float acc = 0.f;
+    if (SCORER == BESS_TRANSE) {
+        for (int e = lane; e < a.W; e += 64) {
+            const float x = to_f32(h[e]) + to_f32(r[e]) - to_f32(t[e]);
+            acc += (a.norm_p == 1) ? fabsf(x) : lp_term(x, static_cast<float>(a.norm_p));
+        }
+    } else if (SCORER == BESS_DISTMULT) {
+        for (int e = lane; e < a.W; e += 64) acc += to_f32(h[e]) * to_f32(r[e]) * to_f32(t[e]);
+    } else {
+        const int d = a.W / 2;
+        for (int e = lane; e < d; e += 64) {
+            const float hr = to_f32(h[e]), hi = to_f32(h[d + e]);
+            const float tr = to_f32(t[e]), ti = to_f32(t[d + e]);
+            float rr, ri;
+            if (SCORER == BESS_ROTATE) {
+                const float ph = to_f32(r[e]);
+                rr = cosf(ph);
+                ri = sinf(ph);
+            } else {
+                rr = to_f32(r[e]);
+                ri = to_f32(r[d + e]);
+            }
+            const float qr = hr * rr - hi * ri;
+            const float qi = hr * ri + hi * rr;
+            if (SCORER == BESS_ROTATE) {
+                const float xr = qr - tr, xi = qi - ti;
+                acc += (a.norm_p == 1) ? (fabsf(xr) + fabsf(xi))
+                                       : (lp_term(xr, static_cast<float>(a.norm_p)) + lp_term(xi, static_cast<float>(a.norm_p)));
+            } else {
+                acc += qr * tr + qi * ti;
+            }
+        }
+    }
+    acc = wave_allreduce_sum(acc);
+    if (SCORER == BESS_TRANSE || SCORER == BESS_ROTATE)
+        acc = -((a.norm_p == 1) ? acc : lp_root(acc, static_cast<float>(a.norm_p)));
+    if (lane == 0) out[s] = acc;
+}
+
+struct QueryArgs {
+    const void* ent_base;
+    const int32_t* ent_idx;
+    const void* rel_table;
+    const int32_t* rel_idx;
+    int64_t n;
+    int W;
+    int Wr;
+    int side;
+};
+
+template <int SCORER>
+__device__ __forceinline__ float query_scalar(float x, float r, bool tail) {
+    if (SCORER == BESS_TRANSE) return tail ? (x + r) : (x - r);
+    return x * r;
+}
+
+template <int SCORER>
+__device__ __forceinline__ void query_pair(float xr, float xi, float r0, float r1, bool tail, float& qr, float& qi) {
+    float rr, ri;
+    if (SCORER == BESS_ROTATE) {
+        const float ph = tail ? r0 : -r0;
+        rr = cosf(ph);
+        ri = sinf(ph);
+    } else {
+        rr = r0;
+        ri = tail ? r1 : -r1;
+    }
+    qr = fmaf(xr, rr, -__fmul_rn(xi, ri));
+    qi = fmaf(xi, rr, __fmul_rn(xr, ri));
+}
+
+template <typename T, int SCORER>
+__device__ __forceinline__ void query_fwd_body(const QueryArgs& a, int64_t q, int lane, float* __restrict__ query) {
+    const T* x = row_ptr(static_cast<const T*>(a.ent_base), a.ent_idx, q, a.W);
+    const T* r = static_cast<const T*>(a.rel_table) + static_cast<int64_t>(a.rel_idx[q]) * a.Wr;
+    float* o = query + q * a.W;
+    const bool tail = a.side == BESS_CORRUPT_TAIL;
+    if (SCORER == BESS_TRANSE || SCORER == BESS_DISTMULT) {
+        for (int e = lane; e < a.W; e += 64) o[e] = query_scalar<SCORER>(to_f32(x[e]), to_f32(r[e]), tail);
+    } else {
+        const int d = a.W / 2;
+        for (int e = lane; e < d; e += 64) {
+            const float r1 = SCORER == BESS_ROTATE ? 0.f : to_f32(r[d + e]);
+            float qr, qi;
+            query_pair<SCORER>(to_f32(x[e]), to_f32(x[d + e]), to_f32(r[e]), r1, tail, qr, qi);
+            o[e] = qr;
+            o[d + e] = qi;
+        }
+    }
+}
+
+}
diff --git a/include/besskge_hip.h b/include/besskge_hip.h
--- a/include/besskge_hip.h
+++ b/include/besskge_hip.h
@@ -127,6 +127,12 @@
                                  const int32_t* neg_idx, int64_t n_neg, float* out,
                                  int64_t ld_out, void* stream);
 int bess_neg_pertriple_sweep(const bess_model_desc* d, int64_t n_query, int64_t n_neg, int32_t* sweep);
+
+int bess_neg_score_pertriple_fwd_triples(const bess_model_desc* d, int32_t side, const void* head_base,
+                                         const int32_t* head_idx, const void* tail_base, const int32_t* tail_idx,
+                                         const void* rel_table, const int32_t* rel_idx, int64_t n_triple,
+                                         const void* neg_base, const int32_t* neg_idx, int64_t n_neg, float* pos,
+                                         float* out, int64_t ld_out, void* stream);
 
 int bess_neg_score_pertriple_bwd(const bess_model_desc* d, const float* query,
                                  int64_t n_query, const void* neg_base,
```
